# NilanEkanayake/TiTok-Video

Hardware: AMD Instinct MI355X
Metric: video clips/sec encode+decode (whole node) (higher is better)
Workload: dtype bf16

## Files before the change

### titok_video_amd/csrc/ttv_api.hip

```cpp
#include <stdarg.h>
#include <stdio.h>
#include <stdlib.h>
#include <string.h>

#include "ttv_common.h"
#include "ttv_kernels.h"

static thread_local char g_err[512] = "";

void ttv_set_error(const char* fmt, ...) {
  va_list ap;
  va_start(ap, fmt);
  vsnprintf(g_err, sizeof(g_err), fmt, ap);
  va_end(ap);
}

int g_ttv_prof_class = 0;
thread_local int g_ttv_debug = 0;
long long* g_ttv_stamps = nullptr;
static hipEvent_t* g_prof_start = nullptr;
static hipEvent_t* g_prof_stop = nullptr;
static int g_prof_cap = 0, g_prof_n = 0;

TtvProfScope::TtvProfScope(int cls, hipStream_t stream) : slot(-1), s(stream) {
  if (g_ttv_prof_class != 0 && cls == g_ttv_prof_class && g_prof_n < g_prof_cap) {
    slot = g_prof_n++;
    (void)hipEventRecord(g_prof_start[slot], s);
  }
}
TtvProfScope::~TtvProfScope() {
  if (slot >= 0) (void)hipEventRecord(g_prof_stop[slot], s);
}

#define TTV_TRY(expr)            \
  do {                           \
    int rc__ = (expr);           \
    if (rc__ != TTV_OK) return rc__; \
  } while (0)

static inline int esize(int dtype) { return dtype == TTV_BF16 ? 2 : 4; }
static inline int64_t align_up(int64_t v) { return (v + 255) & ~(int64_t)255; }

struct TowerWs {
  char *x, *xn, *qkv, *ao, *h, *pa, *pb;
  char *xl, *aol;
  char *f8, *f8mx;
  float* y32;
  float* rstd;
  int64_t total;
};

static TowerWs carve(const ttv_tower_dims* d, const ttv_batch* b, char* base) {
  const int64_t e = esize(d->dtype);
  const int64_t L = b->total_rows, P = b->sum_patches;
  const int64_t g = (int64_t)d->kv_heads * d->head_dim;
  const int64_t pd = (int64_t)d->pix_channels * d->patch_t * d->patch_h * d->patch_w;
  int64_t off = 0;
  TowerWs w;
  auto take = [&](int64_t bytes) { char* p = base ? base + off : nullptr; off += align_up(bytes); return p; };
  w.x = take(L * d->width * e);
  w.xn = take(L * d->width * e);
  w.qkv = take(L * (2 * d->width + 2 * g) * e);
  w.ao = take(L * d->width * e);
  w.y32 = (float*)take(L * d->width * 4);
  w.h = take(L * d->inner * e);
  w.pa = take(P * pd * e);
  w.pb = take(P * d->width * e);
  w.rstd = (float*)take(L * 4);
  w.xl = take((int64_t)b->sum_tokens * d->width * e);
  w.aol = take((int64_t)b->sum_tokens * d->width * e);
  w.f8 = w.f8mx = nullptr;
  if (d->dtype == TTV_BF16 && d->width != 256 && d->width % 128 == 0) {
    const int64_t wide = d->width > d->inner ? d->width : d->inner;
    w.f8 = take(L * wide);
    w.f8mx = take(L * (wide / 128 + 4) * 4);
  }
  w.total = off;
  return w;
}

static int check_dims(const ttv_tower_dims* d, const ttv_batch* b) {
  TTV_CHECK_ARG(d && b, "null dims/batch");
  TTV_CHECK_ARG(d->dtype == TTV_BF16 || d->dtype == TTV_F32, "bad dtype %d", d->dtype);
  TTV_CHECK_ARG(d->head_dim == 64 && d->width == d->q_heads * 64, "width must be q_heads*64");
  TTV_CHECK_ARG(d->width % 64 == 0 && d->width <= 1024, "width %d unsupported", d->width);
  TTV_CHECK_ARG(d->inner % 32 == 0, "GEGLU inner dim must be a multiple of 32");
  TTV_CHECK_ARG(d->token_size >= 1 && d->token_size <= TTV_MAX_TOKEN, "token_size out of range");
  TTV_CHECK_ARG(((int64_t)d->pix_channels * d->patch_t * d->patch_h * d->patch_w) % 8 == 0, "patch vector length must be a multiple of 8");
  TTV_CHECK_ARG(b->n_clips > 0 && b->total_rows == b->sum_tokens + b->sum_patches, "inconsistent batch");
  return TTV_OK;
}

static int run_layer_mx(const ttv_tower_dims* d, const ttv_layer_weights& lw, const ttv_batch* b, const TowerWs& ws, int i, bool& rstd_valid,
                        bool& xq_valid, bool attn_pipe, hipStream_t s) {
  const int L = b->total_rows, dm = d->width, g = d->kv_heads * d->head_dim, dt = d->dtype, nq = 2 * dm + 2 * g, I = d->inner;
  static const bool fused_env = !(getenv("TTV_MX_FUSED_QUANT") && getenv("TTV_MX_FUSED_QUANT")[0] == '0');
  const bool fused_q = fused_env && !(g_ttv_debug & 2048);
  if (!rstd_valid) TTV_TRY(ttvk_row_rstd(ws.x, dt, dm, ws.rstd, L, dm, d->eps, s));
  if (!xq_valid) TTV_TRY(ttvk_quant_mx_fp8(ws.x, dt, dm, ws.f8, dm, ws.f8mx, nullptr, L, dm, s));
  xq_valid = false;
  GemmArgs a = {};
  a.dtype = dt; a.x = ws.f8; a.ldx = dm; a.w = lw.to_qkv_f8; a.ldw = dm; a.M = L; a.N = nq; a.K = dm; a.y = ws.qkv; a.ldy = nq;
  a.rope_cs = b->rope_cs; a.rope_q_end = dm; a.rope_k_begin = 2 * dm; a.rope_k_end = 2 * dm + g;
  TTV_TRY(ttvk_gemm_fp8(EPI_QKV_ROPE, a, ws.rstd, lw.to_qkv_f8_scale, s, ws.f8mx, lw.to_qkv_mx));
  const bool q_scaled = lw.qkv_q_prescaled != 0;
  if (fused_q && q_scaled && !b->qblocks_paired && !attn_pipe && d->head_dim == 64) {
    TTV_TRY(ttvk_attention_mxout(ws.qkv, nq, ws.f8, ws.f8mx, (int)ttvk_mx_scale_ld(dm), b->cu_seqlens, b->qblocks, b->n_qblocks, d->q_heads,
                                 d->kv_heads, s));
  } else {
    TTV_TRY(ttvk_attention(ws.qkv, nq, ws.ao, dm, b->cu_seqlens, b->qblocks, b->n_qblocks, d->q_heads, d->kv_heads, d->head_dim,
                           TTV_ATTN_GATE | (b->qblocks_paired ? TTV_ATTN_PAIRED : 0) | (q_scaled ? TTV_ATTN_QSCALED : 0) |
                               ((b->qblocks_all_full && attn_pipe) ? TTV_ATTN_ALLFULL : 0) | (attn_pipe ? TTV_ATTN_PIPE : 0), dt, s));
    TTV_TRY(ttvk_quant_mx_fp8(ws.ao, dt, dm, ws.f8, dm, ws.f8mx, nullptr, L, dm, s));
  }
  GemmArgs o = {};
  o.dtype = dt; o.x = ws.f8; o.ldx = dm; o.w = lw.out_proj_f8; o.ldw = dm; o.M = L; o.N = dm; o.K = dm; o.resid = ws.x; o.ldr = dm;
  o.alpha = i == 0 ? 1.f : d->alpha; o.y = ws.x; o.ldy = dm;
  TTV_TRY(ttvk_gemm_fp8(EPI_RESID_T, o, nullptr, lw.out_proj_f8_scale, s, ws.f8mx, lw.out_proj_mx));
  if (i > 0) {
    TTV_TRY(ttvk_rmsnorm(ws.x, dt, dm, nullptr, ws.x, dt, dm, nullptr, lw.attn_post_ln, L, dm, d->eps, s, ws.rstd, fused_q ? ws.f8 : nullptr,
                         fused_q ? ws.f8mx : nullptr));
    if (!fused_q) TTV_TRY(ttvk_quant_mx_fp8(ws.x, dt, dm, ws.f8, dm, ws.f8mx, nullptr, L, dm, s));
  } else {
    TTV_TRY(ttvk_row_rstd(ws.x, dt, dm, ws.rstd, L, dm, d->eps, s));
    TTV_TRY(ttvk_quant_mx_fp8(ws.x, dt, dm, ws.f8, dm, ws.f8mx, nullptr, L, dm, s));
  }
  GemmArgs f = {};
  f.dtype = dt; f.x = ws.f8; f.ldx = dm; f.w = lw.w12_f8; f.ldw = dm; f.M = L; f.N = I; f.K = dm; f.y = ws.h; f.ldy = I;
  char* const hq = ws.h;
  char* const hq_mx = ws.xn;
  const bool h_fused = fused_q && (int64_t)ttvk_mx_scale_ld(I) <= (int64_t)dm * 2;
  if (h_fused) { f.yq = hq; f.yq_mx = hq_mx; }
  TTV_TRY(ttvk_gemm_fp8(EPI_GEGLU, f, ws.rstd, lw.w12_f8_scale, s, ws.f8mx, lw.w12_mx));
  GemmArgs f3 = {};
  if (h_fused) {
    f3.x = hq;
  } else {
    TTV_TRY(ttvk_quant_mx_fp8(ws.h, dt, I, ws.f8, I, ws.f8mx, nullptr, L, I, s));
    f3.x = ws.f8;
  }
  f3.dtype = dt; f3.ldx = I; f3.w = lw.w3_f8; f3.ldw = I; f3.M = L; f3.N = dm; f3.K = I; f3.resid = ws.x; f3.ldr = dm;
  f3.alpha = i == 0 ? 1.f : d->alpha; f3.y = ws.x; f3.ldy = dm;
  TTV_TRY(ttvk_gemm_fp8(EPI_RESID_T, f3, nullptr, lw.w3_f8_scale, s, h_fused ? hq_mx : ws.f8mx, lw.w3_mx));
  rstd_valid = false;
  if (i > 0) {
    TTV_TRY(ttvk_rmsnorm(ws.x, dt, dm, nullptr, ws.x, dt, dm, nullptr, lw.ffd_post_ln, L, dm, d->eps, s, ws.rstd, fused_q ? ws.f8 : nullptr,
                         fused_q ? ws.f8mx : nullptr));
    rstd_valid = true;
    xq_valid = fused_q;
  }
  return TTV_OK;
}

static bool rows_f8(int dt, int dm, const void* img, const void* row_scale, const void* mx, const void* folded) {
  return dt == TTV_BF16 && img && row_scale && !mx && dm % 128 == 0 && !(dm == 256 && folded);
}

static int run_layers(const ttv_tower_dims* d, const ttv_tower_weights* w, const ttv_batch* b, const TowerWs& ws, hipStream_t s) {
  const int L = b->total_rows, dm = d->width, g = d->kv_heads * d->head_dim, dt = d->dtype;
  const int split3 = (dt == TTV_F32 && w->f32_split3) ? 1 : 0;
  const bool gen_ok = (dt == TTV_BF16 && dm != 256) || split3;
  static const bool s3img_env = !(getenv("TTV_SPLIT3_IMAGES") && getenv("TTV_SPLIT3_IMAGES")[0] == '0');
  const int s3img = (split3 && s3img_env && !(g_ttv_debug & 4096)) ? 1 : 0;
  const int nq = 2 * dm + 2 * g;
  bool qkv_ready = false;
  bool rstd_valid = false;
  bool xq_valid = false;
  static const bool attn_pipe = getenv("TTV_ATTN_PIPE") && getenv("TTV_ATTN_PIPE")[0] == '1';
  static const bool lat_env = !(getenv("TTV_ENC_LATENT_LAST") && getenv("TTV_ENC_LATENT_LAST")[0] == '0');
  const bool lat_last = lat_env && !(g_ttv_debug & 524288) && d->kind == TTV_ENCODER && b->qblocks_latent && b->n_qblocks_latent > 0 &&
                        b->latent_rows && b->sum_tokens > 0 && b->sum_tokens < L;
  static const bool pat_env = !(getenv("TTV_DEC_PATCH_LAST") && getenv("TTV_DEC_PATCH_LAST")[0] == '0');
  const bool pat_last = pat_env && !(g_ttv_debug & 2097152) && d->kind == TTV_DECODER && d->layers >= 2 && b->qblocks_patch &&
                        b->n_qblocks_patch > 0 && !split3 && !b->qblocks_paired;
  bool compacted = false;
  for (int i = 0; i < d->layers; ++i) {
    const ttv_layer_weights& lw = w->layers[i];
    static const bool keel_f32 = getenv("TTV_KEEL_F32SUM") && getenv("TTV_KEEL_F32SUM")[0] == '1';
    if (dt == TTV_BF16 && dm != 256 && dm % 128 == 0 && d->inner % 128 == 0 && !keel_f32 && lw.to_qkv_f8 && lw.to_qkv_mx && lw.w12_f8 && lw.w12_mx &&
        lw.out_proj_f8 && lw.out_proj_mx && lw.w3_f8 && lw.w3_mx &&
        !(lat_last && i == d->layers - 1)) {
      TTV_TRY(run_layer_mx(d, lw, b, ws, i, rstd_valid, xq_valid, attn_pipe, s));
      qkv_ready = false;
      continue;
    }
    xq_valid = false;
    const bool f8_qkv = rows_f8(dt, dm, lw.to_qkv_f8, lw.to_qkv_f8_scale, lw.to_qkv_mx, lw.to_qkv_pn);
    const bool f8_w12 = rows_f8(dt, dm, lw.w12_f8, lw.w12_f8_scale, lw.w12_mx, lw.w12_pn);
    float* const f8_scales = reinterpret_cast<float*>(ws.xn + (((size_t)L * dm + 255) & ~(size_t)255));
    if (!qkv_ready && f8_qkv) {
      TTV_TRY(ttvk_quant_rows_fp8(ws.x, dt, dm, lw.pre_ln, d->eps, ws.xn, dm, f8_scales, L, dm, s));
      GemmArgs a = {};
      a.dtype = dt; a.x = ws.xn; a.ldx = dm; a.w = lw.to_qkv_f8; a.ldw = dm; a.M = L; a.N = nq; a.K = dm; a.y = ws.qkv; a.ldy = nq;
      a.rope_cs = b->rope_cs; a.rope_q_end = dm; a.rope_k_begin = 2 * dm; a.rope_k_end = 2 * dm + g;
      TTV_TRY(ttvk_gemm_fp8(EPI_QKV_ROPE, a, f8_scales, lw.to_qkv_f8_scale, s));
    } else if (!qkv_ready) {
      const bool fold_qkv = dt == TTV_BF16 && dm == 256 && lw.to_qkv_pn;
      const bool fold_gen = gen_ok && lw.to_qkv_pn;
      if (fold_gen && !rstd_valid) TTV_TRY(ttvk_row_rstd(ws.x, dt, dm, ws.rstd, L, dm, d->eps, s));
      if (!fold_qkv && !fold_gen) TTV_TRY(ttvk_rmsnorm(ws.x, dt, dm, nullptr, ws.xn, dt, dm, nullptr, lw.pre_ln, L, dm, d->eps, s, nullptr, nullptr, nullptr, s3img));
      GemmArgs a = {};
      a.dtype = dt; a.split3 = split3; a.x_image = s3img && !fold_qkv && !fold_gen; a.y_image = s3img ? 2 : 0;
      a.prenorm = fold_qkv; a.eps = d->eps;
      a.row_scale = fold_gen ? ws.rstd : nullptr;
      const void* w_plain = (dt == TTV_BF16 && lw.to_qkv_qs) ? lw.to_qkv_qs : lw.to_qkv;
      a.x = (fold_qkv || fold_gen) ? ws.x : ws.xn; a.ldx = dm; a.w = (fold_qkv || fold_gen) ? lw.to_qkv_pn : w_plain; a.ldw = dm; a.M = L; a.N = nq; a.K = dm; a.y = ws.qkv; a.ldy = nq;
      a.rope_cs = b->rope_cs; a.rope_q_end = dm; a.rope_k_begin = 2 * dm; a.rope_k_end = 2 * dm + g;
      a.rope_ids = b->rope_ids; a.rope_base = b->rope_ids ? b->rope_base : nullptr;
      TTV_TRY(ttvk_gemm(EPI_QKV_ROPE, a, s));
    }
    const bool q_scaled = dt == TTV_BF16 && (lw.to_qkv_pn ? lw.qkv_q_prescaled != 0 : lw.to_qkv_qs != nullptr);
    rstd_valid = false;
    qkv_ready = false;
    const bool lat_now = lat_last && i == d->layers - 1;
    if (lat_now)
      TTV_TRY(ttvk_attention(ws.qkv, nq, ws.ao, dm, b->cu_seqlens, b->qblocks_latent, b->n_qblocks_latent, d->q_heads, d->kv_heads, d->head_dim,
                             TTV_ATTN_GATE | (b->qblocks_all_full ? TTV_ATTN_ALLFULL : 0) | (q_scaled ? TTV_ATTN_QSCALED : 0) | (split3 ? TTV_ATTN_SPLIT3 : 0) |
                                 (s3img ? (TTV_ATTN_SPLIT_OUT | TTV_ATTN_SPLIT_IN) : 0), dt, s));
    else if (pat_last && i == d->layers - 1 && dt == TTV_BF16 && !attn_pipe)
      TTV_TRY(ttvk_attention(ws.qkv, nq, ws.ao, dm, b->cu_seqlens, b->qblocks_patch, b->n_qblocks_patch, d->q_heads, d->kv_heads, d->head_dim,
                             TTV_ATTN_GATE | (b->qblocks_all_full ? TTV_ATTN_ALLFULL : 0) | (q_scaled ? TTV_ATTN_QSCALED : 0), dt, s));
    else if (q_scaled && b->items64 && b->n_items64 > 0 && d->head_dim == 64)
      TTV_TRY(ttvk_attention64(ws.qkv, nq, ws.ao, dm, b->cu_seqlens, b->items64, b->n_items64, d->q_heads, d->kv_heads,
                               TTV_ATTN_GATE | TTV_ATTN_QSCALED, s));
    else
    TTV_TRY(ttvk_attention(ws.qkv, nq, ws.ao, dm, b->cu_seqlens, b->qblocks, b->n_qblocks, d->q_heads, d->kv_heads, d->head_dim,
                           TTV_ATTN_GATE | (b->qblocks_paired ? TTV_ATTN_PAIRED : 0) | (q_scaled ? TTV_ATTN_QSCALED : 0) |
                               (b->qblocks_all_full ? TTV_ATTN_ALLFULL : 0) | (attn_pipe ? TTV_ATTN_PIPE : 0) | (split3 ? TTV_ATTN_SPLIT3 : 0) |
                               (s3img ? (TTV_ATTN_SPLIT_OUT | TTV_ATTN_SPLIT_IN) : 0), dt, s));
    char* cx = ws.x;
    char* cao = ws.ao;
    int Lc = L;
    if (lat_now) {
      const int64_t rb = (int64_t)dm * esize(dt);
      TTV_TRY(ttvk_copy_rows(ws.x, (int64_t)dm * esize(dt), b->latent_rows, ws.xl, (int64_t)dm * esize(dt), nullptr, b->sum_tokens, dm * (int)esize(dt), s));
      TTV_TRY(ttvk_copy_rows(ws.ao, rb, b->latent_rows, ws.aol, rb, nullptr, b->sum_tokens, (int)rb, s));
      cx = ws.xl; cao = ws.aol; Lc = b->sum_tokens;
      compacted = true;
    }
    static const bool keel_f32sum = getenv("TTV_KEEL_F32SUM") && getenv("TTV_KEEL_F32SUM")[0] == '1';
    static const bool use_fused_mlp = !(getenv("TTV_FUSED_MLP") && getenv("TTV_FUSED_MLP")[0] == '0');
    static const bool use_fused_qkv = getenv("TTV_FUSED_QKV") && getenv("TTV_FUSED_QKV")[0] == '1';
    if (use_fused_mlp && ttvk_mlp_fused_supported(dt, dm, d->inner) && lw.mlp_pack) {
      MlpNextQkv nx = {};
      const bool back = use_fused_qkv && i + 1 < d->layers && lw.mlp_pack_qkv_rows == nq && nq % 64 == 0 && dm % 64 == 0 && g % 64 == 0;
      if (back) { nx.qkv = ws.qkv; nx.ld = nq; nx.rope_cs = b->rope_cs; nx.rows = nq; nx.rope_q_end = dm; nx.rope_k_begin = 2 * dm; nx.rope_k_end = 2 * dm + g; }
      TTV_TRY(ttvk_mlp_fused(cao, dm, i == 0 ? nullptr : lw.attn_post_ln, i == 0 ? 1.f : d->alpha, cx, dm, lw.mlp_pack, d->inner,
                             cx, dm, i == 0 ? nullptr : lw.ffd_post_ln, i == 0 ? 1.f : d->alpha, d->eps, Lc, back ? &nx : nullptr, s));
      qkv_ready = back;
      continue;
    }
    GemmArgs o = {};
    o.dtype = dt; o.split3 = split3; o.x_image = s3img;
    o.x = cao; o.ldx = dm; o.w = lw.out_proj; o.ldw = dm; o.M = Lc; o.N = dm; o.K = dm; o.resid = cx; o.ldr = dm;
    if (i == 0) {
      o.alpha = 1.f; o.y = cx; o.ldy = dm;
      TTV_TRY(ttvk_gemm(EPI_RESID_T, o, s));
    } else if (ttvk_gemm_supports_resid_norm(dt, dm, dm)) {
      o.alpha = d->alpha; o.y = cx; o.ldy = dm; o.norm_gain = lw.attn_post_ln; o.eps = d->eps;
      TTV_TRY(ttvk_gemm(EPI_RESID_NORM, o, s));
    } else {
      const bool want = gen_ok && lw.w12_pn && !f8_w12;
      if (dt == TTV_BF16 && !keel_f32sum) {
        o.alpha = d->alpha; o.y = cx; o.ldy = dm;
        TTV_TRY(ttvk_gemm(EPI_RESID_T, o, s));
        TTV_TRY(ttvk_rmsnorm(cx, dt, dm, nullptr, cx, dt, dm, nullptr, lw.attn_post_ln  , Lc, dm, d->eps, s, want ? ws.rstd : nullptr));
      } else {
        o.alpha = d->alpha; o.y = ws.y32; o.ldy = dm;
        TTV_TRY(ttvk_gemm(EPI_RESID_F32, o, s));
        TTV_TRY(ttvk_rmsnorm(ws.y32, TTV_F32, dm, nullptr, cx, dt, dm, nullptr, lw.attn_post_ln  , Lc, dm, d->eps, s, want ? ws.rstd : nullptr));
      }
      rstd_valid = want;
    }
    const bool fold_ffd = dt == TTV_BF16 && dm == 256 && lw.w12_pn;
    const bool fold_ffd_gen = gen_ok && lw.w12_pn && !f8_w12;
    if (f8_w12) {
      TTV_TRY(ttvk_quant_rows_fp8(cx, dt, dm, lw.ffd_norm, d->eps, ws.xn, dm, f8_scales, Lc, dm, s));
      GemmArgs f = {};
      f.dtype = dt; f.x = ws.xn; f.ldx = dm; f.w = lw.w12_f8; f.ldw = dm; f.M = Lc; f.N = d->inner; f.K = dm; f.y = ws.h; f.ldy = d->inner;
      TTV_TRY(ttvk_gemm_fp8(EPI_GEGLU, f, f8_scales, lw.w12_f8_scale, s));
    } else {
    if (fold_ffd_gen && !rstd_valid) TTV_TRY(ttvk_row_rstd(cx, dt, dm, ws.rstd  , Lc, dm, d->eps, s));
    if (!fold_ffd && !fold_ffd_gen) TTV_TRY(ttvk_rmsnorm(cx, dt, dm, nullptr, ws.xn, dt, dm, nullptr, lw.ffd_norm  , Lc, dm, d->eps, s, nullptr, nullptr, nullptr, s3img));
    GemmArgs f = {};
    f.dtype = dt; f.split3 = split3; f.x_image = s3img && !fold_ffd && !fold_ffd_gen; f.y_image = s3img;
    f.prenorm = fold_ffd; f.eps = d->eps;
    f.row_scale = fold_ffd_gen ? ws.rstd : nullptr;
    f.x = (fold_ffd || fold_ffd_gen) ? cx : ws.xn; f.ldx = dm; f.w = (fold_ffd || fold_ffd_gen) ? lw.w12_pn : lw.w12; f.ldw = dm; f.M = Lc; f.N = d->inner; f.K = dm; f.y = ws.h; f.ldy = d->inner;
    TTV_TRY(ttvk_gemm(EPI_GEGLU, f, s));
    }
    rstd_valid = false;
    GemmArgs f3 = {};
    f3.dtype = dt; f3.split3 = split3; f3.x_image = s3img;
    f3.x = ws.h; f3.ldx = d->inner; f3.w = lw.w3; f3.ldw = d->inner; f3.M = Lc; f3.N = dm; f3.K = d->inner; f3.resid = cx; f3.ldr = dm;
    if (i == 0) {
      f3.alpha = 1.f; f3.y = cx; f3.ldy = dm;
      TTV_TRY(ttvk_gemm(EPI_RESID_T, f3, s));
    } else if (ttvk_gemm_supports_resid_norm(dt, dm, d->inner)) {
      f3.alpha = d->alpha; f3.y = cx; f3.ldy = dm; f3.norm_gain = lw.ffd_post_ln; f3.eps = d->eps;
      TTV_TRY(ttvk_gemm(EPI_RESID_NORM, f3, s));
    } else {
      const bool want = gen_ok && i + 1 < d->layers && w->layers[i + 1].to_qkv_pn &&
                        !rows_f8(dt, dm, w->layers[i + 1].to_qkv_f8, w->layers[i + 1].to_qkv_f8_scale, w->layers[i + 1].to_qkv_mx, w->layers[i + 1].to_qkv_pn);
      if (dt == TTV_BF16 && !keel_f32sum) {
        f3.alpha = d->alpha; f3.y = cx; f3.ldy = dm;
        TTV_TRY(ttvk_gemm(EPI_RESID_T, f3, s));
        TTV_TRY(ttvk_rmsnorm(cx, dt, dm, nullptr, cx, dt, dm, nullptr, lw.ffd_post_ln  , Lc, dm, d->eps, s, want ? ws.rstd : nullptr));
      } else {
        f3.alpha = d->alpha; f3.y = ws.y32; f3.ldy = dm;
        TTV_TRY(ttvk_gemm(EPI_RESID_F32, f3, s));
        TTV_TRY(ttvk_rmsnorm(ws.y32, TTV_F32, dm, nullptr, cx, dt, dm, nullptr, lw.ffd_post_ln  , Lc, dm, d->eps, s, want ? ws.rstd : nullptr));
      }
      rstd_valid = want;
    }
  }
  if (compacted)
    TTV_TRY(ttvk_copy_rows(ws.xl, (int64_t)dm * esize(dt), nullptr, ws.x, (int64_t)dm * esize(dt), b->latent_rows, b->sum_tokens, dm * (int)esize(dt), s));
  return TTV_OK;
}

extern "C" {

const char* ttv_error_string(void) { return g_err; }
int ttv_version(void) { return 100; }

int ttv_fsq_forward(const ttv_fsq_params* p, const void* z, int z_dtype, int rows, void* codes, int codes_dtype, int32_t* indices,
                    float* bounded, void* stream) {
  TTV_CHECK_ARG(rows >= 0 && (rows == 0 || (z && codes && indices)), "fsq_forward: null buffer");
  return ttvk_fsq_forward(p, z, z_dtype, rows, codes, codes_dtype, indices, bounded, (hipStream_t)stream);
}

int ttv_fsq_indices_to_codes(const ttv_fsq_params* p, const int32_t* indices, int rows, void* codes, int codes_dtype, void* stream) {
  TTV_CHECK_ARG(rows >= 0 && (rows == 0 || (indices && codes)), "fsq_indices_to_codes: null buffer");
  return ttvk_fsq_indices_to_codes(p, indices, rows, codes, codes_dtype, (hipStream_t)stream);
}

int ttv_vq_codebook_norms(const void* codebook, int dtype, int ld, int N, int C, float* cnorm, void* stream) {
  TTV_CHECK_ARG(N == 0 || (codebook && cnorm), "vq_codebook_norms: null buffer");
  return ttvk_vq_norms(codebook, dtype, ld, N, C, cnorm, (hipStream_t)stream);
}

int64_t ttv_vq_workspace_bytes(int rows) { return ttvk_vq_workspace_bytes(rows); }

int ttv_vq_l2_argmin(const void* z, int dtype, int ldz, const void* codebook, int ldc, const float* cnorm, int rows, int N, int C,
                     int32_t* indices, float* best_dist, void* workspace, int64_t workspace_bytes, void* stream) {
  TTV_CHECK_ARG(rows == 0 || (z && codebook && cnorm && indices), "vq_l2_argmin: null buffer");
  TTV_CHECK_ARG(ldz >= C && ldc >= C, "vq_l2_argmin: leading dims smaller than the codebook dim");
  return ttvk_vq_l2_argmin(z, dtype, ldz, codebook, ldc, cnorm, rows, N, C, indices, best_dist, workspace, workspace_bytes, (hipStream_t)stream);
}

int ttv_vq_lookup(const void* codebook, int dtype, int ldc, const int32_t* indices, int rows, int C, void* codes, int ldo, void* stream) {
  TTV_CHECK_ARG(rows == 0 || (codebook && indices && codes), "vq_lookup: null buffer");
  return ttvk_vq_lookup(codebook, dtype, ldc, indices, rows, C, codes, ldo, (hipStream_t)stream);
}

int ttv_vq_lookup_backward(const void* dcodes, int dtype, int ld, const int32_t* indices, int rows, int C, float* dcodebook, int ldc, void* stream) {
  TTV_CHECK_ARG(rows == 0 || (dcodes && indices && dcodebook), "vq_lookup_backward: null buffer");
  TTV_CHECK_ARG(ld >= C && ldc >= C, "vq_lookup_backward: leading dims smaller than the codebook dim");
  return ttvk_vq_lookup_bwd(dcodes, dtype, ld, indices, rows, C, dcodebook, ldc, (hipStream_t)stream);
}

int ttv_quant_rows_fp8(const void* in, int dtype, int ld_in, const float* gain, float eps, void* out, int ld_out, float* scales, int rows,
                       int width, void* stream) {
  TTV_CHECK_ARG(rows == 0 || (in && out && scales), "quant_rows_fp8: null buffer");
  return ttvk_quant_rows_fp8(in, dtype, ld_in, gain, eps, out, ld_out, scales, rows, width, (hipStream_t)stream);
}

int ttv_split3_pack(const float* w, int ldw, void* out, int ldo, int rows, int K, void* stream) {
  TTV_CHECK_ARG(rows == 0 || (w && out), "split3_pack: null buffer");
  return ttvk_split3_pack(w, ldw, out, ldo, rows, K, (hipStream_t)stream);
}

int ttv_linear_split3(const float* x, int ldx, const void* w_image, int ldw, const float* bias, float* y, int ldy, int M, int N, int K, void* stream) {
  TTV_CHECK_ARG(M == 0 || (x && w_image && y), "linear_split3: null buffer");
  GemmArgs a = {};
  a.dtype = TTV_F32; a.split3 = 1; a.x = x; a.ldx = ldx; a.w = w_image; a.ldw = ldw; a.M = M; a.N = N; a.K = K; a.y = y; a.ldy = ldy; a.bias = bias;
  return ttvk_gemm(EPI_STORE, a, (hipStream_t)stream);
}

int64_t ttv_mx_scale_bytes_per_row(int width) { return ttvk_mx_scale_ld(width); }

int ttv_quant_mx_fp8(const void* in, int dtype, int ld_in, void* out, int ld_out, void* mx, float* row_scales, int rows, int width, void* stream) {
  TTV_CHECK_ARG(rows == 0 || (in && out && mx), "quant_mx_fp8: null buffer");
  TTV_CHECK_ARG(ld_in >= width && ld_out >= width, "quant_mx_fp8: leading dims smaller than the width");
  return ttvk_quant_mx_fp8(in, dtype, ld_in, out, ld_out, mx, row_scales, rows, width, (hipStream_t)stream);
}

int ttv_linear_fp8_mx(const void* xq, int ldx, const void* x_mx, const float* x_row_scale, const void* wq, int ldw, const void* w_mx,
                      const float* w_row_scale, void* y, int ldy, int M, int N, int K, int epilogue, const float* rope_cs, int d_model,
                      int gqa_dim, const void* resid, int ldr, float alpha, void* stream) {
  TTV_CHECK_ARG(M == 0 || (xq && wq && y && x_mx && w_mx), "linear_fp8_mx: null buffer");
  TTV_CHECK_ARG(epilogue >= 0 && epilogue <= 3, "linear_fp8_mx: epilogue 0 (store), 1 (qkv + rotary), 2 (GEGLU) or 3 (alpha * resid + acc)");
  GemmArgs a = {};
  a.dtype = TTV_BF16; a.x = xq; a.ldx = ldx; a.w = wq; a.ldw = ldw; a.M = M; a.N = N; a.K = K; a.y = y; a.ldy = ldy;
  if (epilogue == 1) {
    TTV_CHECK_ARG(rope_cs && N == 2 * d_model + 2 * gqa_dim, "linear_fp8_mx: qkv epilogue needs rope_cs and N = 2 d_model + 2 gqa_dim");
    a.rope_cs = rope_cs; a.rope_q_end = d_model; a.rope_k_begin = 2 * d_model; a.rope_k_end = 2 * d_model + gqa_dim;
  }
  if (epilogue == 3) { a.resid = resid; a.ldr = ldr; a.alpha = alpha; }
  return ttvk_gemm_fp8(epilogue == 0 ? EPI_STORE : epilogue == 1 ? EPI_QKV_ROPE : epilogue == 2 ? EPI_GEGLU : EPI_RESID_T, a, x_row_scale,
                       w_row_scale, (hipStream_t)stream, x_mx, w_mx);
}

int ttv_linear_fp8(const void* xq, int ldx, const float* x_scale, const void* wq, int ldw, const float* w_scale, void* y, int ldy, int M, int N,
                   int K, int epilogue, const float* rope_cs, int d_model, int gqa_dim, void* stream) {
  TTV_CHECK_ARG(M == 0 || (xq && wq && y), "linear_fp8: null buffer");
  TTV_CHECK_ARG(epilogue >= 0 && epilogue <= 2, "linear_fp8: epilogue 0 (store), 1 (qkv + rotary) or 2 (GEGLU)");
  GemmArgs a = {};
  a.dtype = TTV_BF16; a.x = xq; a.ldx = ldx; a.w = wq; a.ldw = ldw; a.M = M; a.N = N; a.K = K; a.y = y; a.ldy = ldy;
  if (epilogue == 1) {
    TTV_CHECK_ARG(rope_cs && N == 2 * d_model + 2 * gqa_dim, "linear_fp8: qkv epilogue needs rope_cs and N = 2 d_model + 2 gqa_dim");
    a.rope_cs = rope_cs; a.rope_q_end = d_model; a.rope_k_begin = 2 * d_model; a.rope_k_end = 2 * d_model + gqa_dim;
  }
  return ttvk_gemm_fp8(epilogue == 0 ? EPI_STORE : epilogue == 1 ? EPI_QKV_ROPE : EPI_GEGLU, a, x_scale, w_scale, (hipStream_t)stream);
}

int ttv_rmsnorm(const void* in, int in_dtype, int ld_in, const int32_t* src_rows, void* out, int out_dtype, int ld_out,
                const int32_t* dst_rows, const float* gain, int rows, int width, float eps, void* stream) {
  TTV_CHECK_ARG(rows >= 0 && (rows == 0 || (in && out && gain)), "rmsnorm: null buffer");
  return ttvk_rmsnorm(in, in_dtype, ld_in, src_rows, out, out_dtype, ld_out, dst_rows, gain, rows, width, eps, (hipStream_t)stream);
}

int ttv_rope_apply(void* x, int dtype, int ld, int rows, int heads, const float* rope_cs, void* stream) {
  TTV_CHECK_ARG(rows == 0 || (x && rope_cs), "rope_apply: null buffer");
  TTV_CHECK_ARG(ld % 4 == 0 && ld >= heads * 64, "rope_apply: bad leading dim");
  return ttvk_rope_apply(x, dtype, ld, rows, heads, rope_cs, (hipStream_t)stream);
}

int ttv_linear(const void* x, int ldx, const void* w, int ldw, const void* bias, const float* add_scalar, void* y, int ldy, int M,
               int N, int K, int dtype, void* stream) {
  TTV_CHECK_ARG(M == 0 || (x && w && y), "linear: null buffer");
  GemmArgs a = {};
  a.dtype = dtype; a.x = x; a.ldx = ldx; a.w = w; a.ldw = ldw; a.M = M; a.N = N; a.K = K; a.y = y; a.ldy = ldy;
  a.bias = bias; a.add_scalar = add_scalar;
  return ttvk_gemm(EPI_STORE, a, (hipStream_t)stream);
}

int ttv_linear_qkv_rope(const void* x, int ldx, const void* w, int ldw, void* y, int ldy, int M, int d_model, int gqa_dim,
                        const float* rope_cs, int dtype, void* stream) {
  TTV_CHECK_ARG(M == 0 || (x && w && y && rope_cs), "linear_qkv_rope: null buffer");
  GemmArgs a = {};
  a.dtype = dtype; a.x = x; a.ldx = ldx; a.w = w; a.ldw = ldw; a.M = M; a.N = 2 * d_model + 2 * gqa_dim; a.K = d_model;
  a.y = y; a.ldy = ldy; a.rope_cs = rope_cs; a.rope_q_end = d_model; a.rope_k_begin = 2 * d_model; a.rope_k_end = 2 * d_model + gqa_dim;
  return ttvk_gemm(EPI_QKV_ROPE, a, (hipStream_t)stream);
}

int ttv_linear_geglu(const void* x, int ldx, const void* w, int ldw, void* y, int ldy, int M, int I, int K, int dtype, void* stream) {
  TTV_CHECK_ARG(M == 0 || (x && w && y), "linear_geglu: null buffer");
  GemmArgs a = {};
  a.dtype = dtype; a.x = x; a.ldx = ldx; a.w = w; a.ldw = ldw; a.M = M; a.N = I; a.K = K; a.y = y; a.ldy = ldy;
  return ttvk_gemm(EPI_GEGLU, a, (hipStream_t)stream);
}

int ttv_linear_residual(const void* x, int ldx, const void* w, int ldw, const void* resid, int ldr, float alpha, void* y, int ldy,
                        int y_f32, int M, int N, int K, int dtype, void* stream) {
  TTV_CHECK_ARG(M == 0 || (x && w && y && resid), "linear_residual: null buffer");
  GemmArgs a = {};
  a.dtype = dtype; a.x = x; a.ldx = ldx; a.w = w; a.ldw = ldw; a.M = M; a.N = N; a.K = K; a.y = y; a.ldy = ldy;
  a.resid = resid; a.ldr = ldr; a.alpha = alpha;
  return ttvk_gemm(y_f32 ? EPI_RESID_F32 : EPI_RESID_T, a, (hipStream_t)stream);
}

int ttv_linear_residual_norm(const void* x, int ldx, const void* w, int ldw, const void* resid, int ldr, float alpha,
                             const float* gain, float eps, void* y, int ldy, int M, int N, int K, int dtype, void* stream) {
  TTV_CHECK_ARG(M == 0 || (x && w && y && resid && gain), "linear_residual_norm: null buffer");
  GemmArgs a = {};
  a.dtype = dtype; a.x = x; a.ldx = ldx; a.w = w; a.ldw = ldw; a.M = M; a.N = N; a.K = K; a.y = y; a.ldy = ldy;
  a.resid = resid; a.ldr = ldr; a.alpha = alpha; a.norm_gain = gain; a.eps = eps;
  if (!ttvk_gemm_supports_resid_norm(dtype, N, K)) {
    ttv_set_error("linear_residual_norm: only bf16 with N == 256 has a fused kernel");
    return TTV_ERR_UNSUPPORTED;
  }
  return ttvk_gemm(EPI_RESID_NORM, a, (hipStream_t)stream);
}

int64_t ttv_mlp_pack_bytes(int inner, int next_qkv_rows) { return ttvk_mlp_pack_bytes(inner, next_qkv_rows); }

int ttv_mlp_pack(const void* w12_folded, const void* w3, const void* out_proj, const void* next_qkv_folded, int next_qkv_rows, int inner,
                 int width, int dtype, void* packed, void* stream) {
  if (!ttvk_mlp_fused_supported(dtype, width, inner)) {
    ttv_set_error("mlp_pack: only bf16, width 256, inner %% 32 == 0");
    return TTV_ERR_UNSUPPORTED;
  }
  return ttvk_mlp_pack(w12_folded, w3, out_proj, next_qkv_folded, next_qkv_rows, inner, packed, (hipStream_t)stream);
}

int ttv_mlp_fused(const void* x, int ldx, const void* mlp_packed, int inner, void* y, int ldy, const float* post_gain, float alpha,
                  float eps, int M, int width, int dtype, void* stream) {
  if (!ttvk_mlp_fused_supported(dtype, width, inner)) {
    ttv_set_error("mlp_fused: only bf16, width 256, inner %% 32 == 0");
    return TTV_ERR_UNSUPPORTED;
  }
  return ttvk_mlp_fused(nullptr, 0, nullptr, 1.f, x, ldx, mlp_packed, inner, y, ldy, post_gain, alpha, eps, M, nullptr, (hipStream_t)stream);
}

int ttv_layer_tail_fused(const void* ao, int ldao, const float* attn_post_gain, float attn_alpha, const void* x, int ldx,
                         const void* mlp_packed, int inner, void* y, int ldy, const float* ffd_post_gain, float ffd_alpha, float eps,
                         int M, int width, int dtype, const ttv_next_qkv* next, void* stream) {
  if (!ttvk_mlp_fused_supported(dtype, width, inner)) {
    ttv_set_error("layer_tail_fused: only bf16, width 256, inner %% 32 == 0");
    return TTV_ERR_UNSUPPORTED;
  }
  TTV_CHECK_ARG(ao, "layer_tail_fused: null attention output");
  MlpNextQkv nx = {};
  if (next) { nx.qkv = next->qkv; nx.ld = next->ld; nx.rope_cs = next->rope_cs; nx.rows = next->rows; nx.rope_q_end = next->rope_q_end;
              nx.rope_k_begin = next->rope_k_begin; nx.rope_k_end = next->rope_k_end; }
  return ttvk_mlp_fused(ao, ldao, attn_post_gain, attn_alpha, x, ldx, mlp_packed, inner, y, ldy, ffd_post_gain, ffd_alpha, eps, M,
                        next ? &nx : nullptr, (hipStream_t)stream);
}

int ttv_fill_const_rows(void* x, int dtype, int ld, const int32_t* rows_map, int rows, int width, const float* mask_token,
                        const float* gain, float eps, void* stream) {
  TTV_CHECK_ARG(rows == 0 || (x && rows_map && mask_token && gain), "fill_const_rows: null buffer");
  return ttvk_fill_const_rows(x, dtype, ld, rows_map, rows, width, mask_token, gain, eps, (hipStream_t)stream);
}

int ttv_decoder_embed(const void* codes, int token_size, const void* w, const void* bias, const float* mask_token, const float* gain,
                      void* x, int dtype, int ld, const int32_t* rows_map, int rows, int width, float eps, void* stream) {
  TTV_CHECK_ARG(rows == 0 || (codes && w && bias && mask_token && gain && x && rows_map), "decoder_embed: null buffer");
  return ttvk_dec_embed(codes, token_size, w, bias, mask_token, gain, x, dtype, ld, rows_map, rows, width, eps, (hipStream_t)stream);
}

int ttv_attention(const void* qkvg, int ld, void* out, int ldo, const int32_t* cu_seqlens, const int32_t* qblocks, int n_qblocks,
                  int q_heads, int kv_heads, int head_dim, int flags, int dtype, void* stream) {
  TTV_CHECK_ARG(n_qblocks == 0 || (qkvg && out && cu_seqlens && qblocks), "attention: null buffer");
  return ttvk_attention(qkvg, ld, out, ldo, cu_seqlens, qblocks, n_qblocks, q_heads, kv_heads, head_dim, flags, dtype, (hipStream_t)stream);
}
int ttv_attention64(const void* qkvg, int ld, void* out, int ldo, const int32_t* cu_seqlens, const int32_t* items, int n_items, int q_heads,
                    int kv_heads, int head_dim, int flags, int dtype, void* stream) {
  TTV_CHECK_ARG(dtype == TTV_BF16 && head_dim == 64, "attention64: bf16, head_dim 64 only");
  return ttvk_attention64(qkvg, ld, out, ldo, cu_seqlens, items, n_items, q_heads, kv_heads, flags, (hipStream_t)stream);
}

int ttv_patch_gather(const void* const* clips, const int32_t* clip_desc, int clip0, int n_clips, int patch_t, int patch_h, int patch_w,
                     int channels, void* patches, int ld, int dtype, int max_patches_per_clip, void* stream) {
  TTV_CHECK_ARG(n_clips == 0 || (clips && clip_desc && patches), "patch_gather: null buffer");
  return ttvk_patch_copy(false, (void* const*)clips, clip_desc, clip0, n_clips, patch_t, patch_h, patch_w, channels, patches, ld, dtype, max_patches_per_clip, (hipStream_t)stream);
}

int ttv_patch_scatter(const void* patches, int ld, const int32_t* clip_desc, int clip0, int n_clips, int patch_t, int patch_h, int patch_w,
                      int channels, void* const* clips, int dtype, int max_patches_per_clip, void* stream) {
  TTV_CHECK_ARG(n_clips == 0 || (clips && clip_desc && patches), "patch_scatter: null buffer");
  return ttvk_patch_copy(true, clips, clip_desc, clip0, n_clips, patch_t, patch_h, patch_w, channels, (void*)patches, ld, dtype, max_patches_per_clip, (hipStream_t)stream);
}

int64_t ttv_tower_workspace_bytes(const ttv_tower_dims* dims, const ttv_batch* batch) {
  if (check_dims(dims, batch) != TTV_OK) return -1;
  return carve(dims, batch, nullptr).total;
}

int ttv_encoder_forward(const ttv_tower_dims* d, const ttv_tower_weights* w, const ttv_batch* b, const void* const* clips,
                        const ttv_fsq_params* fsq, float* z, void* codes, int32_t* indices, float* bounded, void* workspace,
                        int64_t workspace_bytes, void* stream) {
  TTV_TRY(check_dims(d, b));
  TTV_CHECK_ARG(d->kind == TTV_ENCODER, "encoder_forward: dims.kind is not TTV_ENCODER");
  TTV_CHECK_ARG(w && w->layers && clips && workspace, "encoder_forward: null argument");
  TTV_CHECK_ARG(fsq || z, "encoder_forward: neither fsq nor z requested");
  TTV_CHECK_ARG(!fsq || (codes && indices), "encoder_forward: fsq needs codes and indices buffers");
  hipStream_t s = (hipStream_t)stream;
  TowerWs ws = carve(d, b, (char*)workspace);
  TTV_CHECK_ARG(ws.total <= workspace_bytes, "encoder_forward: workspace too small (%lld < %lld)", (long long)workspace_bytes, (long long)ws.total);
  const int dm = d->width, dt = d->dtype, P = b->sum_patches;
  const int pd = d->pix_channels * d->patch_t * d->patch_h * d->patch_w;

  static const bool use_fused_patch = !(getenv("TTV_FUSED_PATCH") && getenv("TTV_FUSED_PATCH")[0] == '0');
  auto pow2 = [](int v) { return v > 0 && (v & (v - 1)) == 0; };
  const bool gather = use_fused_patch && dt == TTV_BF16 && d->patch_w == 8 && pow2(d->patch_t) && pow2(d->patch_h) &&
                      b->n_clips <= TTV_MAX_CLIPS_PER_LAUNCH && b->row_seq && pd % 64 == 0 && pd != 256;
  if (!gather) {
    for (int c0 = 0; c0 < b->n_clips; c0 += TTV_MAX_CLIPS_PER_LAUNCH) {
      const int n = b->n_clips - c0 < TTV_MAX_CLIPS_PER_LAUNCH ? b->n_clips - c0 : TTV_MAX_CLIPS_PER_LAUNCH;
      TTV_TRY(ttvk_patch_copy(false, (void* const*)(clips + c0), b->clip_desc, c0, n, d->patch_t, d->patch_h, d->patch_w, d->pix_channels, ws.pa, pd, dt, b->max_patches_per_clip, s));
    }
  }
  GemmArgs a = {};
  a.dtype = dt; a.x = ws.pa; a.ldx = pd; a.w = w->proj_in_w; a.ldw = pd; a.M = P; a.N = dm; a.K = pd; a.y = ws.pb; a.ldy = dm;
  a.bias = w->proj_in_b; a.add_scalar = w->mask_token;
  a.split3 = (dt == TTV_F32 && w->f32_split3) ? 1 : 0;
  if (gather) {
    a.gather = 1; a.clips = (void* const*)clips; a.n_clips = b->n_clips; a.clip_desc = b->clip_desc; a.patch_rows = b->patch_rows;
    a.row_seq = b->row_seq; a.patch_t = d->patch_t; a.patch_h = d->patch_h; a.patch_w = d->patch_w;
  }
  TTV_TRY(ttvk_gemm(EPI_STORE, a, s));
  TTV_TRY(ttvk_rmsnorm(ws.pb, dt, dm, nullptr, ws.x, dt, dm, b->patch_rows, w->ln_pre_p, P, dm, d->eps, s));
  TTV_TRY(ttvk_fill_const_rows(ws.x, dt, dm, b->latent_rows, b->sum_tokens, dm, w->mask_token, w->ln_pre_t, d->eps, s));

  TTV_TRY(run_layers(d, w, b, ws, s));

  TTV_TRY(ttvk_enc_tail(ws.x, dt, dm, b->latent_rows, b->sum_tokens, dm, w->ln_post, d->eps, w->proj_out_w, w->proj_out_b, d->token_size, fsq, z, codes, indices, bounded, s));
  return TTV_OK;
}

int ttv_decoder_forward(const ttv_tower_dims* d, const ttv_tower_weights* w, const ttv_batch* b, const void* codes,
                        void* const* clips_out, void* workspace, int64_t workspace_bytes, void* stream) {
  TTV_TRY(check_dims(d, b));
  TTV_CHECK_ARG(d->kind == TTV_DECODER, "decoder_forward: dims.kind is not TTV_DECODER");
  TTV_CHECK_ARG(w && w->layers && codes && clips_out && workspace, "decoder_forward: null argument");
  hipStream_t s = (hipStream_t)stream;
  TowerWs ws = carve(d, b, (char*)workspace);
  TTV_CHECK_ARG(ws.total <= workspace_bytes, "decoder_forward: workspace too small (%lld < %lld)", (long long)workspace_bytes, (long long)ws.total);
  const int dm = d->width, dt = d->dtype, P = b->sum_patches;
  const int pd = d->pix_channels * d->patch_t * d->patch_h * d->patch_w;

  TTV_TRY(ttvk_dec_embed(codes, d->token_size, w->proj_in_w, w->proj_in_b, w->mask_token, w->ln_pre_t, ws.x, dt, dm, b->latent_rows, b->sum_tokens, dm, d->eps, s));
  TTV_TRY(ttvk_fill_const_rows(ws.x, dt, dm, b->patch_rows, P, dm, w->mask_token, w->ln_pre_p, d->eps, s));

  TTV_TRY(run_layers(d, w, b, ws, s));

  GemmArgs a = {};
  a.dtype = dt; a.w = w->proj_out_w; a.ldw = dm; a.M = P; a.N = pd; a.K = dm; a.y = ws.pa; a.ldy = pd; a.ldx = dm;
  a.split3 = (dt == TTV_F32 && w->f32_split3) ? 1 : 0;
  a.bias = w->proj_out_b;
  if (dt == TTV_BF16 && dm == 256 && w->proj_out_pn && pd % 8 == 0) {
    a.x = ws.x; a.x_rows = b->patch_rows; a.w = w->proj_out_pn; a.prenorm = 1; a.eps = d->eps;
  } else {
    TTV_TRY(ttvk_rmsnorm(ws.x, dt, dm, b->patch_rows, ws.pb, dt, dm, nullptr, w->ln_post, P, dm, d->eps, s));
    a.x = ws.pb;
  }
  static const bool use_fused_patch = !(getenv("TTV_FUSED_PATCH") && getenv("TTV_FUSED_PATCH")[0] == '0');
  auto pow2 = [](int v) { return v > 0 && (v & (v - 1)) == 0; };
  if (use_fused_patch && dt == TTV_BF16 && dm == 256 && d->patch_w == 8 && pow2(d->patch_t) && pow2(d->patch_h) &&
      b->n_clips <= TTV_MAX_CLIPS_PER_LAUNCH && b->row_seq && pd % 64 == 0) {
    a.clips = clips_out; a.n_clips = b->n_clips; a.clip_desc = b->clip_desc; a.patch_rows = b->patch_rows; a.row_seq = b->row_seq;
    a.patch_t = d->patch_t; a.patch_h = d->patch_h; a.patch_w = d->patch_w;
    return ttvk_gemm(EPI_STORE_PATCH, a, s);
  }
  TTV_TRY(ttvk_gemm(EPI_STORE, a, s));
  for (int c0 = 0; c0 < b->n_clips; c0 += TTV_MAX_CLIPS_PER_LAUNCH) {
    const int n = b->n_clips - c0 < TTV_MAX_CLIPS_PER_LAUNCH ? b->n_clips - c0 : TTV_MAX_CLIPS_PER_LAUNCH;
    TTV_TRY(ttvk_patch_copy(true, clips_out + c0, b->clip_desc, c0, n, d->patch_t, d->patch_h, d->patch_w, d->pix_channels, ws.pa, pd, dt, b->max_patches_per_clip, s));
  }
  return TTV_OK;
}

int ttv_rope_table_build(const float* base_cos, const float* base_sin, int n_ids, int n_freqs, const int32_t* clip_desc, const int32_t* cu_seqlens,
                         const int32_t* row_seq, float* rope_cs, int total_rows, void* stream) {
  TTV_CHECK_ARG(total_rows == 0 || (base_cos && base_sin && clip_desc && cu_seqlens && row_seq && rope_cs), "rope_table_build: null buffer");
  TTV_CHECK_ARG(n_freqs >= 1 && 3 * n_freqs <= 32 && n_ids >= 1, "rope_table_build: bad table shape");
  return ttvk_rope_build(base_cos, base_sin, n_ids, n_freqs, clip_desc, cu_seqlens, row_seq, rope_cs, total_rows, (hipStream_t)stream);
}

int ttv_l1_loss(void* const* recon, void* const* target, void* const* grad, const int32_t* sizes, int n_clips, int dtype, float* loss,
                void* stream) {
  for (int c0 = 0; c0 < n_clips; c0 += TTV_MAX_CLIPS_PER_LAUNCH) {
    const int n = n_clips - c0 < TTV_MAX_CLIPS_PER_LAUNCH ? n_clips - c0 : TTV_MAX_CLIPS_PER_LAUNCH;
    TTV_TRY(ttvk_l1_loss(recon + c0, target + c0, grad ? grad + c0 : nullptr, sizes + c0, n, n_clips, dtype, loss, (hipStream_t)stream));
  }
  return TTV_OK;
}

int ttv_clip_from_u8(const void* frames_thwc, int T, int H, int W, void* clip_cthw, int dtype, void* stream) {
  TTV_CHECK_ARG(frames_thwc && clip_cthw && T > 0 && H > 0 && W > 0, "clip_from_u8: bad argument");
  return ttvk_clip_from_u8(frames_thwc, (long long)T * H * W, clip_cthw, dtype, (hipStream_t)stream);
}

int ttv_sq_err_accumulate(void* const* recon, void* const* target, const int32_t* sizes, int n_clips, int dtype, int clamp, double* acc,
                          void* stream) {
  for (int c0 = 0; c0 < n_clips; c0 += TTV_MAX_CLIPS_PER_LAUNCH) {
    const int n = n_clips - c0 < TTV_MAX_CLIPS_PER_LAUNCH ? n_clips - c0 : TTV_MAX_CLIPS_PER_LAUNCH;
    TTV_TRY(ttvk_sq_err(recon + c0, target + c0, sizes + c0, n, dtype, clamp, acc, (hipStream_t)stream));
  }
  return TTV_OK;
}

int ttv_debug_set(int flags) {
  g_ttv_debug = flags;
  return TTV_OK;
}

int ttv_debug_stamps(void* device_buffer) {
  g_ttv_stamps = (long long*)device_buffer;
  return TTV_OK;
}

int ttv_prof_begin(int kernel_class, int max_records) {
  TTV_CHECK_ARG(g_ttv_prof_class == 0, "prof_begin: already recording");
  TTV_CHECK_ARG(kernel_class > 0 && max_records > 0 && max_records <= (1 << 20), "prof_begin: bad arguments");
  g_prof_start = new hipEvent_t[max_records];
  g_prof_stop = new hipEvent_t[max_records];
  for (int i = 0; i < max_records; ++i) {
    if (hipEventCreate(&g_prof_start[i]) != hipSuccess || hipEventCreate(&g_prof_stop[i]) != hipSuccess) {
      ttv_set_error("prof_begin: hipEventCreate failed");
      return TTV_ERR_LAUNCH;
    }
  }
  g_prof_cap = max_records;
  g_prof_n = 0;
  g_ttv_prof_class = kernel_class;
  return TTV_OK;
}

int ttv_prof_end(double* total_ms, int* count) {
  TTV_CHECK_ARG(g_ttv_prof_class != 0 && total_ms && count, "prof_end: not recording");
  g_ttv_prof_class = 0;
  double tot = 0.0;
  for (int i = 0; i < g_prof_n; ++i) {
    float ms = 0.f;
    (void)hipEventSynchronize(g_prof_stop[i]);
    (void)hipEventElapsedTime(&ms, g_prof_start[i], g_prof_stop[i]);
    tot += ms;
  }
  *total_ms = tot;
  *count = g_prof_n;
  for (int i = 0; i < g_prof_cap; ++i) {
    (void)hipEventDestroy(g_prof_start[i]);
    (void)hipEventDestroy(g_prof_stop[i]);
  }
  delete[] g_prof_start;
  delete[] g_prof_stop;
  g_prof_start = g_prof_stop = nullptr;
  g_prof_cap = g_prof_n = 0;
  return TTV_OK;
}

int ttv_codebook_histogram(const int32_t* indices, int n, int64_t* counts, int codebook_size, void* stream) {
  TTV_CHECK_ARG(n == 0 || (indices && counts), "codebook_histogram: null buffer");
  return ttvk_histogram(indices, n, counts, codebook_size, (hipStream_t)stream);
}

}
```

### titok_video_amd/csrc/ttv_attn.hip

```cpp
#include <stdlib.h>

#include "ttv_common.h"
#include "ttv_kernels.h"

#define QB 128
#define KB 64
#define ATTN_DEFER_THR 8.0f
#ifndef ATTN_LAZY
#define ATTN_LAZY 1
#endif
#ifndef ATTN_DMA_LATE
#define ATTN_DMA_LATE 1
#endif
#ifndef ATTN_PRIO
#define ATTN_PRIO 0
#endif
#define ATTN_LAZY_LOG2 30
#define ATTN_LAZY_BIG 1073741824.0f
typedef float f32x2 __attribute__((ext_vector_type(2)));

typedef __attribute__((address_space(3))) bf16x4 lds_bf16x4;

__device__ __forceinline__ bf16x4 lds_read_tr16(const char* lds_ptr) {
  return __builtin_amdgcn_ds_read_tr16_b64_v4bf16((lds_bf16x4*)(lds_ptr));
// ... 1044 lines not shown
        l_run += psum;
#pragma unroll
        for (int e = 0; e < 16; ++e) {
          const int vk = t * 32 + (e & 3) + 8 * (e >> 2) + 4 * h;
          const float v0 = vl[vk * 64 + r], v1 = vl[vk * 64 + 32 + r];
          o_acc[0] = __builtin_amdgcn_mfma_f32_32x32x2f32(v0, sc[e], o_acc[0], 0, 0, 0);
          o_acc[1] = __builtin_amdgcn_mfma_f32_32x32x2f32(v1, sc[e], o_acc[1], 0, 0, 0);
        }
      }
    }
  }
#undef A32_GLOAD
#undef A32_LSTORE
  if (!wave_live) return;

  const float l_tot = l_run + __shfl_xor(l_run, 32, 64);
  const float inv_l = 1.0f / l_tot;
  if (lse_out && qrow < q_lim && h == 0)
    lse_out[(size_t)(s0 + qrow) * (d_model >> 6) + head] = m_run * (c_exp * 0.69314718055994530942f) + logf(l_tot);
  if (qrow < q_lim) {
    float* orow = out + (size_t)(s0 + qrow) * ldo + head * 64;
    const float* grow = gbase + (size_t)qrow * ld;
#pragma unroll
    for (int dt = 0; dt < 2; ++dt)
#pragma unroll
      for (int g = 0; g < 4; ++g) {
        const int d0 = dt * 32 + 8 * g + 4 * h;
        f32x4 v = {o_acc[dt][4 * g] * inv_l, o_acc[dt][4 * g + 1] * inv_l, o_acc[dt][4 * g + 2] * inv_l, o_acc[dt][4 * g + 3] * inv_l};
        if (GATE) {
          const f32x4 gt = *reinterpret_cast<const f32x4*>(grow + d0);
#pragma unroll
          for (int e = 0; e < 4; ++e) v[e] *= 1.0f / (1.0f + expf(-gt[e]));
        }
        *reinterpret_cast<f32x4*>(orow + d0) = v;
      }
  }
}

__device__ __forceinline__ void split4_f32(const uint4 v, uint2& hi, uint2& lo) {
  const float x0 = __uint_as_float(v.x), x1 = __uint_as_float(v.y), x2 = __uint_as_float(v.z), x3 = __uint_as_float(v.w);
  const bf16_t h0 = (bf16_t)x0, h1 = (bf16_t)x1, h2 = (bf16_t)x2, h3 = (bf16_t)x3;
  const bf16x4 hv = {h0, h1, h2, h3};
  const bf16x4 lv = {(bf16_t)(x0 - (float)h0), (bf16_t)(x1 - (float)h1), (bf16_t)(x2 - (float)h2), (bf16_t)(x3 - (float)h3)};
  hi = __builtin_bit_cast(uint2, hv);
  lo = __builtin_bit_cast(uint2, lv);
}

template <bool GATE, bool IMG = false>
__global__ __launch_bounds__(256, 2) void k_attn_split3(const float* __restrict__ qkvg, int ld, float* __restrict__ out, int ldo,
                                                        const int* __restrict__ cu, const int* __restrict__ qblocks, int d_model, int gqa,
                                                        int rep, float c_exp , int out_image) {
  __shared__ __attribute__((aligned(16))) uint4 tiles[2][4][KB * 8];
  const int tid = threadIdx.x, lane = tid & 63;
  const int wave = __builtin_amdgcn_readfirstlane(tid >> 6);
  const int r = lane & 31, h = lane >> 5;
  const int seq = qblocks[4 * blockIdx.x], q0 = qblocks[4 * blockIdx.x + 1], head = qblocks[4 * blockIdx.x + 2];
  const int mode = qblocks[4 * blockIdx.x + 3];
  if (seq < 0) return;
  const int s0 = cu[seq], S = cu[seq + 1] - s0;
  const int q_lim = (mode && q0 + 64 < S) ? q0 + 64 : S;
  const bool wave_live = !(mode && wave >= 2);
  const int kvh = head / rep;
  const float* qbase = qkvg + (size_t)s0 * ld + head * 64;
  const float* gbase = qkvg + (size_t)s0 * ld + d_model + head * 64;
  const float* kbase = qkvg + (size_t)s0 * ld + 2 * d_model + kvh * 64;
  const float* vbase = kbase + gqa;

  const int qrow = q0 + wave * 32 + r;
  const int qrc = qrow < S ? qrow : S - 1;
  bf16x8 qh[4], ql[4];
#pragma unroll
  for (int ks = 0; ks < 4; ++ks) {
    const uint4 a = *reinterpret_cast<const uint4*>(qbase + (size_t)qrc * ld + ks * 16 + h * 8);
    const uint4 b = *reinterpret_cast<const uint4*>(qbase + (size_t)qrc * ld + ks * 16 + h * 8 + 4);
    if (IMG) {
      qh[ks] = __builtin_bit_cast(bf16x8, a);
      ql[ks] = __builtin_bit_cast(bf16x8, b);
    } else {
      uint2 ah, al, bh, bl;
      split4_f32(a, ah, al);
      split4_f32(b, bh, bl);
      qh[ks] = __builtin_bit_cast(bf16x8, make_uint4(ah.x, ah.y, bh.x, bh.y));
      ql[ks] = __builtin_bit_cast(bf16x8, make_uint4(al.x, al.y, bl.x, bl.y));
    }
  }

  const int skey = tid >> 4, sch = tid & 15;
  uint4 sk[4], sv[4];
#define S3_GLOAD(kt_)                                                                      \
  do {                                                                                     \
    _Pragma("unroll") for (int i__ = 0; i__ < 4; ++i__) {                                  \
      int k__ = (kt_) * KB + skey + 16 * i__;                                              \
      k__ = k__ < S ? k__ : S - 1;                                                         \
      sk[i__] = *reinterpret_cast<const uint4*>(kbase + (size_t)k__ * ld + sch * 4);       \
      sv[i__] = *reinterpret_cast<const uint4*>(vbase + (size_t)k__ * ld + sch * 4);       \
    }                                                                                      \
  } while (0)
  char* const tile0 = reinterpret_cast<char*>(&tiles[0][0][0]);
  constexpr int STAGE = 4 * KB * 128, PLANE = KB * 128;
  const int kst = skey * 128 + (((sch >> 1) ^ ((skey >> 1) & 7)) << 4) + (sch & 1) * 8;
  const int vst = skey * 128 + (((sch >> 1) ^ (((skey >> 1) & 1) << 2)) << 4) + (sch & 1) * 8;
#define S3_LSTORE(stage_)                                                                  \
  do {                                                                                     \
    char* const sb__ = tile0 + (stage_) * STAGE;                                           \
    _Pragma("unroll") for (int i__ = 0; i__ < 4; ++i__) {                                  \
      uint2 hi__, lo__;                                                                    \
      split4_f32(sk[i__], hi__, lo__);                                                     \
      *reinterpret_cast<uint2*>(sb__ + kst + i__ * 2048) = hi__;                           \
      *reinterpret_cast<uint2*>(sb__ + PLANE + kst + i__ * 2048) = lo__;                   \
      split4_f32(sv[i__], hi__, lo__);                                                     \
      *reinterpret_cast<uint2*>(sb__ + 2 * PLANE + vst + i__ * 2048) = hi__;               \
      *reinterpret_cast<uint2*>(sb__ + 3 * PLANE + vst + i__ * 2048) = lo__;               \
    }                                                                                      \
  } while (0)

  const int ksw = (r >> 1) & 7;
  int koff[4];
#pragma unroll
  for (int ks = 0; ks < 4; ++ks) koff[ks] = r * 128 + (((ks * 2 + h) ^ ksw) << 4);
  const int gi = lane & 15, tq = gi >> 2, tp = gi & 3, g16 = (lane >> 4) & 1;
  const int vsw = (tq >> 1) & 1;
  const int vlane = (4 * h + tq) * 128 + (g16 * 2 + (tp >> 1)) * 16 + (tp & 1) * 8;
  const int voff_d0 = vlane + (vsw ? 64 : 0), voff_d1 = vlane + (vsw ? 0 : 64);

  f32x16 o_acc[2];
#pragma unroll
  for (int dt = 0; dt < 2; ++dt)
#pragma unroll
    for (int e = 0; e < 16; ++e) o_acc[dt][e] = 0.f;
  float m_run = -INFINITY, l_run = 0.f;
  const f32x16 zero16 = {0.f, 0.f, 0.f, 0.f, 0.f, 0.f, 0.f, 0.f, 0.f, 0.f, 0.f, 0.f, 0.f, 0.f, 0.f, 0.f};

  const int nkt = (S + KB - 1) / KB;
  const uint32_t tiles_lds = (uint32_t)(uintptr_t)(__attribute__((address_space(3))) void*)&tiles[0][0][0];
  const int drow = lane >> 3, dpos = lane & 7;
#define S3_DMA(voff_, base_, dst_)                                                                               \
  do {                                                                                                           \
    unsigned keep__;                                                                                             \
    asm volatile("s_mov_b32 %0, m0\n\ts_mov_b32 m0, %3\n\ts_nop 0\n\tglobal_load_lds_dwordx4 %1, %2\n\ts_mov_b32 m0, %0" \
                 : "=&s"(keep__) : "v"(voff_), "s"(base_), "s"(dst_) : "memory");                                 \
  } while (0)
#define S3_DMA_TILE(kt_, stage_)                                                                                 \
  do {                                                                                                           \
    _Pragma("unroll") for (int i__ = 0; i__ < 2; ++i__) {                                                        \
      const int row__ = wave * 16 + i__ * 8 + drow;                                                              \
      int key__ = (kt_) * KB + row__;                                                                            \
      key__ = key__ < S ? key__ : S - 1;                                                                         \
      const uint32_t rb__ = (uint32_t)key__ * (uint32_t)ld * 4u;                                                 \
      const uint32_t kc__ = (uint32_t)((dpos ^ ((row__ >> 1) & 7)) * 32);                                        \
      const uint32_t vc__ = (uint32_t)((dpos ^ (((row__ >> 1) & 1) << 2)) * 32);                                 \
      const uint32_t dst__ = tiles_lds + (stage_) * STAGE + (wave * 16 + i__ * 8) * 128;                         \
      S3_DMA(rb__ + kc__, kbase, dst__);                                                                         \
      S3_DMA(rb__ + kc__ + 16u, kbase, dst__ + PLANE);                                                           \
      S3_DMA(rb__ + vc__, vbase, dst__ + 2 * PLANE);                                                             \
      S3_DMA(rb__ + vc__ + 16u, vbase, dst__ + 3 * PLANE);                                                       \
    }                                                                                                            \
  } while (0)
  if (IMG) {
    S3_DMA_TILE(0, 0);
  } else {
    S3_GLOAD(0);
    S3_LSTORE(0);
    if (nkt > 1) S3_GLOAD(1);
  }
  for (int kt = 0; kt < nkt; ++kt) {
    if (IMG) __builtin_amdgcn_s_waitcnt(0x0F70);
    __syncthreads();
    if (IMG) {
      if (kt + 1 < nkt) S3_DMA_TILE(kt + 1, (kt + 1) & 1);
    } else if (kt + 1 < nkt) {
      S3_LSTORE((kt + 1) & 1);
      if (kt + 2 < nkt) S3_GLOAD(kt + 2);
    }
    if (!wave_live) continue;
    const char* const tk_h = tile0 + (kt & 1) * STAGE;
    const char* const tk_l = tk_h + PLANE;
    const char* const tv_h = tk_h + 2 * PLANE;
    const char* const tv_l = tk_h + 3 * PLANE;
#pragma unroll
    for (int t = 0; t < 2; ++t) {
      if (kt * KB + t * 32 >= S) break;
      f32x16 sc = zero16;
      {
        bf16x8 kfh[4], kfl[4];
#pragma unroll
        for (int ks = 0; ks < 4; ++ks) {
          kfh[ks] = *reinterpret_cast<const bf16x8*>(tk_h + koff[ks] + t * 4096);
          kfl[ks] = *reinterpret_cast<const bf16x8*>(tk_l + koff[ks] + t * 4096);
        }
#pragma unroll
        for (int ks = 0; ks < 4; ++ks) sc = __builtin_amdgcn_mfma_f32_32x32x16_bf16(kfl[ks], qh[ks], sc, 0, 0, 0);
#pragma unroll
        for (int ks = 0; ks < 4; ++ks) sc = __builtin_amdgcn_mfma_f32_32x32x16_bf16(kfh[ks], ql[ks], sc, 0, 0, 0);
#pragma unroll
        for (int ks = 0; ks < 4; ++ks) sc = __builtin_amdgcn_mfma_f32_32x32x16_bf16(kfh[ks], qh[ks], sc, 0, 0, 0);
      }
      if (kt * KB + t * 32 + 32 > S) {
#pragma unroll
        for (int e = 0; e < 16; ++e) {
          const int kk = kt * KB + t * 32 + (e & 3) + 8 * (e >> 2) + 4 * h;
          if (kk >= S) sc[e] = -INFINITY;
        }
      }
      float mx = sc[0];
#pragma unroll
      for (int e = 1; e < 16; ++e) mx = fmaxf(mx, sc[e]);
      mx = fmaxf(mx, __shfl_xor(mx, 32, 64));
      const float m_new = fmaxf(m_run, mx);
      const float mc = m_new * c_exp;
      float psum = 0.f;
#pragma unroll
      for (int e = 0; e < 16; ++e) {
        sc[e] = __builtin_amdgcn_exp2f(fmaf(sc[e], c_exp, -mc));
        psum += sc[e];
      }
      if (__builtin_amdgcn_ballot_w64(m_new > m_run) != 0ull) {
        const float alpha = __builtin_amdgcn_exp2f((m_run - m_new) * c_exp);
        l_run *= alpha;
#pragma unroll
        for (int dt = 0; dt < 2; ++dt)
#pragma unroll
          for (int e = 0; e < 16; ++e) o_acc[dt][e] *= alpha;
        m_run = m_new;
      }
      l_run += psum;
      bf16x8 ph[2], pl[2];
#pragma unroll
      for (int sp = 0; sp < 2; ++sp)
#pragma unroll
        for (int j = 0; j < 8; ++j) {
          const bf16_t hv = (bf16_t)sc[8 * sp + j];
          ph[sp][j] = hv;
          pl[sp][j] = (bf16_t)(sc[8 * sp + j] - (float)hv);
        }
#define S3_VFRAG(base_, dt_, sp_)                                                                                  \
  ({                                                                                                               \
    const char* vb__ = (base_) + ((dt_) == 0 ? voff_d0 : voff_d1) + t * 4096 + (sp_) * 2048;                       \
    const bf16x4 lo__ = lds_read_tr16(vb__), hi__ = lds_read_tr16(vb__ + 1024);                                    \
    (bf16x8){lo__[0], lo__[1], lo__[2], lo__[3], hi__[0], hi__[1], hi__[2], hi__[3]};                              \
  })
#pragma unroll
      for (int dt = 0; dt < 2; ++dt) {
        const bf16x8 vh0 = S3_VFRAG(tv_h, dt, 0), vh1 = S3_VFRAG(tv_h, dt, 1);
        const bf16x8 vl0 = S3_VFRAG(tv_l, dt, 0), vl1 = S3_VFRAG(tv_l, dt, 1);
        o_acc[dt] = __builtin_amdgcn_mfma_f32_32x32x16_bf16(vl0, ph[0], o_acc[dt], 0, 0, 0);
        o_acc[dt] = __builtin_amdgcn_mfma_f32_32x32x16_bf16(vl1, ph[1], o_acc[dt], 0, 0, 0);
        o_acc[dt] = __builtin_amdgcn_mfma_f32_32x32x16_bf16(vh0, pl[0], o_acc[dt], 0, 0, 0);
        o_acc[dt] = __builtin_amdgcn_mfma_f32_32x32x16_bf16(vh1, pl[1], o_acc[dt], 0, 0, 0);
        o_acc[dt] = __builtin_amdgcn_mfma_f32_32x32x16_bf16(vh0, ph[0], o_acc[dt], 0, 0, 0);
        o_acc[dt] = __builtin_amdgcn_mfma_f32_32x32x16_bf16(vh1, ph[1], o_acc[dt], 0, 0, 0);
      }
#undef S3_VFRAG
    }
  }
#undef S3_GLOAD
#undef S3_LSTORE
#undef S3_DMA_TILE
#undef S3_DMA
  if (!wave_live) return;

  const float l_tot = l_run + __shfl_xor(l_run, 32, 64);
  const float inv_l = 1.0f / l_tot;
  if (qrow < q_lim) {
    float* orow = out + (size_t)(s0 + qrow) * ldo + head * 64;
    const float* grow = gbase + (size_t)qrow * ld;
#pragma unroll
    for (int dt = 0; dt < 2; ++dt)
#pragma unroll
      for (int g = 0; g < 4; ++g) {
        const int d0 = dt * 32 + 8 * g + 4 * h;
        f32x4 v = {o_acc[dt][4 * g] * inv_l, o_acc[dt][4 * g + 1] * inv_l, o_acc[dt][4 * g + 2] * inv_l, o_acc[dt][4 * g + 3] * inv_l};
        if (GATE) {
          const f32x4 gt = *reinterpret_cast<const f32x4*>(grow + d0);
#pragma unroll
          for (int e = 0; e < 4; ++e) v[e] *= 1.0f / (1.0f + expf(-gt[e]));
        }
        if (out_image) {
          uint2 hi, lo;
          split4_f32(__builtin_bit_cast(uint4, v), hi, lo);
          *reinterpret_cast<uint4*>(orow + d0) = make_uint4(hi.x, hi.y, lo.x, lo.y);
        } else {
          *reinterpret_cast<f32x4*>(orow + d0) = v;
        }
      }
  }
}

int ttvk_attention_mxout(const void* qkvg, int ld, void* out_q, void* out_mx, int ld_mx, const int* cu_seqlens, const int* qblocks,
                         int n_qblocks, int q_heads, int kv_heads, hipStream_t s) {
  if (n_qblocks == 0) return TTV_OK;
  TTV_CHECK_ARG(kv_heads > 0 && q_heads % kv_heads == 0, "attention_mxout: q_heads %% kv_heads");
  const int d_model = q_heads * 64, gqa = kv_heads * 64, rep = q_heads / kv_heads;
  TTV_CHECK_ARG(ld >= 2 * d_model + 2 * gqa && ld % 8 == 0 && d_model % 128 == 0 && ld_mx == (int)(4 * ((d_model / 128 + 3) / 4 * 4)),
                "attention_mxout: bad leading dims (d_model %% 128, ld_mx = 4 * round_up(d_model / 128, 4))");
  TTV_CHECK_ARG(qkvg && out_q && out_mx && (uintptr_t)qkvg % 16 == 0 && (uintptr_t)out_q % 8 == 0, "attention_mxout: null / unaligned pointers");
  static const float defer_thr = getenv("TTV_ATTN_THR") ? (float)atof(getenv("TTV_ATTN_THR")) : ATTN_DEFER_THR;
  TtvProfScope prof(TTV_KC_ATTENTION, s);
  hipLaunchKernelGGL((k_attn_bf16<true, 1, true, false, true>), dim3(n_qblocks), dim3(256), 0, s, (const bf16_t*)qkvg, ld, (bf16_t*)nullptr, ld_mx,
                     cu_seqlens, qblocks, n_qblocks, d_model, gqa, rep, 1.0f, (float*)out_mx, (bf16_t*)out_q, defer_thr, g_ttv_stamps);
  TTV_CHECK_LAUNCH("attention_mxout");
  return TTV_OK;
}

int ttvk_attention(const void* qkvg, int ld, void* out, int ldo, const int* cu_seqlens, const int* qblocks, int n_qblocks,
                   int q_heads, int kv_heads, int head_dim, int flags, int dtype, hipStream_t s, float* lse_out, void* out_raw) {
  const int gate_mul = flags & 1, paired = (flags >> 1) & 1, prescaled = (flags >> 2) & 1;
  TTV_CHECK_ARG(!prescaled || dtype == TTV_BF16, "attention: pre-scaled q is a bf16 path option");
  TTV_CHECK_ARG(!out_raw || (dtype == TTV_BF16 && gate_mul), "attention: the second (ungated) output is a bf16 + gate option");
  if (n_qblocks == 0) return TTV_OK;
  TTV_CHECK_ARG(head_dim == 64, "attention: head_dim %d unsupported (the reference fixes 64, utils.py:8)", head_dim);
  TTV_CHECK_ARG(kv_heads > 0 && q_heads % kv_heads == 0, "attention: q_heads %% kv_heads");
  const int d_model = q_heads * 64, gqa = kv_heads * 64, rep = q_heads / kv_heads;
  TTV_CHECK_ARG(ld >= 2 * d_model + 2 * gqa && ld % 8 == 0 && ldo % 4 == 0, "attention: bad leading dims");
  TTV_CHECK_ARG((uintptr_t)qkvg % 16 == 0 && (uintptr_t)out % (dtype == TTV_F32 ? 16 : 8) == 0, "attention: unaligned pointers");
  dim3 grid(n_qblocks);
  const float scale = 0.125f;
  TtvProfScope prof(TTV_KC_ATTENTION, s);
  if (dtype == TTV_BF16) {
    const float c_exp = scale * 1.44269504088896340736f;
    const float c_eff = prescaled ? 1.0f : c_exp;
    static const float defer_thr = getenv("TTV_ATTN_THR") ? (float)atof(getenv("TTV_ATTN_THR")) : ATTN_DEFER_THR;
#define ATTN_LAUNCH(G_, NE_, P_, T_, grid_, threads_)                                                                                   \
  hipLaunchKernelGGL((k_attn_bf16<G_, NE_, (P_) && (NE_) == 1, T_>), grid_, dim3(threads_), 0, s, (const bf16_t*)qkvg, ld, (bf16_t*)out, ldo, \
                     cu_seqlens, qblocks, n_qblocks, d_model, gqa, rep, c_eff, lse_out, (bf16_t*)out_raw, defer_thr, g_ttv_stamps)
#define ATTN_PICK(NE_, grid_, threads_)                                                  \
  do {                                                                                   \
    if (tape) { if (gate_mul) ATTN_LAUNCH(true, NE_, false, true, grid_, threads_); else ATTN_LAUNCH(false, NE_, false, true, grid_, threads_); }  \
    else if (gate_mul) { if (prescaled) ATTN_LAUNCH(true, NE_, true, false, grid_, threads_); else ATTN_LAUNCH(true, NE_, false, false, grid_, threads_); }   \
    else { if (prescaled) ATTN_LAUNCH(false, NE_, true, false, grid_, threads_); else ATTN_LAUNCH(false, NE_, false, false, grid_, threads_); }          \
  } while (0)
    const bool tape = lse_out != nullptr || out_raw != nullptr;
    TTV_CHECK_ARG(!tape || !prescaled, "attention: the training-tape outputs need unscaled q");
    static const bool swp_env = !(getenv("TTV_ATTN_SWP") && getenv("TTV_ATTN_SWP")[0] == '0');
    if (swp_env && !(flags & TTV_ATTN_PIPE) && (flags & TTV_ATTN_ALLFULL) && prescaled && !paired && !tape && !(g_ttv_debug & 1048576)) {
      return ttvk_attention_swp(qkvg, ld, out, ldo, cu_seqlens, qblocks, n_qblocks, q_heads, kv_heads, gate_mul, s);
    }
    if ((flags & TTV_ATTN_PIPE) && (flags & TTV_ATTN_ALLFULL) && prescaled && !paired && !tape) {
      static const float pipe_thr = getenv("TTV_ATTN_PIPE_THR") ? (float)atof(getenv("TTV_ATTN_PIPE_THR")) : ATTN_PIPE_THR;
      if (gate_mul) hipLaunchKernelGGL((k_attn_pipe<true>), grid, dim3(256), 0, s, (const bf16_t*)qkvg, ld, (bf16_t*)out, ldo, cu_seqlens, qblocks, d_model, gqa, rep, pipe_thr, g_ttv_stamps);
      else hipLaunchKernelGGL((k_attn_pipe<false>), grid, dim3(256), 0, s, (const bf16_t*)qkvg, ld, (bf16_t*)out, ldo, cu_seqlens, qblocks, d_model, gqa, rep, pipe_thr, g_ttv_stamps);
    } else if (paired) {
      const int rows = ttv_cdiv(n_qblocks, 8), pairs = ttv_cdiv(rows, 2);
      dim3 g2(pairs * 8);
      ATTN_PICK(2, g2, 512);
    } else {
      ATTN_PICK(1, grid, 256);
    }
#undef ATTN_PICK
#undef ATTN_LAUNCH
  } else if (dtype == TTV_F32) {
    const float c_exp = scale * 1.44269504088896340736f;
    if (flags & TTV_ATTN_SPLIT3) {
      TTV_CHECK_ARG(!lse_out, "attention: the split-bf16 kernel is an inference path (no tape outputs)");
      const int img = (flags & TTV_ATTN_SPLIT_OUT) ? 1 : 0;
      if (flags & TTV_ATTN_SPLIT_IN) {
        if (gate_mul) hipLaunchKernelGGL((k_attn_split3<true, true>), grid, dim3(256), 0, s, (const float*)qkvg, ld, (float*)out, ldo, cu_seqlens, qblocks, d_model, gqa, rep, c_exp, img);
        else hipLaunchKernelGGL((k_attn_split3<false, true>), grid, dim3(256), 0, s, (const float*)qkvg, ld, (float*)out, ldo, cu_seqlens, qblocks, d_model, gqa, rep, c_exp, img);
      } else if (gate_mul) hipLaunchKernelGGL((k_attn_split3<true>), grid, dim3(256), 0, s, (const float*)qkvg, ld, (float*)out, ldo, cu_seqlens, qblocks, d_model, gqa, rep, c_exp, img);
      else hipLaunchKernelGGL((k_attn_split3<false>), grid, dim3(256), 0, s, (const float*)qkvg, ld, (float*)out, ldo, cu_seqlens, qblocks, d_model, gqa, rep, c_exp, img);
    } else if (gate_mul)
      hipLaunchKernelGGL((k_attn_f32<true>), grid, dim3(256), 0, s, (const float*)qkvg, ld, (float*)out, ldo, cu_seqlens, qblocks, d_model, gqa, rep, c_exp, lse_out);
    else
      hipLaunchKernelGGL((k_attn_f32<false>), grid, dim3(256), 0, s, (const float*)qkvg, ld, (float*)out, ldo, cu_seqlens, qblocks, d_model, gqa, rep, c_exp, lse_out);
  } else {
    ttv_set_error("attention: bad dtype");
    return TTV_ERR_INVALID;
  }
  TTV_CHECK_LAUNCH("attention");
  return TTV_OK;
}
```

### titok_video_amd/csrc/ttv_attn_swp.hip

```cpp
#include <stdlib.h>

#include "ttv_common.h"
#include "ttv_kernels.h"

#define SWP_KB 64
#define SWP_NS 3
#ifndef SWP_OCC
#define SWP_OCC 3
#endif

typedef __attribute__((address_space(3))) bf16x4 swp_lds_bf16x4;
__device__ __forceinline__ bf16x4 swp_read_tr16(const char* lds_ptr) {
  return __builtin_amdgcn_ds_read_tr16_b64_v4bf16((swp_lds_bf16x4*)(lds_ptr));
}

#ifdef SWP_STAMPS
#define SWP_STAMP_DECL unsigned long long st_prev__ = 0, st_acc__[6] = {0, 0, 0, 0, 0, 0}
#define SWP_STAMP_START()                                                                              \
  do {                                                                                                 \
    __builtin_amdgcn_sched_barrier(0);                                                                 \
    asm volatile("s_memtime %0\n\ts_waitcnt lgkmcnt(0)" : "=s"(st_prev__)::"memory");                  \
    __builtin_amdgcn_sched_barrier(0);                                                                 \
  } while (0)
#define SWP_STAMP(seg_)                                                                                \
  do {                                                                                                 \
    unsigned long long t__;                                                                            \
    __builtin_amdgcn_sched_barrier(0);                                                                 \
    asm volatile("s_memtime %0\n\ts_waitcnt lgkmcnt(0)" : "=s"(t__)::"memory");                        \
    __builtin_amdgcn_sched_barrier(0);                                                                 \
    st_acc__[seg_] += t__ - st_prev__;                                                                 \
    st_prev__ = t__;                                                                                   \
  } while (0)
#else
#define SWP_STAMP_DECL
#define SWP_STAMP_START()
#define SWP_STAMP(seg_)
#endif

template <bool GATE>
__global__ __launch_bounds__(256, SWP_OCC) void k_attn_swp(const bf16_t* __restrict__ qkvg, int ld, bf16_t* __restrict__ out, int ldo,
                                                     const int* __restrict__ cu, const int* __restrict__ qblocks, int d_model, int gqa,
                                                     int rep, long long* __restrict__ stamps) {
  __shared__ __attribute__((aligned(16))) uint4 kl[SWP_NS][SWP_KB * 8];
  __shared__ __attribute__((aligned(16))) uint4 vl[SWP_NS][SWP_KB * 8];

#ifdef SWP_STAMPS
  unsigned long long st_entry__;
  asm volatile("s_memtime %0\n\ts_waitcnt lgkmcnt(0)" : "=s"(st_entry__)::"memory");
#endif
  const int tid = threadIdx.x, lane = tid & 63;
  const int wave = __builtin_amdgcn_readfirstlane(tid >> 6);
  const int r = lane & 31, h = lane >> 5;
  const int tix = blockIdx.x;
  const int seq = qblocks[4 * tix], q0 = qblocks[4 * tix + 1], head = qblocks[4 * tix + 2];
  if (seq < 0) return;
  const int s0 = cu[seq], S = cu[seq + 1] - s0;
  const int kvh = head / rep;
  const bf16_t* qbase = qkvg + (size_t)s0 * ld + head * 64;
  const bf16_t* gbase = qkvg + (size_t)s0 * ld + d_model + head * 64;
  const bf16_t* kbase = qkvg + (size_t)s0 * ld + 2 * d_model + kvh * 64;
  const bf16_t* vbase = kbase + gqa;
  const int nkt = (S + SWP_KB - 1) / SWP_KB;

  const uint32_t kl_lds = (uint32_t)(uintptr_t)(__attribute__((address_space(3))) void*)&kl[0][0];
  const uint32_t vl_lds = (uint32_t)(uintptr_t)(__attribute__((address_space(3))) void*)&vl[0][0];
  const int drow = wave * 8 + (lane >> 3);
  const int kc = ((lane & 7) ^ ((drow >> 1) & 7)) * 8;
  const int vc = ((lane & 7) ^ (((drow >> 1) & 1) << 2)) * 8;
  const uint32_t dK = (uint32_t)(drow * ld + kc) * 2u;
  const uint32_t dV = (uint32_t)(drow * ld + vc) * 2u;
#define SWP_DMA16(voff_, base_, dst_)                                                                            \
  do {                                                                                                           \
    unsigned keep__;                                                                                             \
    asm volatile("s_mov_b32 %0, m0\n\ts_mov_b32 m0, %3\n\ts_nop 0\n\tglobal_load_lds_dwordx4 %1, %2\n\ts_mov_b32 m0, %0" \
                 : "=&s"(keep__) : "v"(voff_), "s"(base_), "s"(dst_) : "memory");                                 \
  } while (0)
#define SWP_DMA_TILE(base_, lds_, kt_, slot_, d_, c_)                                                            \
  do {                                                                                                           \
    const int key0__ = (kt_) * SWP_KB;                                                                           \
    if (key0__ >= S) break;                                                                                      \
    const bf16_t* b__ = (base_) + (size_t)key0__ * ld;                                                           \
    const uint32_t dst__ = (lds_) + (slot_) * (SWP_KB * 128) + wave * 1024;                                      \
    if (key0__ + SWP_KB <= S) {                                                                                  \
      const bf16_t* b32__ = b__ + (size_t)32 * ld;                                                               \
      unsigned keep__;                                                                                           \
      asm volatile("s_mov_b32 %0, m0\n\ts_mov_b32 m0, %4\n\ts_nop 0\n\tglobal_load_lds_dwordx4 %1, %2\n\t"         \
                   "s_add_u32 m0, %4, 0x1000\n\ts_nop 0\n\tglobal_load_lds_dwordx4 %1, %3\n\ts_mov_b32 m0, %0"      \
                   : "=&s"(keep__) : "v"(d_), "s"(b__), "s"(b32__), "s"(dst__) : "memory", "scc");                   \
    } else {                                                                                                     \
      const int lim__ = S - 1 - key0__;                                                                          \
      const int g0__ = drow < lim__ ? drow : lim__, g1__ = drow + 32 < lim__ ? drow + 32 : lim__;                \
      SWP_DMA16((uint32_t)(g0__ * ld + (c_)) * 2u, b__, dst__);                                                  \
      SWP_DMA16((uint32_t)(g1__ * ld + (c_)) * 2u, b__, dst__ + 4096);                                           \
    }                                                                                                            \
  } while (0)
#define SWP_DMA_K(kt_, slot_) SWP_DMA_TILE(kbase, kl_lds, kt_, slot_, dK, kc)
#define SWP_DMA_V(kt_, slot_) SWP_DMA_TILE(vbase, vl_lds, kt_, slot_, dV, vc)

  SWP_DMA_K(0, 0);
  SWP_DMA_V(0, 0);
  SWP_DMA_K(1, 1);
  SWP_DMA_K(2, 2);
  SWP_DMA_V(1, 1);
  const int qrow = q0 + wave * 32 + r;
  const int qrc = qrow < S ? qrow : S - 1;
  bf16x8 qf[4];
#pragma unroll
  for (int ks = 0; ks < 4; ++ks) qf[ks] = *reinterpret_cast<const bf16x8*>(qbase + (size_t)qrc * ld + ks * 16 + h * 8);

  const int ksw = (r >> 1) & 7;
  const char* const kbase_lds = reinterpret_cast<const char*>(&kl[0][0]);
  const char* const vbase_lds = reinterpret_cast<const char*>(&vl[0][0]);
  const char* const ka0 = kbase_lds + r * 128 + (((0 * 2 + h) ^ ksw) << 4);
  const char* const ka1 = kbase_lds + r * 128 + (((1 * 2 + h) ^ ksw) << 4);
  const char* const ka2 = kbase_lds + r * 128 + (((2 * 2 + h) ^ ksw) << 4);
  const char* const ka3 = kbase_lds + r * 128 + (((3 * 2 + h) ^ ksw) << 4);
  const int gi = lane & 15, tq = gi >> 2, tp = gi & 3, g16 = (lane >> 4) & 1;
  const int vsw = (tq >> 1) & 1;
  const int vlane = (4 * h + tq) * 128 + (g16 * 2 + (tp >> 1)) * 16 + (tp & 1) * 8;
  const char* const va0 = vbase_lds + vlane + (vsw ? 64 : 0);
  const char* const va1 = vbase_lds + vlane + (vsw ? 0 : 64);
  const f32x16 zero16 = {0.f, 0.f, 0.f, 0.f, 0.f, 0.f, 0.f, 0.f, 0.f, 0.f, 0.f, 0.f, 0.f, 0.f, 0.f, 0.f};

  f32x16 o0 = zero16, o1 = zero16;
  float l_run = 0.f;
  f32x16 sA0, sA1, sB0, sB1;
  bf16x8 kf00, kf01, kf02, kf03, kf10, kf11, kf12, kf13;
  bf16x8 vf00, vf01, vf02, vf03, vf10, vf11, vf12, vf13;
  bf16x8 pa0, pa1, pa2, pa3, pb0, pb1, pb2, pb3;
  float sum_a, sum_b;

#define SWP_LOADK_H(J_, so_)                                                                                     \
  do {                                                                                                           \
    if ((J_) == 0) {                                                                                             \
      kf00 = *reinterpret_cast<const bf16x8*>(ka0 + (so_));                                                      \
      kf01 = *reinterpret_cast<const bf16x8*>(ka1 + (so_));                                                      \
      kf02 = *reinterpret_cast<const bf16x8*>(ka2 + (so_));                                                      \
      kf03 = *reinterpret_cast<const bf16x8*>(ka3 + (so_));                                                      \
    } else {                                                                                                     \
      kf10 = *reinterpret_cast<const bf16x8*>(ka0 + (so_) + 4096);                                               \
      kf11 = *reinterpret_cast<const bf16x8*>(ka1 + (so_) + 4096);                                               \
      kf12 = *reinterpret_cast<const bf16x8*>(ka2 + (so_) + 4096);                                               \
      kf13 = *reinterpret_cast<const bf16x8*>(ka3 + (so_) + 4096);                                               \
    }                                                                                                            \
  } while (0)
#define SWP_VFRAG(va_, OFF_)                                                                                     \
  ({                                                                                                             \
    const bf16x4 lo__ = swp_read_tr16((va_) + (OFF_)), hi__ = swp_read_tr16((va_) + (OFF_) + 1024);              \
    (bf16x8){lo__[0], lo__[1], lo__[2], lo__[3], hi__[0], hi__[1], hi__[2], hi__[3]};                            \
  })
#define SWP_LOADV_H(J_, so_)                                                                                     \
  do {                                                                                                           \
    if ((J_) == 0) {                                                                                             \
      vf00 = SWP_VFRAG(va0, (so_));        vf10 = SWP_VFRAG(va1, (so_));                                         \
      vf01 = SWP_VFRAG(va0, (so_) + 2048); vf11 = SWP_VFRAG(va1, (so_) + 2048);                                  \
    } else {                                                                                                     \
      vf02 = SWP_VFRAG(va0, (so_) + 4096); vf12 = SWP_VFRAG(va1, (so_) + 4096);                                  \
      vf03 = SWP_VFRAG(va0, (so_) + 6144); vf13 = SWP_VFRAG(va1, (so_) + 6144);                                  \
    }                                                                                                            \
  } while (0)
#define SWP_EXP8(s_, Q_, f_, FIRST_)                                                                             \
  do {                                                                                                           \
    float p__[8];                                                                                                \
    _Pragma("unroll") for (int e__ = 0; e__ < 8; ++e__) p__[e__] = __builtin_amdgcn_exp2f(s_[8 * (Q_) + e__]);   \
    if (FIRST_) { sum_a = p__[0]; sum_b = p__[1]; } else { sum_a += p__[0]; sum_b += p__[1]; }                   \
    _Pragma("unroll") for (int e__ = 2; e__ < 8; e__ += 2) { sum_a += p__[e__]; sum_b += p__[e__ + 1]; }         \
    f_ = (bf16x8){(bf16_t)p__[0], (bf16_t)p__[1], (bf16_t)p__[2], (bf16_t)p__[3], (bf16_t)p__[4], (bf16_t)p__[5],  \
                  (bf16_t)p__[6], (bf16_t)p__[7]};                                                               \
     \
    asm volatile("" : "+v"(f_), "+v"(sum_a), "+v"(sum_b));                                                       \
  } while (0)
#define SWP_MASK(c0_, c1_, kt_)                                                                                  \
  do {                                                                                                           \
    if ((kt_) == nkt - 1 && nkt * SWP_KB > S) {                                                                  \
      int h4__ = 4 * h;                                                                                          \
      asm volatile("" : "+v"(h4__));       \
      _Pragma("unroll") for (int e__ = 0; e__ < 16; ++e__) {                                                     \
        const int key__ = (kt_) * SWP_KB + (e__ & 3) + 8 * (e__ >> 2) + h4__;                                    \
        if (key__ >= S) c0_[e__] = -INFINITY;                                                                    \
        if (key__ + 32 >= S) c1_[e__] = -INFINITY;                                                               \
      }                                                                                                          \
    }                                                                                                            \
  } while (0)
#define SWP_SCORES_H(d_, k0_, k1_, k2_, k3_)                                                                     \
  do {                                                                                                           \
    d_ = __builtin_amdgcn_mfma_f32_32x32x16_bf16(k0_, qf[0], zero16, 0, 0, 0);                                   \
    d_ = __builtin_amdgcn_mfma_f32_32x32x16_bf16(k1_, qf[1], d_, 0, 0, 0);                                       \
    d_ = __builtin_amdgcn_mfma_f32_32x32x16_bf16(k2_, qf[2], d_, 0, 0, 0);                                       \
    d_ = __builtin_amdgcn_mfma_f32_32x32x16_bf16(k3_, qf[3], d_, 0, 0, 0);                                       \
  } while (0)
#define SWP_PV_H(va_, vb_, vc_, vd_, f0_, f1_)                                                                   \
  do {                                                                                                           \
    o0 = __builtin_amdgcn_mfma_f32_32x32x16_bf16(va_, f0_, o0, 0, 0, 0);                                         \
    o1 = __builtin_amdgcn_mfma_f32_32x32x16_bf16(vb_, f0_, o1, 0, 0, 0);                                         \
    o0 = __builtin_amdgcn_mfma_f32_32x32x16_bf16(vc_, f1_, o0, 0, 0, 0);                                         \
    o1 = __builtin_amdgcn_mfma_f32_32x32x16_bf16(vd_, f1_, o1, 0, 0, 0);                                         \
  } while (0)
#define SWP_GAPS4(NDS_)                                                                                          \
  do {                                                                                                           \
    _Pragma("unroll") for (int i__ = 0; i__ < 4; ++i__) {                                                        \
      __builtin_amdgcn_sched_group_barrier(0x008, 1, 0);                                                         \
      __builtin_amdgcn_sched_group_barrier(0x100, NDS_, 0);                                                      \
      __builtin_amdgcn_sched_group_barrier(0x400, 2, 0);                                                         \
      __builtin_amdgcn_sched_group_barrier(0x002, 3, 0);                                                         \
    }                                                                                                            \
    __builtin_amdgcn_sched_barrier(0);                                                                           \
  } while (0)

#define SWP_TOP(t_)                                                                                              \
  do {                                                                                                           \
    if ((t_) + 3 < nkt) asm volatile("s_waitcnt vmcnt(4) lgkmcnt(0)" ::: "memory");                              \
    else if ((t_) + 1 < nkt) asm volatile("s_waitcnt vmcnt(2) lgkmcnt(0)" ::: "memory");                         \
    else asm volatile("s_waitcnt vmcnt(0) lgkmcnt(0)" ::: "memory");                                             \
    SWP_STAMP(0);                                                                                                \
    asm volatile("s_barrier" ::: "memory");       \
    SWP_STAMP(1);                                                                                                \
  } while (0)

#define SWP_ITER(t_, so0_, so1_, so2_, cur1_, nxt0_, nxt1_, pc0_, pc1_, pc2_, pc3_, pn0_, pn1_)                  \
  do {                                                                                                           \
    const int tt__ = (t_);                                                                                       \
    SWP_TOP(tt__);                                                                                               \
          \
    SWP_LOADV_H(0, so0_);                                                                                        \
    SWP_SCORES_H(nxt0_, kf00, kf01, kf02, kf03);                                                                 \
    SWP_EXP8(cur1_, 0, pc2_, false);                                                                             \
    SWP_GAPS4(2);                                                                                                \
    SWP_DMA_V(tt__ + 2, (so2_) >> 13);                                                                           \
    __builtin_amdgcn_sched_barrier(0);                                                                           \
    SWP_LOADV_H(1, so0_);                                                                                        \
    SWP_SCORES_H(nxt1_, kf10, kf11, kf12, kf13);                                                                 \
    SWP_EXP8(cur1_, 1, pc3_, false);                                                                             \
    SWP_GAPS4(2);                                                                                                \
    SWP_STAMP(2);                                                                                                \
    l_run += sum_a + sum_b;                                                                                      \
    if (tt__ + 1 == nkt - 1 && nkt * SWP_KB > S) {                                                               \
      asm volatile("s_nop 7\n\ts_nop 7\n\ts_nop 3" ::: "memory");      \
      SWP_MASK(nxt0_, nxt1_, tt__ + 1);                                                                          \
    }                                                                                                            \
    SWP_STAMP(3);                                                                                                \
     \
    SWP_LOADK_H(0, so2_);                                                                                        \
    SWP_PV_H(vf00, vf10, vf01, vf11, pc0_, pc1_);                                                                \
    SWP_EXP8(nxt0_, 0, pn0_, true);                                                                              \
    SWP_GAPS4(1);                                                                                                \
    SWP_DMA_K(tt__ + 4, (so1_) >> 13);                                                                           \
    __builtin_amdgcn_sched_barrier(0);                                                                           \
    SWP_LOADK_H(1, so2_);                                                                                        \
    SWP_PV_H(vf02, vf12, vf03, vf13, pc2_, pc3_);                                                                \
    SWP_EXP8(nxt0_, 1, pn1_, false);                                                                             \
    SWP_GAPS4(1);                                                                                                \
    SWP_STAMP(4);                                                                                                \
  } while (0)

  __builtin_amdgcn_s_waitcnt(0x0F70);
  __syncthreads();
  SWP_LOADK_H(0, 0);
  SWP_LOADK_H(1, 0);
  SWP_SCORES_H(sA0, kf00, kf01, kf02, kf03);
  SWP_SCORES_H(sA1, kf10, kf11, kf12, kf13);
  SWP_MASK(sA0, sA1, 0);
  __syncthreads();
  SWP_DMA_K(3, 0);
  SWP_LOADK_H(0, SWP_KB * 128);
  SWP_LOADK_H(1, SWP_KB * 128);
  SWP_EXP8(sA0, 0, pa0, true);
  SWP_EXP8(sA0, 1, pa1, false);
  SWP_STAMP_DECL;
  SWP_STAMP_START();
#ifdef SWP_STAMPS
  const unsigned long long st_loop_start__ = st_prev__;
  unsigned long long st_real0__;
  asm volatile("s_memrealtime %0\n\ts_waitcnt lgkmcnt(0)" : "=s"(st_real0__)::"memory");
#endif

#define SWP_LAST(t_, so0_, cur1_, pc0_, pc1_, pc2_, pc3_)                                                        \
  do {                                                                                                           \
    SWP_TOP(t_);                                                                                                 \
    SWP_LOADV_H(0, so0_);                                                                                        \
    SWP_PV_H(vf00, vf10, vf01, vf11, pc0_, pc1_);                                                                \
    SWP_EXP8(cur1_, 0, pc2_, false);                                                                             \
    SWP_GAPS4(2);                                                                                                \
    SWP_LOADV_H(1, so0_);                                                                                        \
    SWP_EXP8(cur1_, 1, pc3_, false);                                                                             \
    __builtin_amdgcn_sched_barrier(0);                                                                           \
    SWP_STAMP(2);                                                                                                \
    l_run += sum_a + sum_b;                                                                                      \
    SWP_PV_H(vf02, vf12, vf03, vf13, pc2_, pc3_);                                                                \
    SWP_STAMP(4);                                                                                                \
  } while (0)

  {
    int t = 0;
    int so0 = 0, so1 = SWP_KB * 128, so2 = 2 * SWP_KB * 128;
    for (;;) {
      if (t == nkt - 1) break;
      SWP_ITER(t, so0, so1, so2, sA1, sB0, sB1, pa0, pa1, pa2, pa3, pb0, pb1);
      ++t;
      if (t == nkt - 1) {
        sA1 = sB1; pa0 = pb0; pa1 = pb1; so0 = so1;
        break;
      }
      SWP_ITER(t, so1, so2, so0, sB1, sA0, sA1, pb0, pb1, pb2, pb3, pa0, pa1);
      ++t;
      const int so = so0;
      so0 = so2;
      so2 = so1;
      so1 = so;
    }
    SWP_LAST(t, so0, sA1, pa0, pa1, pa2, pa3);
  }
#ifdef SWP_STAMPS
  const unsigned long long st_loop_end__ = st_prev__;
  unsigned long long st_real1__;
  asm volatile("s_memrealtime %0\n\ts_waitcnt lgkmcnt(0)" : "=s"(st_real1__)::"memory");
  st_acc__[5] = st_real1__ - st_real0__;
#endif

  float l_tot = l_run + __shfl_xor(l_run, 32, 64);
  const bool out_of_range = !(l_tot > 8.6736174e-19f && l_tot < 1.1529215e18f);
  if (__syncthreads_or(out_of_range)) {
    float m_run = -INFINITY;
    l_run = 0.f;
    o0 = zero16;
    o1 = zero16;
    for (int kt = 0; kt < nkt; ++kt) {
      __syncthreads();
      SWP_DMA_K(kt, 0);
      SWP_DMA_V(kt, 0);
      __builtin_amdgcn_s_waitcnt(0x0F70);
      __syncthreads();
      SWP_LOADK_H(0, 0);
      SWP_LOADK_H(1, 0);
      SWP_SCORES_H(sA0, kf00, kf01, kf02, kf03);
      SWP_SCORES_H(sA1, kf10, kf11, kf12, kf13);
      SWP_MASK(sA0, sA1, kt);
      float mx = fmaxf(sA0[0], sA1[0]);
#pragma unroll
      for (int e = 1; e < 16; ++e) mx = fmaxf(mx, fmaxf(sA0[e], sA1[e]));
      mx = fmaxf(mx, __shfl_xor(mx, 32, 64));
      const float m_new = fmaxf(m_run, mx);
      const float alpha = __builtin_amdgcn_exp2f(m_run - m_new);
      float ps = 0.f;
#pragma unroll
      for (int e = 0; e < 16; ++e) {
        sA0[e] = __builtin_amdgcn_exp2f(sA0[e] - m_new);
        sA1[e] = __builtin_amdgcn_exp2f(sA1[e] - m_new);
        ps += sA0[e] + sA1[e];
        o0[e] *= alpha;
        o1[e] *= alpha;
      }
      l_run = l_run * alpha + ps;
      m_run = m_new;
#define SWP_PACKS(c_, Q_)                                                                                         \
  ((bf16x8){(bf16_t)c_[8 * Q_ + 0], (bf16_t)c_[8 * Q_ + 1], (bf16_t)c_[8 * Q_ + 2], (bf16_t)c_[8 * Q_ + 3], (bf16_t)c_[8 * Q_ + 4], \
            (bf16_t)c_[8 * Q_ + 5], (bf16_t)c_[8 * Q_ + 6], (bf16_t)c_[8 * Q_ + 7]})
      pa0 = SWP_PACKS(sA0, 0); pa1 = SWP_PACKS(sA0, 1); pa2 = SWP_PACKS(sA1, 0); pa3 = SWP_PACKS(sA1, 1);
#undef SWP_PACKS
      SWP_LOADV_H(0, 0);
      SWP_LOADV_H(1, 0);
      SWP_PV_H(vf00, vf10, vf01, vf11, pa0, pa1);
      SWP_PV_H(vf02, vf12, vf03, vf13, pa2, pa3);
    }
    l_tot = l_run + __shfl_xor(l_run, 32, 64);
  }

  const float inv_l = __builtin_amdgcn_rcpf(l_tot);
  {
    bf16_t* orow = out + (size_t)(s0 + qrc) * ldo + head * 64;
    const bf16_t* grow = gbase + (size_t)qrc * ld;
    const bool store = qrow < S;
#pragma unroll
    for (int dt = 0; dt < 2; ++dt)
#pragma unroll
      for (int gp = 0; gp < 2; ++gp) {
        uint2 pk[2];
#pragma unroll
        for (int gg = 0; gg < 2; ++gg) {
          const int g = 2 * gp + gg;
          const int d0 = dt * 32 + 8 * g + 4 * h;
          const f32x16& oa = dt ? o1 : o0;
          f32x4 v = {oa[4 * g] * inv_l, oa[4 * g + 1] * inv_l, oa[4 * g + 2] * inv_l, oa[4 * g + 3] * inv_l};
          if (GATE) {
            const f32x4 gt = Vec4<bf16_t>::load(grow + d0);
#pragma unroll
            for (int e = 0; e < 4; ++e) v[e] *= __builtin_amdgcn_rcpf(1.0f + __builtin_amdgcn_exp2f(gt[e] * -1.44269504088896340736f));
          }
          const bf16x4 b4 = {(bf16_t)v[0], (bf16_t)v[1], (bf16_t)v[2], (bf16_t)v[3]};
          pk[gg] = __builtin_bit_cast(uint2, b4);
        }
        const auto sx = __builtin_amdgcn_permlane32_swap(pk[0].x, pk[1].x, false, false);
        const auto sy = __builtin_amdgcn_permlane32_swap(pk[0].y, pk[1].y, false, false);
        const uint4 o16 = {sx[0], sy[0], sx[1], sy[1]};
        if (store) *reinterpret_cast<uint4*>(orow + dt * 32 + 16 * gp + 8 * h) = o16;
      }
  }
#ifdef SWP_STAMPS
  if (stamps && blockIdx.x % 37 == 0 && lane == 0) {
    unsigned long long st_end__;
    asm volatile("s_waitcnt vmcnt(0)\n\ts_memtime %0\n\ts_waitcnt lgkmcnt(0)" : "=s"(st_end__)::"memory");
    long long* dst = stamps + ((size_t)(blockIdx.x / 37) * 4 + wave) * 8;
    for (int i = 0; i < 6; ++i) dst[i] = (long long)st_acc__[i];
    dst[6] = (long long)(st_loop_start__ - st_entry__);
    dst[7] = (long long)(st_end__ - st_loop_end__);
  }
#endif
}

int ttvk_attention_swp(const void* qkvg, int ld, void* out, int ldo, const int* cu_seqlens, const int* qblocks, int n_qblocks,
                       int q_heads, int kv_heads, int gate_mul, hipStream_t s) {
  const int d_model = q_heads * 64, gqa = kv_heads * 64, rep = q_heads / kv_heads;
  dim3 grid(n_qblocks);
  if (gate_mul)
    hipLaunchKernelGGL((k_attn_swp<true>), grid, dim3(256), 0, s, (const bf16_t*)qkvg, ld, (bf16_t*)out, ldo, cu_seqlens, qblocks, d_model,
                       gqa, rep, g_ttv_stamps);
  else
    hipLaunchKernelGGL((k_attn_swp<false>), grid, dim3(256), 0, s, (const bf16_t*)qkvg, ld, (bf16_t*)out, ldo, cu_seqlens, qblocks, d_model,
                       gqa, rep, g_ttv_stamps);
  TTV_CHECK_LAUNCH("attention_swp");
  return TTV_OK;
}
```

### titok_video_amd/csrc/ttv_elem.hip

```cpp
#include "ttv_common.h"
#include "ttv_kernels.h"

#define ROWS_PER_BLOCK 4
#define MAX_ITERS 4

__device__ __forceinline__ int mx_quant4(const f32x4 y, int& byte) {
  float a = fmaxf(fmaxf(fabsf(y[0]), fabsf(y[1])), fmaxf(fabsf(y[2]), fabsf(y[3])));
  a = fmaxf(a, __shfl_xor(a, 1));
  a = fmaxf(a, __shfl_xor(a, 2));
  a = fmaxf(a, __shfl_xor(a, 4));
  const uint32_t tb = __float_as_uint(a * (1.0f / 448.0f));
  byte = (int)((tb >> 23) & 0xFF) + ((tb & 0x7FFFFF) ? 1 : 0);
  byte = a > 0.f ? (byte < 1 ? 1 : (byte > 254 ? 254 : byte)) : 127;
  const float inv_blk = __uint_as_float((uint32_t)(254 - byte) << 23);
  int w = 0;
  w = __builtin_amdgcn_cvt_pk_fp8_f32(y[0] * inv_blk, y[1] * inv_blk, w, false);
  w = __builtin_amdgcn_cvt_pk_fp8_f32(y[2] * inv_blk, y[3] * inv_blk, w, true);
  return w;
}

template <typename TI, typename TO>
__global__ __launch_bounds__(256) void k_rmsnorm(const TI* __restrict__ in, int ld_in, const int* __restrict__ src_rows,
                                                 TO* __restrict__ out, int ld_out, const int* __restrict__ dst_rows,
                                                 const float* __restrict__ gain, int rows, int d, float eps,
// ... 238 lines not shown
    }
  }
}

int ttvk_quant_rows_fp8(const void* in, int in_dtype, int ld_in, const float* gain, float eps, void* out, int ld_out, float* scales, int rows,
                        int d, hipStream_t s) {
  if (rows == 0) return TTV_OK;
  TTV_CHECK_ARG(d % 4 == 0 && d <= 64 * 4 * MAX_ITERS, "quant_rows_fp8: width %d must be a multiple of 4 and <= 1024", d);
  TTV_CHECK_ARG(ld_in % 4 == 0 && ld_out % 4 == 0 && (uintptr_t)out % 4 == 0, "quant_rows_fp8: leading dims must be multiples of 4");
  dim3 grid(ttv_cdiv(rows, ROWS_PER_BLOCK));
  if (in_dtype == TTV_BF16) hipLaunchKernelGGL((k_quant_rows_fp8<bf16_t>), grid, dim3(256), 0, s, (const bf16_t*)in, ld_in, gain, eps, (uint8_t*)out, ld_out, scales, rows, d);
  else if (in_dtype == TTV_F32) hipLaunchKernelGGL((k_quant_rows_fp8<float>), grid, dim3(256), 0, s, (const float*)in, ld_in, gain, eps, (uint8_t*)out, ld_out, scales, rows, d);
  else { ttv_set_error("quant_rows_fp8: bad dtype"); return TTV_ERR_INVALID; }
  TTV_CHECK_LAUNCH("quant_rows_fp8");
  return TTV_OK;
}

__global__ __launch_bounds__(256) void k_split3_pack(const float* __restrict__ w, int ldw, uint4* __restrict__ out, int ldo4, int rows, int k4) {
  const long i = (long)blockIdx.x * 256 + threadIdx.x;
  if (i >= (long)rows * k4) return;
  const int r = (int)(i / k4), c = (int)(i % k4);
  const f32x4 v = *reinterpret_cast<const f32x4*>(w + (size_t)r * ldw + c * 4);
  bf16x4 hv, lv;
#pragma unroll
  for (int e = 0; e < 4; ++e) {
    hv[e] = (bf16_t)v[e];
    lv[e] = (bf16_t)(v[e] - (float)hv[e]);
  }
  const uint2 hp = __builtin_bit_cast(uint2, hv), lp = __builtin_bit_cast(uint2, lv);
  out[(size_t)r * ldo4 + c] = make_uint4(hp.x, hp.y, lp.x, lp.y);
}

int ttvk_split3_pack(const float* w, int ldw, void* out, int ldo, int rows, int K, hipStream_t s) {
  if (rows == 0) return TTV_OK;
  TTV_CHECK_ARG(K > 0 && K % 4 == 0 && ldw % 4 == 0 && ldo % 4 == 0 && (uintptr_t)w % 16 == 0 && (uintptr_t)out % 16 == 0, "split3_pack: K and leading dims must be multiples of 4, pointers 16-byte aligned");
  const long n = (long)rows * (K / 4);
  hipLaunchKernelGGL(k_split3_pack, dim3((unsigned)((n + 255) / 256)), dim3(256), 0, s, w, ldw, (uint4*)out, ldo / 4, rows, K / 4);
  TTV_CHECK_LAUNCH("split3_pack");
  return TTV_OK;
}

template <typename TI>
__global__ __launch_bounds__(256) void k_quant_mx_fp8(const TI* __restrict__ in, int ld_in, uint8_t* __restrict__ out, int ld_out,
                                                      uint8_t* __restrict__ mx, int ld_mx, int nkp, float* __restrict__ row_scales,
                                                      int rows, int d) {
  const int wave = threadIdx.x >> 6, lane = threadIdx.x & 63;
  const int r = blockIdx.x * ROWS_PER_BLOCK + wave;
  if (r >= rows) return;
  const TI* p = in + (size_t)r * ld_in;
  float inv_row = 1.0f;
  if (row_scales) {
    float amax = 0.f;
    for (int c = lane * 4; c < d; c += 256) {
      const f32x4 y = Vec4<TI>::load(p + c);
      amax = fmaxf(amax, fmaxf(fmaxf(fabsf(y[0]), fabsf(y[1])), fmaxf(fabsf(y[2]), fabsf(y[3]))));
    }
    amax = wave_max(amax);
    const float scale = amax > 0.f ? amax * (1.0f / 448.0f) : 1.0f;
    inv_row = 1.0f / scale;
    if (lane == 0) row_scales[r] = scale;
  }
  uint8_t* q = out + (size_t)r * ld_out;
  uint8_t* m = mx + (size_t)r * ld_mx;
  for (int c = lane * 4; c < d; c += 256) {
    const f32x4 y = Vec4<TI>::load(p + c) * inv_row;
    float a = fmaxf(fmaxf(fabsf(y[0]), fabsf(y[1])), fmaxf(fabsf(y[2]), fabsf(y[3])));
    a = fmaxf(a, __shfl_xor(a, 1));
    a = fmaxf(a, __shfl_xor(a, 2));
    a = fmaxf(a, __shfl_xor(a, 4));
    const uint32_t tb = __float_as_uint(a * (1.0f / 448.0f));
    int byte = (int)((tb >> 23) & 0xFF) + ((tb & 0x7FFFFF) ? 1 : 0);
    byte = a > 0.f ? (byte < 1 ? 1 : (byte > 254 ? 254 : byte)) : 127;
    const float inv_blk = __uint_as_float((uint32_t)(254 - byte) << 23);
    int w = 0;
    w = __builtin_amdgcn_cvt_pk_fp8_f32(y[0] * inv_blk, y[1] * inv_blk, w, false);
    w = __builtin_amdgcn_cvt_pk_fp8_f32(y[2] * inv_blk, y[3] * inv_blk, w, true);
    *reinterpret_cast<int*>(q + c) = w;
    if ((lane & 7) == 0) {
      const int b = c >> 5;
      m[(b & 3) * nkp + (b >> 2)] = (uint8_t)byte;
    }
  }
}

int64_t ttvk_mx_scale_ld(int d) { return 4 * (int64_t)((d / 128 + 3) / 4 * 4); }

int ttvk_quant_mx_fp8(const void* in, int in_dtype, int ld_in, void* out, int ld_out, void* mx, float* row_scales, int rows, int d, hipStream_t s) {
  if (rows == 0) return TTV_OK;
  TTV_CHECK_ARG(d > 0 && d % 128 == 0, "quant_mx_fp8: width %d must be a multiple of 128", d);
  TTV_CHECK_ARG(ld_in % 4 == 0 && ld_out % 4 == 0 && (uintptr_t)out % 4 == 0 && (uintptr_t)mx % 4 == 0, "quant_mx_fp8: alignment");
  const int nkp = (d / 128 + 3) / 4 * 4;
  dim3 grid(ttv_cdiv(rows, ROWS_PER_BLOCK));
  if (in_dtype == TTV_BF16) hipLaunchKernelGGL((k_quant_mx_fp8<bf16_t>), grid, dim3(256), 0, s, (const bf16_t*)in, ld_in, (uint8_t*)out, ld_out, (uint8_t*)mx, 4 * nkp, nkp, row_scales, rows, d);
  else if (in_dtype == TTV_F32) hipLaunchKernelGGL((k_quant_mx_fp8<float>), grid, dim3(256), 0, s, (const float*)in, ld_in, (uint8_t*)out, ld_out, (uint8_t*)mx, 4 * nkp, nkp, row_scales, rows, d);
  else { ttv_set_error("quant_mx_fp8: bad dtype"); return TTV_ERR_INVALID; }
  TTV_CHECK_LAUNCH("quant_mx_fp8");
  return TTV_OK;
}

template <typename T>
__global__ __launch_bounds__(256) void k_fill_const_rows(T* __restrict__ x, int ld, const int* __restrict__ rows_map, int rows,
                                                         int d, const float* __restrict__ mask_token,
                                                         const float* __restrict__ gain, float eps) {
  const int wave = threadIdx.x >> 6, lane = threadIdx.x & 63;
  const int r = blockIdx.x * ROWS_PER_BLOCK + wave;
  if (r >= rows) return;
  const float m = round_to<T>(mask_token[0]);
  const float rstd = 1.0f / sqrtf(m * m + eps);
  T* q = x + (size_t)rows_map[r] * ld;
  for (int c = lane * 4; c < d; c += 256) {
    const f32x4 g = *reinterpret_cast<const f32x4*>(gain + c);
    f32x4 o = {m * rstd * g[0], m * rstd * g[1], m * rstd * g[2], m * rstd * g[3]};
    Vec4<T>::store(q + c, o);
  }
}

int ttvk_fill_const_rows(void* x, int dtype, int ld, const int* rows_map, int rows, int d, const float* mask_token,
                         const float* gain, float eps, hipStream_t s) {
  if (rows == 0) return TTV_OK;
  TTV_CHECK_ARG(d % 4 == 0, "fill_const_rows: width %% 4");
  dim3 grid(ttv_cdiv(rows, ROWS_PER_BLOCK));
  if (dtype == TTV_BF16)
    hipLaunchKernelGGL((k_fill_const_rows<bf16_t>), grid, dim3(256), 0, s, (bf16_t*)x, ld, rows_map, rows, d, mask_token, gain, eps);
  else
    hipLaunchKernelGGL((k_fill_const_rows<float>), grid, dim3(256), 0, s, (float*)x, ld, rows_map, rows, d, mask_token, gain, eps);
  TTV_CHECK_LAUNCH("fill_const_rows");
  return TTV_OK;
}

template <typename T>
__global__ __launch_bounds__(256) void k_dec_embed(const T* __restrict__ codes, int C, const T* __restrict__ w ,
                                                   const T* __restrict__ bias, const float* __restrict__ mask_token,
                                                   const float* __restrict__ gain, T* __restrict__ x, int ld,
                                                   const int* __restrict__ rows_map, int rows, int d, float eps, T* __restrict__ hpre) {
  const int wave = threadIdx.x >> 6, lane = threadIdx.x & 63;
  const int r = blockIdx.x * ROWS_PER_BLOCK + wave;
  if (r >= rows) return;
  float cz[TTV_MAX_FSQ];
#pragma unroll
  for (int c = 0; c < TTV_MAX_FSQ; ++c) cz[c] = c < C ? Cvt<T>::to_f(codes[(size_t)r * C + c]) : 0.f;
  const T* crow = codes + (size_t)r * C;
  const float m = round_to<T>(mask_token[0]);
  float v[MAX_ITERS][4];
  float ss = 0.f;
#pragma unroll
  for (int it = 0; it < MAX_ITERS; ++it) {
#pragma unroll
    for (int e = 0; e < 4; ++e) {
      const int f = (it * 64 + lane) * 4 + e;
      float h = 0.f;
      if (f < d) {
        if (C <= TTV_MAX_FSQ) {
#pragma unroll
          for (int c = 0; c < TTV_MAX_FSQ; ++c)
            if (c < C) h += cz[c] * Cvt<T>::to_f(w[(size_t)f * C + c]);
        } else if ((C & 3) == 0) {
          const T* wrow = w + (size_t)f * C;
          for (int c = 0; c < C; c += 4) {
            const f32x4 cv = Vec4<T>::load(crow + c), wv = Vec4<T>::load(wrow + c);
            h += cv[0] * wv[0];
            h += cv[1] * wv[1];
            h += cv[2] * wv[2];
            h += cv[3] * wv[3];
          }
        } else {
          for (int c = 0; c < C; ++c) h += Cvt<T>::to_f(crow[c]) * Cvt<T>::to_f(w[(size_t)f * C + c]);
        }
        h = round_to<T>(h + Cvt<T>::to_f(bias[f]));
        h = round_to<T>(h + m);
      }
      v[it][e] = h;
      ss += h * h;
    }
    if (hpre && (it * 64 + lane) * 4 < d)
      Vec4<T>::store(hpre + (size_t)r * d + (it * 64 + lane) * 4, (f32x4){v[it][0], v[it][1], v[it][2], v[it][3]});
  }
  ss = wave_sum(ss);
  const float rstd = 1.0f / sqrtf(ss / (float)d + eps);
  T* q = x + (size_t)rows_map[r] * ld;
#pragma unroll
  for (int it = 0; it < MAX_ITERS; ++it) {
    const int c0 = (it * 64 + lane) * 4;
    if (c0 < d) {
      const f32x4 g = *reinterpret_cast<const f32x4*>(gain + c0);
      f32x4 o = {v[it][0] * rstd * g[0], v[it][1] * rstd * g[1], v[it][2] * rstd * g[2], v[it][3] * rstd * g[3]};
      Vec4<T>::store(q + c0, o);
    }
  }
}

int ttvk_dec_embed(const void* codes, int C, const void* w, const void* bias, const float* mask_token, const float* gain,
                   void* x, int dtype, int ld, const int* rows_map, int rows, int d, float eps, hipStream_t s) {
  return ttvk_dec_embed_ex(codes, C, w, bias, mask_token, gain, x, dtype, ld, rows_map, rows, d, eps, nullptr, s);
}

int ttvk_dec_embed_ex(const void* codes, int C, const void* w, const void* bias, const float* mask_token, const float* gain, void* x,
                      int dtype, int ld, const int* rows_map, int rows, int d, float eps, void* hpre, hipStream_t s) {
  if (rows == 0) return TTV_OK;
  TTV_CHECK_ARG(C >= 1 && C <= TTV_MAX_TOKEN, "dec_embed: token_size %d out of range", C);
  TTV_CHECK_ARG(d % 4 == 0 && d <= 1024, "dec_embed: width");
  dim3 grid(ttv_cdiv(rows, ROWS_PER_BLOCK));
  if (dtype == TTV_BF16)
    hipLaunchKernelGGL((k_dec_embed<bf16_t>), grid, dim3(256), 0, s, (const bf16_t*)codes, C, (const bf16_t*)w, (const bf16_t*)bias, mask_token, gain, (bf16_t*)x, ld, rows_map, rows, d, eps, (bf16_t*)hpre);
  else
    hipLaunchKernelGGL((k_dec_embed<float>), grid, dim3(256), 0, s, (const float*)codes, C, (const float*)w, (const float*)bias, mask_token, gain, (float*)x, ld, rows_map, rows, d, eps, (float*)hpre);
  TTV_CHECK_LAUNCH("dec_embed");
  return TTV_OK;
}

struct FsqDev {
  int n;
  float half_l[TTV_MAX_FSQ], offset[TTV_MAX_FSQ], shift[TTV_MAX_FSQ], half_width[TTV_MAX_FSQ], basis[TTV_MAX_FSQ];
  int levels[TTV_MAX_FSQ], ibasis[TTV_MAX_FSQ];
};

static FsqDev to_dev(const ttv_fsq_params* p) {
  FsqDev d;
  d.n = p->n;
  for (int i = 0; i < TTV_MAX_FSQ; ++i) {
    d.half_l[i] = p->half_l[i]; d.offset[i] = p->offset[i]; d.shift[i] = p->shift[i];
    d.half_width[i] = p->half_width[i]; d.basis[i] = (float)p->basis[i];
    d.levels[i] = p->levels[i]; d.ibasis[i] = p->basis[i];
  }
  return d;
}

__device__ __forceinline__ float fsq_channel(const FsqDev& p, int c, float z, float* bounded_out, float* code_out) {
  const float b = __fsub_rn(__fmul_rn(tanhf(__fadd_rn(z, p.shift[c])), p.half_l[c]), p.offset[c]);
  const float q = rintf(b);
  const float code = __fdiv_rn(q, p.half_width[c]);
  const float zhat = __fadd_rn(__fmul_rn(code, p.half_width[c]), p.half_width[c]);
  *bounded_out = b;
  *code_out = code;
  return __fmul_rn(zhat, p.basis[c]);
}

template <typename TZ, typename TC>
__global__ __launch_bounds__(256) void k_fsq_forward(FsqDev p, const TZ* __restrict__ z, int rows, TC* __restrict__ codes,
                                                     int* __restrict__ indices, float* __restrict__ bounded) {
  const int r = blockIdx.x * 256 + threadIdx.x;
  if (r >= rows) return;
  float acc = 0.f;
  for (int c = 0; c < p.n; ++c) {
    float b, code;
    acc = __fadd_rn(acc, fsq_channel(p, c, Cvt<TZ>::to_f(z[(size_t)r * p.n + c]), &b, &code));
    codes[(size_t)r * p.n + c] = Cvt<TC>::from_f(code);
    if (bounded) bounded[(size_t)r * p.n + c] = b;
  }
  indices[r] = (int)acc;
}

int ttvk_fsq_forward(const ttv_fsq_params* p, const void* z, int z_dtype, int rows, void* codes, int codes_dtype, int* indices,
                     float* bounded, hipStream_t s) {
  TTV_CHECK_ARG(p && p->n >= 1 && p->n <= TTV_MAX_FSQ, "fsq: codebook_dim out of range");
  if (rows == 0) return TTV_OK;
  FsqDev d = to_dev(p);
  dim3 grid(ttv_cdiv(rows, 256));
  if (z_dtype == TTV_F32 && codes_dtype == TTV_F32)
    hipLaunchKernelGGL((k_fsq_forward<float, float>), grid, dim3(256), 0, s, d, (const float*)z, rows, (float*)codes, indices, bounded);
  else if (z_dtype == TTV_F32 && codes_dtype == TTV_BF16)
    hipLaunchKernelGGL((k_fsq_forward<float, bf16_t>), grid, dim3(256), 0, s, d, (const float*)z, rows, (bf16_t*)codes, indices, bounded);
  else if (z_dtype == TTV_BF16 && codes_dtype == TTV_BF16)
    hipLaunchKernelGGL((k_fsq_forward<bf16_t, bf16_t>), grid, dim3(256), 0, s, d, (const bf16_t*)z, rows, (bf16_t*)codes, indices, bounded);
  else if (z_dtype == TTV_BF16 && codes_dtype == TTV_F32)
    hipLaunchKernelGGL((k_fsq_forward<bf16_t, float>), grid, dim3(256), 0, s, d, (const bf16_t*)z, rows, (float*)codes, indices, bounded);
  else { ttv_set_error("fsq: bad dtypes"); return TTV_ERR_INVALID; }
  TTV_CHECK_LAUNCH("fsq_forward");
  return TTV_OK;
}

template <typename TC>
__global__ __launch_bounds__(256) void k_fsq_indices_to_codes(FsqDev p, const int* __restrict__ indices, int rows,
                                                              TC* __restrict__ codes) {
  const int r = blockIdx.x * 256 + threadIdx.x;
  if (r >= rows) return;
  const int idx = indices[r];
  for (int c = 0; c < p.n; ++c) {
    const int lvl = (idx / p.ibasis[c]) % p.levels[c];
    const float hw = p.half_width[c];
    codes[(size_t)r * p.n + c] = Cvt<TC>::from_f(__fdiv_rn(__fsub_rn((float)lvl, hw), hw));
  }
}

int ttvk_fsq_indices_to_codes(const ttv_fsq_params* p, const int* indices, int rows, void* codes, int codes_dtype, hipStream_t s) {
  TTV_CHECK_ARG(p && p->n >= 1 && p->n <= TTV_MAX_FSQ, "fsq: codebook_dim out of range");
  if (rows == 0) return TTV_OK;
  FsqDev d = to_dev(p);
  dim3 grid(ttv_cdiv(rows, 256));
  if (codes_dtype == TTV_F32) hipLaunchKernelGGL((k_fsq_indices_to_codes<float>), grid, dim3(256), 0, s, d, indices, rows, (float*)codes);
  else hipLaunchKernelGGL((k_fsq_indices_to_codes<bf16_t>), grid, dim3(256), 0, s, d, indices, rows, (bf16_t*)codes);
  TTV_CHECK_LAUNCH("fsq_indices_to_codes");
  return TTV_OK;
}

template <typename T>
__global__ __launch_bounds__(256) void k_enc_tail(const T* __restrict__ x, int ld, const int* __restrict__ rows_map, int rows,
                                                  int d, const float* __restrict__ gain, float eps,
                                                  const T* __restrict__ w , const T* __restrict__ bias, int C,
                                                  FsqDev p, int have_fsq, float* __restrict__ z_out, T* __restrict__ codes,
                                                  int* __restrict__ indices, float* __restrict__ bounded) {
  const int wave = threadIdx.x >> 6, lane = threadIdx.x & 63;
  const int r = blockIdx.x * ROWS_PER_BLOCK + wave;
  if (r >= rows) return;
  const T* px = x + (size_t)rows_map[r] * ld;
  f32x4 v[MAX_ITERS];
  float ss = 0.f;
#pragma unroll
  for (int it = 0; it < MAX_ITERS; ++it) {
    const int c = (it * 64 + lane) * 4;
    if (c < d) {
      v[it] = Vec4<T>::load(px + c);
      ss += v[it][0] * v[it][0] + v[it][1] * v[it][1] + v[it][2] * v[it][2] + v[it][3] * v[it][3];
    } else {
      v[it] = (f32x4){0.f, 0.f, 0.f, 0.f};
    }
  }
  ss = wave_sum(ss);
  const float rstd = 1.0f / sqrtf(ss / (float)d + eps);
#pragma unroll
  for (int it = 0; it < MAX_ITERS; ++it) {
    const int c = (it * 64 + lane) * 4;
    if (c < d) {
      const f32x4 g = *reinterpret_cast<const f32x4*>(gain + c);
#pragma unroll
      for (int e = 0; e < 4; ++e) v[it][e] = round_to<T>(v[it][e] * rstd * g[e]);
    }
  }
  float zc[TTV_MAX_FSQ];
#pragma unroll
  for (int c = 0; c < TTV_MAX_FSQ; ++c) zc[c] = 0.f;
  for (int c = 0; c < C; ++c) {
    float acc = 0.f;
#pragma unroll
    for (int it = 0; it < MAX_ITERS; ++it) {
      const int f = (it * 64 + lane) * 4;
      if (f < d) {
        const f32x4 wv = Vec4<T>::load(w + (size_t)c * d + f);
        acc += v[it][0] * wv[0] + v[it][1] * wv[1] + v[it][2] * wv[2] + v[it][3] * wv[3];
      }
    }
    const float zv = wave_sum(acc) + Cvt<T>::to_f(bias[c]);
    if (lane == 0 && z_out) z_out[(size_t)r * C + c] = zv;
    if (have_fsq) {
#pragma unroll
      for (int k = 0; k < TTV_MAX_FSQ; ++k)
        if (k == c) zc[k] = zv;
    }
  }
  if (lane == 0 && have_fsq) {
    float idx = 0.f;
    for (int c = 0; c < C; ++c) {
      {
        float b, code;
        idx = __fadd_rn(idx, fsq_channel(p, c, zc[c], &b, &code));
        codes[(size_t)r * C + c] = Cvt<T>::from_f(code);
        if (bounded) bounded[(size_t)r * C + c] = b;
      }
    }
    if (have_fsq) indices[r] = (int)idx;
  }
}

int ttvk_enc_tail(const void* x, int dtype, int ld, const int* rows_map, int rows, int d, const float* gain, float eps,
                  const void* w, const void* bias, int C, const ttv_fsq_params* fsq, float* z_out, void* codes, int* indices,
                  float* bounded, hipStream_t s) {
  if (rows == 0) return TTV_OK;
  TTV_CHECK_ARG(C >= 1 && C <= (fsq ? TTV_MAX_FSQ : TTV_MAX_TOKEN), "enc_tail: token_size %d out of range", C);
  TTV_CHECK_ARG(d % 4 == 0 && d <= 1024, "enc_tail: width");
  TTV_CHECK_ARG(!fsq || fsq->n == C, "enc_tail: fsq dim != token_size");
  FsqDev p;
  if (fsq) p = to_dev(fsq); else { p = FsqDev(); p.n = 0; }
  dim3 grid(ttv_cdiv(rows, ROWS_PER_BLOCK));
  if (dtype == TTV_BF16)
    hipLaunchKernelGGL((k_enc_tail<bf16_t>), grid, dim3(256), 0, s, (const bf16_t*)x, ld, rows_map, rows, d, gain, eps, (const bf16_t*)w, (const bf16_t*)bias, C, p, fsq ? 1 : 0, z_out, (bf16_t*)codes, indices, bounded);
  else
    hipLaunchKernelGGL((k_enc_tail<float>), grid, dim3(256), 0, s, (const float*)x, ld, rows_map, rows, d, gain, eps, (const float*)w, (const float*)bias, C, p, fsq ? 1 : 0, z_out, (float*)codes, indices, bounded);
  TTV_CHECK_LAUNCH("enc_tail");
  return TTV_OK;
}


template <typename T, bool SCATTER>
__global__ __launch_bounds__(256) void k_patch_copy(ClipPtrs clips, const int* __restrict__ clip_desc, int clip0, int pt, int ph,
                                                    int pw, int C, T* __restrict__ patches, int ld) {
  const int* ds = clip_desc + (size_t)(clip0 + blockIdx.y) * 8;
  const int Tn = ds[0], H = ds[1], W = ds[2], gh = ds[4], gw = ds[5], base = ds[6];
  const int P = ds[3] * gh * gw;
  const int nseg = C * pt * ph;
  const int total = P * nseg;
  T* clip = reinterpret_cast<T*>(clips.p[blockIdx.y]);
  for (int idx = blockIdx.x * 256 + threadIdx.x; idx < total; idx += gridDim.x * 256) {
    const int p = idx / nseg, sg = idx - p * nseg;
    const int c = sg / (pt * ph), ipt = (sg / ph) % pt, iph = sg % ph;
    const int gwi = p % gw, ghi = (p / gw) % gh, gti = p / (gw * gh);
    T* src = clip + (((size_t)c * Tn + gti * pt + ipt) * H + ghi * ph + iph) * W + gwi * pw;
    T* dst = patches + (size_t)(base + p) * ld + sg * pw;
    if ((pw * sizeof(T)) % 16 == 0) {
      for (int e = 0; e < (int)(pw * sizeof(T) / 16); ++e) {
        if (SCATTER) reinterpret_cast<uint4*>(src)[e] = reinterpret_cast<const uint4*>(dst)[e];
        else reinterpret_cast<uint4*>(dst)[e] = reinterpret_cast<const uint4*>(src)[e];
      }
    } else {
      for (int e = 0; e < pw; ++e) {
        if (SCATTER) src[e] = dst[e]; else dst[e] = src[e];
      }
    }
  }
}

int ttvk_patch_copy(bool scatter, void* const* clips, const int* clip_desc, int clip0, int n_clips, int pt, int ph, int pw,
                    int C, void* patches, int ld, int dtype, int max_patches, hipStream_t s) {
  TTV_CHECK_ARG(n_clips >= 0 && n_clips <= TTV_MAX_CLIPS_PER_LAUNCH, "patch_copy: at most %d clips per call", TTV_MAX_CLIPS_PER_LAUNCH);
  if (n_clips == 0 || max_patches == 0) return TTV_OK;
  ClipPtrs cp;
  for (int i = 0; i < n_clips; ++i) cp.p[i] = clips[i];
  TtvProfScope prof(TTV_KC_PATCH, s);
  const int total = max_patches * C * pt * ph;
  dim3 grid(ttv_cdiv(total, 256) > 4096 ? 4096 : ttv_cdiv(total, 256), n_clips);
  if (dtype == TTV_BF16) {
    if (scatter) hipLaunchKernelGGL((k_patch_copy<bf16_t, true>), grid, dim3(256), 0, s, cp, clip_desc, clip0, pt, ph, pw, C, (bf16_t*)patches, ld);
    else hipLaunchKernelGGL((k_patch_copy<bf16_t, false>), grid, dim3(256), 0, s, cp, clip_desc, clip0, pt, ph, pw, C, (bf16_t*)patches, ld);
  } else {
    if (scatter) hipLaunchKernelGGL((k_patch_copy<float, true>), grid, dim3(256), 0, s, cp, clip_desc, clip0, pt, ph, pw, C, (float*)patches, ld);
    else hipLaunchKernelGGL((k_patch_copy<float, false>), grid, dim3(256), 0, s, cp, clip_desc, clip0, pt, ph, pw, C, (float*)patches, ld);
  }
  TTV_CHECK_LAUNCH("patch_copy");
  return TTV_OK;
}

template <typename T>
__global__ __launch_bounds__(256) void k_rope_apply(T* __restrict__ x, int ld, int rows, int heads,
                                                    const float* __restrict__ cs, float sgn) {
  const long total = (long)rows * heads * 16;
  for (long i = (long)blockIdx.x * 256 + threadIdx.x; i < total; i += (long)gridDim.x * 256) {
    const int q4 = (int)(i % 16), h = (int)((i / 16) % heads);
    const long r = i / (16 * heads);
    T* p = x + r * ld + h * 64 + q4 * 4;
    const float* c = cs + r * 64 + q4 * 2;
    f32x4 v = Vec4<T>::load(p);
    const float c0 = c[0], c1 = c[1], s0 = sgn * c[32], s1 = sgn * c[33];
    f32x4 o = {v[0] * c0 - v[1] * s0, v[0] * s0 + v[1] * c0, v[2] * c1 - v[3] * s1, v[2] * s1 + v[3] * c1};
    Vec4<T>::store(p, o);
  }
}

int ttvk_rope_apply(void* x, int dtype, int ld, int rows, int heads, const float* cs, hipStream_t s) {
  return ttvk_rope_apply_dir(x, dtype, ld, rows, heads, cs, 0, s);
}

int ttvk_rope_apply_dir(void* x, int dtype, int ld, int rows, int heads, const float* cs, int conj, hipStream_t s) {
  if (rows == 0) return TTV_OK;
  const float sgn = conj ? -1.f : 1.f;
  const long total = (long)rows * heads * 16;
  int blocks = (int)((total + 255) / 256);
  if (blocks > 8192) blocks = 8192;
  if (dtype == TTV_BF16) hipLaunchKernelGGL((k_rope_apply<bf16_t>), dim3(blocks), dim3(256), 0, s, (bf16_t*)x, ld, rows, heads, cs, sgn);
  else hipLaunchKernelGGL((k_rope_apply<float>), dim3(blocks), dim3(256), 0, s, (float*)x, ld, rows, heads, cs, sgn);
  TTV_CHECK_LAUNCH("rope_apply");
  return TTV_OK;
}

__global__ __launch_bounds__(256) void k_histogram(const int* __restrict__ idx, int n, unsigned long long* __restrict__ counts,
                                                   int size) {
  for (int i = blockIdx.x * 256 + threadIdx.x; i < n; i += gridDim.x * 256) {
    const int v = idx[i];
    if (v >= 0 && v < size) atomicAdd(&counts[v], 1ULL);
  }
}

int ttvk_histogram(const int* idx, int n, int64_t* counts, int size, hipStream_t s) {
  if (n == 0) return TTV_OK;
  int blocks = ttv_cdiv(n, 256);
  if (blocks > 1024) blocks = 1024;
  hipLaunchKernelGGL(k_histogram, dim3(blocks), dim3(256), 0, s, idx, n, (unsigned long long*)counts, size);
  TTV_CHECK_LAUNCH("histogram");
  return TTV_OK;
}

template <typename T>
__global__ __launch_bounds__(256) void k_const_rows_bwd(const float* __restrict__ colsum, const float* __restrict__ mask_token,
                                                        const float* __restrict__ gain, float eps, float* __restrict__ dgain,
                                                        float* __restrict__ dmask, int d) {
  __shared__ float red[4];
  const float m = round_to<T>(mask_token[0]);
  const float rstd = 1.0f / sqrtf(m * m + eps);
  float acc = 0.f;
  for (int f = threadIdx.x; f < d; f += 256) {
    atomicAdd(dgain + f, colsum[f] * m * rstd);
    acc += colsum[f] * gain[f];
  }
  acc = wave_sum(acc);
  if ((threadIdx.x & 63) == 0) red[threadIdx.x >> 6] = acc;
  __syncthreads();
  if (threadIdx.x == 0) atomicAdd(dmask, (red[0] + red[1] + red[2] + red[3]) * eps * rstd * rstd * rstd);
}

int ttvk_const_rows_bwd(const float* colsum, const float* mask_token, const float* gain, int dt, float eps, float* dgain, float* dmask,
                        int d, hipStream_t s) {
  if (!dgain && !dmask) return TTV_OK;
  if (dt == TTV_BF16) hipLaunchKernelGGL((k_const_rows_bwd<bf16_t>), dim3(1), dim3(256), 0, s, colsum, mask_token, gain, eps, dgain, dmask, d);
  else hipLaunchKernelGGL((k_const_rows_bwd<float>), dim3(1), dim3(256), 0, s, colsum, mask_token, gain, eps, dgain, dmask, d);
  TTV_CHECK_LAUNCH("const_rows_bwd");
  return TTV_OK;
}

__global__ __launch_bounds__(256) void k_rope_build(const float* __restrict__ base_cos, const float* __restrict__ base_sin, int n_ids,
                                                    int F, const int* __restrict__ clip_desc, const int* __restrict__ cu,
                                                    const int* __restrict__ row_seq, float* __restrict__ out, int total_rows) {
  const int i = blockIdx.x * 256 + threadIdx.x;
  if (i >= total_rows * 32) return;
  const int row = i >> 5, j = i & 31;
  const int b = row_seq[row];
  const int* ds = clip_desc + b * 8;
  const int gh = ds[4], gw = ds[5];
  const int P = ds[3] * gh * gw, S = cu[b + 1] - cu[b], K = S - P;
  const int local = row - cu[b];
  float c = 1.f, sn = 0.f;
  if (j < 3 * F) {
    const int f = j / 3, axis = j - 3 * f;
    int id;
    if (local < K) id = local;
    else {
      const int p = local - K;
      const int w = p % gw, h = (p / gw) % gh, t = p / (gw * gh);
      id = (axis == 0 ? t : axis == 1 ? h : w) + K;
    }
    id = id < n_ids ? id : n_ids - 1;
    c = base_cos[id * F + f];
    sn = base_sin[id * F + f];
  }
  out[(size_t)row * 64 + j] = c;
  out[(size_t)row * 64 + 32 + j] = sn;
}

int ttvk_rope_build(const float* base_cos, const float* base_sin, int n_ids, int F, const int* clip_desc, const int* cu, const int* row_seq,
                    float* out, int total_rows, hipStream_t s) {
  if (total_rows == 0) return TTV_OK;
  hipLaunchKernelGGL(k_rope_build, dim3(ttv_cdiv(total_rows * 32, 256)), dim3(256), 0, s, base_cos, base_sin, n_ids, F, clip_desc, cu, row_seq, out, total_rows);
  TTV_CHECK_LAUNCH("rope_build");
  return TTV_OK;
}


template <typename T>
__global__ __launch_bounds__(256) void k_clip_from_u8(const uint8_t* __restrict__ frames, T* __restrict__ clip, long long n_pix) {
  const long long q = (long long)blockIdx.x * 256 + threadIdx.x;
  const long long p0 = q * 4;
  if (p0 >= n_pix) return;
  if (p0 + 4 <= n_pix) {
    const uint32_t* src = reinterpret_cast<const uint32_t*>(frames + p0 * 3);
    const uint32_t w0 = src[0], w1 = src[1], w2 = src[2];
    const uint8_t b[12] = {(uint8_t)w0, (uint8_t)(w0 >> 8), (uint8_t)(w0 >> 16), (uint8_t)(w0 >> 24), (uint8_t)w1, (uint8_t)(w1 >> 8),
                           (uint8_t)(w1 >> 16), (uint8_t)(w1 >> 24), (uint8_t)w2, (uint8_t)(w2 >> 8), (uint8_t)(w2 >> 16), (uint8_t)(w2 >> 24)};
#pragma unroll
    for (int c = 0; c < 3; ++c) {
      f32x4 v;
#pragma unroll
      for (int i = 0; i < 4; ++i) v[i] = __fsub_rn(__fdiv_rn((float)b[3 * i + c], 127.5f), 1.0f);
      Vec4<T>::store(clip + (size_t)c * n_pix + p0, v);
    }
  } else {
    for (long long p = p0; p < n_pix; ++p)
      for (int c = 0; c < 3; ++c) clip[(size_t)c * n_pix + p] = Cvt<T>::from_f(__fsub_rn(__fdiv_rn((float)frames[p * 3 + c], 127.5f), 1.0f));
  }
}

int ttvk_clip_from_u8(const void* frames, long long n_pix, void* clip, int dtype, hipStream_t s) {
  if (n_pix == 0) return TTV_OK;
  TTV_CHECK_ARG((uintptr_t)frames % 4 == 0 && (uintptr_t)clip % 16 == 0 && n_pix % 4 == 0, "clip_from_u8: frames 4-byte, clip 16-byte aligned, T*H*W %% 4 == 0");
  const long long groups = (n_pix + 3) / 4;
  dim3 grid((unsigned)((groups + 255) / 256));
  if (dtype == TTV_BF16) hipLaunchKernelGGL((k_clip_from_u8<bf16_t>), grid, dim3(256), 0, s, (const uint8_t*)frames, (bf16_t*)clip, n_pix);
  else if (dtype == TTV_F32) hipLaunchKernelGGL((k_clip_from_u8<float>), grid, dim3(256), 0, s, (const uint8_t*)frames, (float*)clip, n_pix);
  else { ttv_set_error("clip_from_u8: bad dtype"); return TTV_ERR_INVALID; }
  TTV_CHECK_LAUNCH("clip_from_u8");
  return TTV_OK;
}
```

### titok_video_amd/csrc/ttv_kernels.h

```cpp
#pragma once
#include <hip/hip_runtime.h>
#include <stdint.h>

#include "../../include/titok_hip.h"

int ttvk_rmsnorm(const void* in, int in_dtype, int ld_in, const int* src_rows, void* out, int out_dtype, int ld_out,
                 const int* dst_rows, const float* gain, int rows, int d, float eps, hipStream_t s, float* next_rstd = nullptr,
                 void* mx_q = nullptr, void* mx_s = nullptr,
                 int split_image = 0);
int ttvk_row_rstd(const void* in, int dtype, int ld_in, float* rstd, int rows, int d, float eps, hipStream_t s);
int ttvk_copy_rows(const void* src, int64_t ld_src_bytes, const int* src_rows, void* dst, int64_t ld_dst_bytes, const int* dst_rows, int rows,
                   int row_bytes, hipStream_t s);
int ttvk_fill_const_rows(void* x, int dtype, int ld, const int* rows_map, int rows, int d, const float* mask_token,
                         const float* gain, float eps, hipStream_t s);
int ttvk_dec_embed(const void* codes, int C, const void* w, const void* bias, const float* mask_token, const float* gain,
                   void* x, int dtype, int ld, const int* rows_map, int rows, int d, float eps, hipStream_t s);
int ttvk_fsq_forward(const ttv_fsq_params* p, const void* z, int z_dtype, int rows, void* codes, int codes_dtype, int* indices,
                     float* bounded, hipStream_t s);
int ttvk_fsq_indices_to_codes(const ttv_fsq_params* p, const int* indices, int rows, void* codes, int codes_dtype, hipStream_t s);
int ttvk_enc_tail(const void* x, int dtype, int ld, const int* rows_map, int rows, int d, const float* gain, float eps,
                  const void* w, const void* bias, int C, const ttv_fsq_params* fsq, float* z_out, void* codes, int* indices,
                  float* bounded, hipStream_t s);
int ttvk_patch_copy(bool scatter, void* const* clips, const int* clip_desc, int clip0, int n_clips, int pt, int ph, int pw,
                    int C, void* patches, int ld, int dtype, int max_patches, hipStream_t s);
int ttvk_rope_apply(void* x, int dtype, int ld, int rows, int heads, const float* cs, hipStream_t s);
int ttvk_histogram(const int* idx, int n, int64_t* counts, int size, hipStream_t s);
int ttvk_quant_rows_fp8(const void* in, int in_dtype, int ld_in, const float* gain, float eps, void* out, int ld_out, float* scales, int rows,
                        int d, hipStream_t s);

int ttvk_split3_pack(const float* w, int ldw, void* out, int ldo, int rows, int K, hipStream_t s);
int64_t ttvk_mx_scale_ld(int d);
int ttvk_quant_mx_fp8(const void* in, int in_dtype, int ld_in, void* out, int ld_out, void* mx, float* row_scales, int rows, int d, hipStream_t s);

int ttvk_clip_from_u8(const void* frames, long long n_pix, void* clip, int dtype, hipStream_t s);

enum GemmEpilogue {
  EPI_STORE = 0,
  EPI_QKV_ROPE,
  EPI_GEGLU,
  EPI_RESID_T,
  EPI_RESID_F32,
  EPI_RESID_NORM,
  EPI_STORE_PATCH,
};

struct GemmArgs {
  const void* x; int ldx;
  const void* w; int ldw;
  int M, N, K;
  void* y; int ldy;
  const void* bias;
  const float* add_scalar;
  const void* resid; int ldr;
  float alpha;
  const float* rope_cs;
  const int* rope_ids; const float* rope_base;
  int rope_q_end, rope_k_begin, rope_k_end;
  int dtype;
  const float* norm_gain;
  float* sum_f32; int ld_sum;
  void* y2; int ldy2; const float* norm_gain2;
  void* yq; void* yq_mx;
  int split3;
  int x_image, y_image;
  int prenorm;
  const float* row_scale;
  const int* x_rows;
  float eps;
  int gather;
  void* const* clips;
  int n_clips;
  const int* clip_desc;
  const int* patch_rows;
  const int* row_seq;
  int patch_t, patch_h, patch_w;
};
struct ClipPtrs { void* p[TTV_MAX_CLIPS_PER_LAUNCH]; };
int ttvk_gemm(GemmEpilogue epi, const GemmArgs& a, hipStream_t s);
int ttvk_gemm_fp8(GemmEpilogue epi, const GemmArgs& a, const float* x_scale, const float* w_scale, hipStream_t s, const void* x_mx = nullptr,
                  const void* w_mx = nullptr);
bool ttvk_gemm_supports_resid_norm(int dtype, int N, int K);

int ttvk_attention(const void* qkvg, int ld, void* out, int ldo, const int* cu_seqlens, const int* qblocks, int n_qblocks,
                   int q_heads, int kv_heads, int head_dim, int flags, int dtype, hipStream_t s, float* lse_out = nullptr,
                   void* out_raw = nullptr);

int ttvk_attention_swp(const void* qkvg, int ld, void* out, int ldo, const int* cu_seqlens, const int* qblocks, int n_qblocks,
                       int q_heads, int kv_heads, int gate_mul, hipStream_t s);
int ttvk_attention_mxout(const void* qkvg, int ld, void* out_q, void* out_mx, int ld_mx, const int* cu_seqlens, const int* qblocks,
                         int n_qblocks, int q_heads, int kv_heads, hipStream_t s);

int ttvk_attention64(const void* qkvg, int ld, void* out, int ldo, const int* cu_seqlens, const int* items, int n_items, int q_heads,
                     int kv_heads, int flags, hipStream_t s);

int ttvk_vq_norms(const void* cb, int dtype, int ld, int N, int C, float* cnorm, hipStream_t s);
int64_t ttvk_vq_workspace_bytes(int rows);
int ttvk_vq_l2_argmin(const void* z, int dtype, int ldz, const void* cb, int ldc, const float* cnorm, int rows, int N, int C, int* indices,
                      float* best_dist, void* workspace, int64_t workspace_bytes, hipStream_t s);
int ttvk_vq_lookup(const void* cb, int dtype, int ldc, const int* indices, int rows, int C, void* codes, int ldo, hipStream_t s);
int ttvk_vq_lookup_bwd(const void* dcodes, int dtype, int ld, const int* indices, int rows, int C, float* dcb, int ldc, hipStream_t s);

bool ttvk_mlp_fused_supported(int dtype, int width, int inner);
struct MlpNextQkv {
  void* qkv; int ld;
  const float* rope_cs;
  int rows;
  int rope_q_end, rope_k_begin, rope_k_end;
};
int64_t ttvk_mlp_pack_bytes(int inner, int next_qkv_rows);
int ttvk_mlp_pack(const void* w12_folded, const void* w3, const void* wo, const void* next_qkv_folded, int next_qkv_rows, int inner,
                  void* packed, hipStream_t s);
int ttvk_mlp_fused(const void* ao, int ldao, const float* front_gain, float front_alpha, const void* x, int ldx, const void* packed,
                   int inner, void* y, int ldy, const float* post_gain, float alpha, float eps, int M, const MlpNextQkv* nq, hipStream_t s);

int ttvk_l1_loss(void* const* recon, void* const* target, void* const* grad, const int* sizes, int n_clips, int total_clips, int dtype,
                 float* loss, hipStream_t s);
int ttvk_sq_err(void* const* recon, void* const* target, const int* sizes, int n_clips, int dtype, int clamp, double* acc2, hipStream_t s);
int ttvk_rmsnorm_bwd_chain(const void* x, int ldx, const void* dy, int lddy, const float* gain1, float* dgain1, float* dx, int lddx,
                           const void* y, int y_dt, int ldy, const float* gain2, float* dgain2, float out_scale, void* cast_out, int ldc, int rows,
                           int d, float eps, int dt, hipStream_t s);
int ttvk_rmsnorm_bwd(const void* x, int x_dt, int ldx, const int* xr, const void* dy, int dy_dt, int lddy, const int* dyr,
                     const float* gain, void* dx, int dx_dt, int lddx, const int* dxr, int acc, float* dgain, int rows, int d, float eps,
                     hipStream_t s);
int ttvk_colsum(const void* a, int dt, int lda, const int* rows_map, int rows, int n, float* out, hipStream_t s);
int ttvk_sumall(const void* a, int dt, int lda, const int* rows_map, int rows, int n, const float* colw, float scale, float* out, hipStream_t s);
int ttvk_gate_fwd(const void* a, int lda, const void* gate, int ldg, void* ag, int ldo, int rows, int d, int dt, hipStream_t s);
int ttvk_gate_bwd(const void* dag, int ldd, const void* a, int lda, const void* gate, int ldg, void* da, int ldda, void* dgate, int lddg,
                  int rows, int d, int dt, float* delta, hipStream_t s);
int ttvk_geglu_fwd(const void* u, int ldu, void* h, int ldh, int rows, int I, int dt, hipStream_t s);
int ttvk_geglu_bwd(const void* u, int ldu, const void* dh, int lddh, void* du, int lddu, int rows, int I, int dt, hipStream_t s);
int ttvk_scale_cast(const float* a, float alpha, float* b, void* c, int dt, long n, hipStream_t s);
int ttvk_to_f32(const void* a, int dt, float* b, long n, int accumulate, hipStream_t s);
int ttvk_fsq_bwd(const ttv_fsq_params* fp, const float* z, const void* dcodes, int dt, float* dz, int rows, hipStream_t s);
#define TTV_WGRAD_BATCH 6
struct WgradBatch {
  int n = 0;
  int64_t used_bytes = 0;
  struct Entry { const float* part; float* dw; int splits, lddw, N, K, tiles_n, tiles; } e[TTV_WGRAD_BATCH];
};
int ttvk_wgrad(const void* dy, int lddy, const void* x, int ldx, float* dw, int lddw, int L, int N, int K, int dt, float* part,
               int64_t part_bytes, hipStream_t s, WgradBatch* batch = nullptr);
int ttvk_wgrad_flush(WgradBatch* batch, hipStream_t s);
int64_t ttvk_wgrad_ws_bytes(int L, int N, int K);
int ttvk_outer_small(const void* a, int a_dt, int lda, int C, const void* b, int b_dt, int ldb, const int* b_rows, float* dw, int lddw,
                     int transpose_out, int rows, int d, hipStream_t s);
int ttvk_expand_small(const void* a, int a_dt, int lda, int C, const void* w, int w_dt, int ldw, int w_cf, void* out, int o_dt, int ldo,
                      int rows, int d, hipStream_t s);
int ttvk_reduce_small(const void* a, int a_dt, int lda, const int* a_rows, const void* w, int w_dt, int ldw, int C, float* out, int ldo,
                      int rows, int d, hipStream_t s);
int ttvk_attention_bwd(const void* qkvg, int ld, const void* o, int ldo, const void* dout, int ldd, const float* lse, float* delta,
                       const int* cu, const int* blocks64, int n_blocks64, const int* row_seq, void* dqkvg, int ldg, float* dkv_scratch,
                       int total_rows, int hq, int hkv, int dt, const float* rope_cs, hipStream_t s, int delta_ready = 0, const int* qlim_desc = nullptr);
int ttvk_rope_apply_dir(void* x, int dtype, int ld, int rows, int heads, const float* cs, int conj, hipStream_t s);
int ttvk_dec_embed_ex(const void* codes, int C, const void* w, const void* bias, const float* mask_token, const float* gain, void* x,
                      int dtype, int ld, const int* rows_map, int rows, int d, float eps, void* hpre, hipStream_t s);
int ttvk_const_rows_bwd(const float* colsum, const float* mask_token, const float* gain, int dt, float eps, float* dgain, float* dmask,
                        int d, hipStream_t s);
int ttvk_rope_build(const float* base_cos, const float* base_sin, int n_ids, int F, const int* clip_desc, const int* cu, const int* row_seq,
                    float* out, int total_rows, hipStream_t s);
```

### titok_video_amd/csrc/ttv_mlp.hip

```cpp
#include "ttv_common.h"
#include "ttv_kernels.h"

#define MLP_W12_CHUNKS 2048
#define MLP_W3_CHUNKS 1024
#define MLP_PANEL_CHUNKS (MLP_W12_CHUNKS + MLP_W3_CHUNKS)
#define MLP_WO_CHUNKS (4 * MLP_W12_CHUNKS)

struct MlpDev {
  const bf16_t* x; int ldx;
  const uint4* pack;
  const bf16_t* ao; int ldao;
  const float* front_gain;
  float front_alpha;
  bf16_t* qkv; int ldq;
  const float* rope_cs;
  int nqp, rope_q_end, rope_k_begin, rope_k_end;
  int I;
  bf16_t* y; int ldy;
  const float* post_gain;
  float alpha, eps;
  int M, n_tiles, debug;
  long long* stamps;
};

__global__ void k_mlp_pack(const bf16_t* __restrict__ w12f, const bf16_t* __restrict__ w3, const bf16_t* __restrict__ wo,
                           const bf16_t* __restrict__ wq, int nq_rows, int I, uint4* __restrict__ out) {
  const int np = I / 32;
  const int nqp = (nq_rows + 63) / 64;
  const int o = blockIdx.x * blockDim.x + threadIdx.x;
  if (o >= np * MLP_PANEL_CHUNKS + MLP_WO_CHUNKS + nqp * MLP_W12_CHUNKS) return;
  if (o >= np * MLP_PANEL_CHUNKS + MLP_WO_CHUNKS) {
    const int c = o - np * MLP_PANEL_CHUNKS - MLP_WO_CHUNKS, qp = c / MLP_W12_CHUNKS, cc = c - qp * MLP_W12_CHUNKS;
    const int r = cc >> 5, cp = cc & 31;
    const int ch = (cp & 16) | ((cp & 15) ^ (r & 15));
    int srow = qp * 64 + r;
    srow = srow < nq_rows ? srow : nq_rows - 1;
    const bf16_t* src = wq + (size_t)srow * 256 + (ch >> 2) * 32 + (ch & 3) * 4;
    const uint2 lo = *reinterpret_cast<const uint2*>(src), hi = *reinterpret_cast<const uint2*>(src + 16);
    out[o] = make_uint4(lo.x, lo.y, hi.x, hi.y);
    return;
  }
  if (o >= np * MLP_PANEL_CHUNKS) {
    const int c = o - np * MLP_PANEL_CHUNKS, wp = c / MLP_W12_CHUNKS, cc = c - wp * MLP_W12_CHUNKS;
    const int r = cc >> 5, cp = cc & 31;
    const int ch = (cp & 16) | ((cp & 15) ^ (r & 15));
    out[o] = wo ? *reinterpret_cast<const uint4*>(wo + (size_t)(wp * 64 + r) * 256 + ch * 8) : make_uint4(0, 0, 0, 0);
    return;
  }
  const int pn = o / MLP_PANEL_CHUNKS, c = o - pn * MLP_PANEL_CHUNKS;
  if (c < MLP_W12_CHUNKS) {
    const int r = c >> 5, cp = c & 31;
    const int ch = (cp & 16) | ((cp & 15) ^ (r & 15));
    const int srow = r < 32 ? pn * 32 + r : I + pn * 32 + (r - 32);
    const bf16_t* src = w12f + (size_t)srow * 256 + (ch >> 2) * 32 + (ch & 3) * 4;
    const uint2 lo = *reinterpret_cast<const uint2*>(src), hi = *reinterpret_cast<const uint2*>(src + 16);
    out[o] = make_uint4(lo.x, lo.y, hi.x, hi.y);
  } else {
    const int c3 = c - MLP_W12_CHUNKS, kq = c3 >> 8, row = c3 & 255;
    bf16x8 v;
#pragma unroll
    for (int j = 0; j < 8; ++j) v[j] = w3[(size_t)row * I + pn * 32 + (j < 4 ? 4 * kq + j : 16 + 4 * kq + (j - 4))];
    out[o] = __builtin_bit_cast(uint4, v);
  }
}

typedef uint32_t u32x2_t __attribute__((ext_vector_type(2)));
typedef uint32_t u32x4_t __attribute__((ext_vector_type(4)));
__device__ __forceinline__ f32x4 cvt4(bf16x4 b) { return (f32x4){(float)b[0], (float)b[1], (float)b[2], (float)b[3]}; }
#define MLP_LD12(img_, t_, s8_)                                                                                    \
  __builtin_bit_cast(bf16x8, (img_)[((t_) * 16 + l15) * 32 + ((((s8_) * 4 + kq) & 16) | ((((s8_) * 4 + kq) & 15) ^ l15))])
#define MLP_GLDS_4(src_, dst_)                                                                                     \
  do {                                                                                                             \
    unsigned keep__;                                                                                               \
    asm volatile("s_mov_b32 %0, m0\n\t"                                                                            \
                 "s_mov_b32 m0, %6\n\ts_nop 0\n\tglobal_load_lds_dwordx4 %1, %5\n\t"                               \
                 "s_add_u32 m0, %6, 0x2000\n\ts_nop 0\n\tglobal_load_lds_dwordx4 %2, %5\n\t"                       \
                 "s_add_u32 m0, %6, 0x4000\n\ts_nop 0\n\tglobal_load_lds_dwordx4 %3, %5\n\t"                       \
                 "s_add_u32 m0, %6, 0x6000\n\ts_nop 0\n\tglobal_load_lds_dwordx4 %4, %5\n\t"                       \
                 "s_mov_b32 m0, %0"                                                                                \
                 : "=&s"(keep__)                                                                                   \
                 : "v"(lane16), "v"(lane16 + 8192u), "v"(lane16 + 16384u), "v"(lane16 + 24576u), "s"(src_), "s"(dst_) \
                 : "memory", "scc");                                                                               \
  } while (0)
#define MLP_GLDS_2(src_, dst_)                                                                                     \
  do {                                                                                                             \
    unsigned keep__;                                                                                               \
    asm volatile("s_mov_b32 %0, m0\n\t"                                                                            \
                 "s_mov_b32 m0, %4\n\ts_nop 0\n\tglobal_load_lds_dwordx4 %1, %3\n\t"                               \
                 "s_add_u32 m0, %4, 0x2000\n\ts_nop 0\n\tglobal_load_lds_dwordx4 %2, %3\n\t"                       \
                 "s_mov_b32 m0, %0"                                                                                \
                 : "=&s"(keep__)                                                                                   \
                 : "v"(lane16), "v"(lane16 + 8192u), "s"(src_), "s"(dst_)                                          \
                 : "memory", "scc");                                                                               \
  } while (0)
#ifdef MLP_STAMPS
#define MLP_STAMP()                                                                                                \
  do {                                                                                                             \
    if (p.stamps && blockIdx.x == 0 && (wave & 3) == 0 && lane == 0 && n_stamp < 64)                               \
      p.stamps[(wave >> 2) * 64 + n_stamp++] = (long long)__builtin_readcyclecounter();                            \
  } while (0)
#else
#define MLP_STAMP() do { (void)n_stamp; } while (0)
#endif

template <int TPB, int T1, int T2, bool GELU_FIRST, bool KEEL, bool FRONT, bool BACK>
__device__ __forceinline__ void mlp_wave(const MlpDev& p, uint4* l12, uint4* l3, uint4* hb, const float* gl, int tile, int wave, int lane,
                                         int P1F, int P2F, int& n_stamp) {
  constexpr int T1A = T1 > 0 ? T1 : 1, T2A = T2 > 0 ? T2 : 1;
  const int l15 = lane & 15, kq = lane >> 4;
  const int np = p.I / 32;
  const uint32_t lane16 = lane * 16;
  const uint32_t lds_l12 = (uint32_t)(uintptr_t)(__attribute__((address_space(3))) void*)l12;
  const uint32_t lds_l3 = (uint32_t)(uintptr_t)(__attribute__((address_space(3))) void*)l3;
#define GLDS_W12(pn_, buf_)                                                                                        \
  do {                                                                                                             \
    const uint4* src__ = p.pack + ((size_t)(pn_) * MLP_PANEL_CHUNKS + wave * 64);                                  \
    const uint32_t dst__ = lds_l12 + ((buf_) * MLP_W12_CHUNKS + wave * 64) * 16;                                   \
    MLP_GLDS_4(src__, dst__);                                                                                      \
  } while (0)
#define GLDS_W3(pn_, buf_)                                                                                         \
  do {                                                                                                             \
    const uint4* src__ = p.pack + ((size_t)(pn_) * MLP_PANEL_CHUNKS + MLP_W12_CHUNKS + wave * 64);                 \
    const uint32_t dst__ = lds_l3 + ((buf_) * MLP_W3_CHUNKS + wave * 64) * 16;                                     \
    MLP_GLDS_2(src__, dst__);                                                                                      \
  } while (0)

  const int tok0 = tile * (16 * TPB) + l15;
  typedef __attribute__((address_space(1))) char gchar;
  typedef __attribute__((address_space(1))) const char gcchar;
  gcchar* const gx = (gcchar*)p.x;
  gcchar* const gao = (gcchar*)p.ao;
  gchar* const gy = (gchar*)p.y;

  MLP_STAMP();
  __syncthreads();

  bf16x8 bfr[T1A][8];
  float rstd[T1A];
  if (FRONT) {
#define GLDS_WO(wp_, buf_)                                                                                         \
  do {                                                                                                             \
    const uint4* src__ = p.pack + ((size_t)np * MLP_PANEL_CHUNKS + (wp_) * MLP_W12_CHUNKS + wave * 64);            \
    const uint32_t dst__ = lds_l12 + ((buf_) * MLP_W12_CHUNKS + wave * 64) * 16;                                   \
    MLP_GLDS_4(src__, dst__);                                                                                      \
  } while (0)
    GLDS_WO(0, 0);
    bf16x8 abf[T1A][8];
#pragma unroll
    for (int j = 0; j < T1; ++j) {
      const int t = tok0 + 16 * (P1F + j);
      const int tc = t < p.M ? t : p.M - 1;
      const uint32_t aoff = ((uint32_t)tc * (uint32_t)p.ldao + kq * 8) * 2u;
#pragma unroll
      for (int s8 = 0; s8 < 8; ++s8) abf[j][s8] = *(const __attribute__((address_space(1))) bf16x8*)(gao + aoff + s8 * 64);
    }
    f32x4 facc[16][T1A];
    __builtin_amdgcn_s_waitcnt(0x0F70);
    __syncthreads();
#pragma unroll
    for (int wp = 0; wp < 4; ++wp) {
      if (wp + 1 < 4) GLDS_WO(wp + 1, (wp + 1) & 1);
      const uint4* img = l12 + (wp & 1) * MLP_W12_CHUNKS;
      bf16x8 a[2][4];
      if constexpr (T1 > 0) {
#pragma unroll
      for (int i = 0; i < 4; ++i) a[0][i] = MLP_LD12(img, i, 0);
#pragma unroll
      for (int s8 = 0; s8 < 8; ++s8) {
        if (s8 + 1 < 8) {
#pragma unroll
          for (int i = 0; i < 4; ++i) a[(s8 + 1) & 1][i] = MLP_LD12(img, i, s8 + 1);
        }
#pragma unroll
        for (int i = 0; i < 4; ++i)
#pragma unroll
          for (int j = 0; j < T1; ++j)
            facc[4 * wp + i][j] = __builtin_amdgcn_mfma_f32_16x16x32_bf16(a[s8 & 1][i], abf[j][s8],
                                                                           s8 ? facc[4 * wp + i][j] : (f32x4){0.f, 0.f, 0.f, 0.f}, 0, 0, 0);
        if (s8 + 1 < 8) __builtin_amdgcn_sched_group_barrier(0x100, 4, 0);
        __builtin_amdgcn_sched_group_barrier(0x008, 4 * T1A, 0);
        __builtin_amdgcn_sched_barrier(0);
      }
      }
      __builtin_amdgcn_s_waitcnt(0x0F70);
      __syncthreads();
    }
#undef GLDS_WO
    GLDS_W12(0, 0);
#pragma unroll
    for (int j = 0; j < T1; ++j) {
      const int t = tok0 + 16 * (P1F + j);
      const int tc = t < p.M ? t : p.M - 1;
      const uint32_t roff = ((uint32_t)tc * (uint32_t)p.ldx + kq * 4) * 2u;
      float ss = 0.f;
#pragma unroll
      for (int m = 0; m < 16; ++m) {
        facc[m][j] += p.front_alpha * cvt4(*(const __attribute__((address_space(1))) bf16x4*)(gx + roff + m * 32));
#pragma unroll
        for (int e = 0; e < 4; ++e) ss = fmaf(facc[m][j][e], facc[m][j][e], ss);
      }
      float scale = 1.0f;
      if (p.front_gain) {
        ss = quad16_sum(ss);
        scale = 1.0f / sqrtf(ss * (1.0f / 256.0f) + p.eps);
      }
      float ss2 = 0.f;
#pragma unroll
      for (int s8 = 0; s8 < 8; ++s8) {
        bf16x4 q[2];
#pragma unroll
        for (int u = 0; u < 2; ++u) {
          const int m = 2 * s8 + u;
          f32x4 v = facc[m][j];
          if (p.front_gain) {
            const f32x4 g = *reinterpret_cast<const f32x4*>(gl + 256 + m * 16 + kq * 4);
#pragma unroll
            for (int e = 0; e < 4; ++e) v[e] = v[e] * scale * g[e];
          }
          q[u] = (bf16x4){(bf16_t)v[0], (bf16_t)v[1], (bf16_t)v[2], (bf16_t)v[3]};
#pragma unroll
          for (int e = 0; e < 4; ++e) {
            const float r = (float)q[u][e];
            ss2 = fmaf(r, r, ss2);
          }
        }
        bfr[j][s8] = (bf16x8){q[0][0], q[0][1], q[0][2], q[0][3], q[1][0], q[1][1], q[1][2], q[1][3]};
      }
      ss2 = quad16_sum(ss2);
      rstd[j] = 1.0f / sqrtf(ss2 * (1.0f / 256.0f) + p.eps);
    }
  } else {
    GLDS_W12(0, 0);
#pragma unroll
    for (int j = 0; j < T1; ++j) {
      const int t = tok0 + 16 * (P1F + j);
      const int tc = t < p.M ? t : p.M - 1;
      const uint32_t xoff = ((uint32_t)tc * (uint32_t)p.ldx + kq * 4) * 2u;
#pragma unroll
      for (int s8 = 0; s8 < 8; ++s8) {
        const u32x2_t lo = *(const __attribute__((address_space(1))) u32x2_t*)(gx + xoff + s8 * 64);
        const u32x2_t hi = *(const __attribute__((address_space(1))) u32x2_t*)(gx + xoff + (s8 * 64 + 32));
        bfr[j][s8] = __builtin_bit_cast(bf16x8, (u32x4_t){lo.x, lo.y, hi.x, hi.y});
      }
    }
#pragma unroll
    for (int j = 0; j < T1; ++j) {
      float ss = 0.f;
#pragma unroll
      for (int s8 = 0; s8 < 8; ++s8)
#pragma unroll
        for (int e = 0; e < 8; ++e) {
          const float v = (float)bfr[j][s8][e];
          ss = fmaf(v, v, ss);
        }
      ss = quad16_sum(ss);
      rstd[j] = 1.0f / sqrtf(ss * (1.0f / 256.0f) + p.eps);
    }
  }
  f32x4 out[16][T2A];
#pragma unroll
  for (int m = 0; m < 16; ++m)
#pragma unroll
    for (int j = 0; j < T2; ++j) out[m][j] = (f32x4){0.f, 0.f, 0.f, 0.f};

  __builtin_amdgcn_s_waitcnt(0x0F70);
  __syncthreads();
  MLP_STAMP();

  for (int it = 0; it <= np; ++it) {
    if (it + 1 < np && !(p.debug & 2)) GLDS_W12(it + 1, (it + 1) & 1);
    if (it < np && (!(p.debug & 2) || it == 0)) GLDS_W3(it, it & 1);

    f32x4 acc1[4][T1A];
    if (T1 > 0 && it < np) {
      const uint4* img = l12 + (it & 1) * MLP_W12_CHUNKS;
      bf16x8 a[2][4];
#pragma unroll
      for (int i = 0; i < 4; ++i) a[0][i] = MLP_LD12(img, i, 0);
#pragma unroll
      for (int s8 = 0; s8 < 8; ++s8) {
        if (s8 + 1 < 8) {
#pragma unroll
          for (int i = 0; i < 4; ++i) a[(s8 + 1) & 1][i] = MLP_LD12(img, i, s8 + 1);
        }
#pragma unroll
        for (int i = 0; i < 4; ++i)
#pragma unroll
          for (int j = 0; j < T1; ++j)
            acc1[i][j] = __builtin_amdgcn_mfma_f32_16x16x32_bf16(a[s8 & 1][i], bfr[j][s8],
                                                                  s8 ? acc1[i][j] : (f32x4){0.f, 0.f, 0.f, 0.f}, 0, 0, 0);
        if (s8 + 1 < 8) __builtin_amdgcn_sched_group_barrier(0x100, 4, 0);
        __builtin_amdgcn_sched_group_barrier(0x008, 4 * T1A, 0);
        __builtin_amdgcn_sched_barrier(0);
      }
    }
    if (!GELU_FIRST) {
      if (T2 > 0 && it >= 1 && !(p.debug & 16)) {
        const int pn = it - 1;
        const uint4* w3l = l3 + (pn & 1) * MLP_W3_CHUNKS + kq * 256 + l15;
        const uint4* hsrc = hb + ((pn & 1) * TPB + P2F) * 64 + lane;
        bf16x8 hf[T2A];
  #pragma unroll
        for (int j = 0; j < T2; ++j) hf[j] = __builtin_bit_cast(bf16x8, hsrc[j * 64]);
        bf16x8 w3f[4];
  #pragma unroll
        for (int r = 0; r < 4; ++r) w3f[r] = __builtin_bit_cast(bf16x8, w3l[r * 16]);
  #pragma unroll
        for (int m = 0; m < 16; ++m) {
  #pragma unroll
          for (int j = 0; j < T2; ++j) out[m][j] = __builtin_amdgcn_mfma_f32_16x16x32_bf16(w3f[m & 3], hf[j], out[m][j], 0, 0, 0);
          if (m + 4 < 16) w3f[m & 3] = __builtin_bit_cast(bf16x8, w3l[(m + 4) * 16]);
          __builtin_amdgcn_sched_group_barrier(0x008, T2A, 0);
          if (m + 4 < 16) __builtin_amdgcn_sched_group_barrier(0x100, 1, 0);
          __builtin_amdgcn_sched_barrier(0);
        }
      }
    }
    if (T1 > 0 && it < np) {
      uint4* hdst = hb + ((it & 1) * TPB + P1F) * 64 + lane;
#pragma unroll
      for (int j = 0; j < T1; ++j) {
        float gg[8], xx[8], hh[8];
#pragma unroll
        for (int i = 0; i < 2; ++i)
#pragma unroll
          for (int e = 0; e < 4; ++e) {
            gg[4 * i + e] = acc1[2 + i][j][e] * rstd[j];
            xx[4 * i + e] = acc1[i][j][e] * rstd[j];
          }
        if (p.debug & 4) {
#pragma unroll
          for (int k = 0; k < 8; ++k) hh[k] = gg[k] + xx[k];
        } else {
          geglu_fast8(gg, xx, hh);
        }
        uint32_t hw[4];
        typedef bf16_t bf16x2_t __attribute__((ext_vector_type(2)));
#pragma unroll
        for (int k = 0; k < 4; ++k) {
          const bf16x2_t q = {(bf16_t)hh[2 * k], (bf16_t)hh[2 * k + 1]};
          hw[k] = __builtin_bit_cast(uint32_t, q);
        }
        hdst[j * 64] = make_uint4(hw[0], hw[1], hw[2], hw[3]);
      }
    }
    if (GELU_FIRST) {
      if (T2 > 0 && it >= 1 && !(p.debug & 16)) {
        const int pn = it - 1;
        const uint4* w3l = l3 + (pn & 1) * MLP_W3_CHUNKS + kq * 256 + l15;
        const uint4* hsrc = hb + ((pn & 1) * TPB + P2F) * 64 + lane;
        bf16x8 hf[T2A];
  #pragma unroll
        for (int j = 0; j < T2; ++j) hf[j] = __builtin_bit_cast(bf16x8, hsrc[j * 64]);
        bf16x8 w3f[4];
  #pragma unroll
        for (int r = 0; r < 4; ++r) w3f[r] = __builtin_bit_cast(bf16x8, w3l[r * 16]);
  #pragma unroll
        for (int m = 0; m < 16; ++m) {
  #pragma unroll
          for (int j = 0; j < T2; ++j) out[m][j] = __builtin_amdgcn_mfma_f32_16x16x32_bf16(w3f[m & 3], hf[j], out[m][j], 0, 0, 0);
          if (m + 4 < 16) w3f[m & 3] = __builtin_bit_cast(bf16x8, w3l[(m + 4) * 16]);
          __builtin_amdgcn_sched_group_barrier(0x008, T2A, 0);
          if (m + 4 < 16) __builtin_amdgcn_sched_group_barrier(0x100, 1, 0);
          __builtin_amdgcn_sched_barrier(0);
        }
      }
    }
    if (it >= 4 && it < 8) MLP_STAMP();
    __builtin_amdgcn_s_waitcnt(0x0F70);
    __syncthreads();
    if (it >= 4 && it < 8) MLP_STAMP();
  }
  MLP_STAMP();

  uint4* const xres = l12;
  if (FRONT) {
#pragma unroll
    for (int j = 0; j < T1; ++j)
#pragma unroll
      for (int s8 = 0; s8 < 8; ++s8) xres[((P1F + j) * 8 + s8) * 64 + lane] = __builtin_bit_cast(uint4, bfr[j][s8]);
    __syncthreads();
  }

  bf16x8 xq[T2A][8];
  float rstdq[T2A];
#pragma unroll
  for (int j = 0; j < T2; ++j) {
    const int t = tok0 + 16 * (P2F + j);
    const bool tv = t < p.M;
    const int tc = tv ? t : p.M - 1;
    const uint32_t roff = ((uint32_t)tc * (uint32_t)p.ldx + kq * 4) * 2u;
    float ss = 0.f;
#pragma unroll
    for (int s8 = 0; s8 < 8; ++s8) {
      f32x4 rv0, rv1;
      if (FRONT) {
        const bf16x8 rb = __builtin_bit_cast(bf16x8, xres[((P2F + j) * 8 + s8) * 64 + lane]);
        rv0 = (f32x4){(float)rb[0], (float)rb[1], (float)rb[2], (float)rb[3]};
        rv1 = (f32x4){(float)rb[4], (float)rb[5], (float)rb[6], (float)rb[7]};
      } else {
        rv0 = cvt4(*(const __attribute__((address_space(1))) bf16x4*)(gx + roff + (2 * s8) * 32));
        rv1 = cvt4(*(const __attribute__((address_space(1))) bf16x4*)(gx + roff + (2 * s8 + 1) * 32));
      }
      out[2 * s8][j] += p.alpha * rv0;
      out[2 * s8 + 1][j] += p.alpha * rv1;
#pragma unroll
      for (int e = 0; e < 4; ++e) {
        ss = fmaf(out[2 * s8][j][e], out[2 * s8][j][e], ss);
        ss = fmaf(out[2 * s8 + 1][j][e], out[2 * s8 + 1][j][e], ss);
      }
    }
    float scale = 1.0f;
    if (KEEL) {
      ss = quad16_sum(ss);
      scale = 1.0f / sqrtf(ss * (1.0f / 256.0f) + p.eps);
    }
    const bool odd = kq & 1;
    const uint32_t yoff = ((uint32_t)tc * (uint32_t)p.ldy + (odd ? 16 + kq * 4 - 4 : kq * 4)) * 2u;
    float ssq = 0.f;
#pragma unroll
    for (int ip = 0; ip < 8; ++ip) {
      const int i0 = 2 * ip, i1 = 2 * ip + 1;
      f32x4 y0 = out[i0][j], y1 = out[i1][j];
      if (KEEL) {
        const f32x4 g0 = *reinterpret_cast<const f32x4*>(gl + i0 * 16 + kq * 4);
        const f32x4 g1 = *reinterpret_cast<const f32x4*>(gl + i1 * 16 + kq * 4);
#pragma unroll
        for (int e = 0; e < 4; ++e) { y0[e] = y0[e] * scale * g0[e]; y1[e] = y1[e] * scale * g1[e]; }
      }
      const bf16x4 q0 = {(bf16_t)y0[0], (bf16_t)y0[1], (bf16_t)y0[2], (bf16_t)y0[3]};
      const bf16x4 q1 = {(bf16_t)y1[0], (bf16_t)y1[1], (bf16_t)y1[2], (bf16_t)y1[3]};
      const uint2 p0 = __builtin_bit_cast(uint2, q0), p1 = __builtin_bit_cast(uint2, q1);
      if (BACK) {
        xq[j][ip] = __builtin_bit_cast(bf16x8, make_uint4(p0.x, p0.y, p1.x, p1.y));
#pragma unroll
        for (int e = 0; e < 4; ++e) {
          const float r0 = (float)q0[e], r1 = (float)q1[e];
          ssq = fmaf(r0, r0, ssq);
          ssq = fmaf(r1, r1, ssq);
        }
      }
      const uint4 ov = xchg16_pair(p0, p1);
      if (tv && !(p.debug & 1)) *(__attribute__((address_space(1))) u32x4_t*)(gy + yoff + ip * 64) = (u32x4_t){ov.x, ov.y, ov.z, ov.w};
    }
    if (BACK) {
      ssq = quad16_sum(ssq);
      rstdq[j] = 1.0f / sqrtf(ssq * (1.0f / 256.0f) + p.eps);
    }
  }
  MLP_STAMP();

  if (BACK) {
#define GLDS_WQ(qp_, buf_)                                                                                         \
  do {                                                                                                             \
    const uint4* src__ = p.pack + ((size_t)np * MLP_PANEL_CHUNKS + MLP_WO_CHUNKS + (qp_) * MLP_W12_CHUNKS + wave * 64); \
    const uint32_t dst__ = lds_l12 + ((buf_) * MLP_W12_CHUNKS + wave * 64) * 16;                                   \
    MLP_GLDS_4(src__, dst__);                                                                                      \
  } while (0)
    __syncthreads();
    GLDS_WQ(0, 0);
    gchar* const gq = (gchar*)p.qkv;
    gcchar* const grope = (gcchar*)p.rope_cs;
    f32x2 rc[4][T2A], rs[4][T2A];
    uint32_t qoff[T2A];
    bool qv[T2A];
#pragma unroll
    for (int j = 0; j < T2; ++j) {
      const int t = tok0 + 16 * (P2F + j);
      qv[j] = t < p.M;
      const int tc = qv[j] ? t : p.M - 1;
      qoff[j] = ((uint32_t)tc * (uint32_t)p.ldq + kq * 4) * 2u;
      gcchar* cs = grope + ((uint32_t)tc * 64u + kq * 2) * 4u;
#pragma unroll
      for (int i = 0; i < 4; ++i) {
        rc[i][j] = *(const __attribute__((address_space(1))) f32x2*)(cs + i * 32);
        rs[i][j] = *(const __attribute__((address_space(1))) f32x2*)(cs + 128 + i * 32);
      }
    }
    __builtin_amdgcn_s_waitcnt(0x0F70);
    __syncthreads();
    for (int qp = 0; qp < p.nqp; ++qp) {
      if (qp + 1 < p.nqp) GLDS_WQ(qp + 1, (qp + 1) & 1);
      const uint4* img = l12 + (qp & 1) * MLP_W12_CHUNKS;
      f32x4 qa[4][T2A];
      bf16x8 a[2][4];
#pragma unroll
      for (int i = 0; i < 4; ++i) a[0][i] = MLP_LD12(img, i, 0);
#pragma unroll
      for (int s8 = 0; s8 < 8; ++s8) {
        if (s8 + 1 < 8) {
#pragma unroll
          for (int i = 0; i < 4; ++i) a[(s8 + 1) & 1][i] = MLP_LD12(img, i, s8 + 1);
        }
#pragma unroll
        for (int i = 0; i < 4; ++i)
#pragma unroll
          for (int j = 0; j < T2; ++j)
            qa[i][j] = __builtin_amdgcn_mfma_f32_16x16x32_bf16(a[s8 & 1][i], xq[j][s8], s8 ? qa[i][j] : (f32x4){0.f, 0.f, 0.f, 0.f}, 0, 0, 0);
        if (s8 + 1 < 8) __builtin_amdgcn_sched_group_barrier(0x100, 4, 0);
        __builtin_amdgcn_sched_group_barrier(0x008, 4 * T2A, 0);
        __builtin_amdgcn_sched_barrier(0);
      }
      __builtin_amdgcn_s_waitcnt(0x0F70);
      __syncthreads();
      const int f_first = qp * 64;
      const bool rot = f_first < p.rope_q_end || (f_first >= p.rope_k_begin && f_first < p.rope_k_end);
#pragma unroll
      for (int j = 0; j < T2; ++j) {
        const bool odd = kq & 1;
        gchar* const qrow = gq + (qoff[j] - (uint32_t)(kq * 4) * 2u) + (uint32_t)(f_first + (odd ? 16 + kq * 4 - 4 : kq * 4)) * 2u;
#pragma unroll
        for (int ip = 0; ip < 2; ++ip) {
          uint2 pk[2];
#pragma unroll
          for (int u = 0; u < 2; ++u) {
            const int i = 2 * ip + u;
            f32x4 v = qa[i][j] * rstdq[j];
            if (rot)
              v = (f32x4){v[0] * rc[i][j].x - v[1] * rs[i][j].x, v[0] * rs[i][j].x + v[1] * rc[i][j].x,
                          v[2] * rc[i][j].y - v[3] * rs[i][j].y, v[2] * rs[i][j].y + v[3] * rc[i][j].y};
            const bf16x4 q = {(bf16_t)v[0], (bf16_t)v[1], (bf16_t)v[2], (bf16_t)v[3]};
            pk[u] = __builtin_bit_cast(uint2, q);
          }
          const uint4 ox = xchg16_pair(pk[0], pk[1]);
          const u32x4_t ov = {ox.x, ox.y, ox.z, ox.w};
          if (qv[j]) *(__attribute__((address_space(1))) u32x4_t*)(qrow + ip * 64) = ov;
        }
      }
    }
#undef GLDS_WQ
    MLP_STAMP();
  }
#undef GLDS_W12
#undef GLDS_W3
}

template <int TILES, bool KEEL, bool FRONT, bool BACK>
__global__ __launch_bounds__(512, 1) void k_mlp256(MlpDev p) {
  extern __shared__ __attribute__((aligned(16))) uint4 smem[];
  uint4* const l12 = smem;
  uint4* const l3 = smem + 2 * MLP_W12_CHUNKS;
  uint4* const hb = l3 + 2 * MLP_W3_CHUNKS;
  float* const gl = reinterpret_cast<float*>(hb + 2 * TILES * 64);
  if (threadIdx.x < 256) {
    gl[threadIdx.x] = p.post_gain ? p.post_gain[threadIdx.x] : 1.0f;
    gl[256 + threadIdx.x] = (FRONT && p.front_gain) ? p.front_gain[threadIdx.x] : 1.0f;
  }
  const int lane = threadIdx.x & 63;
  const int wave = __builtin_amdgcn_readfirstlane(threadIdx.x >> 6);
  int n_stamp = 0;
  const int tile = blockIdx.x;
  if constexpr (TILES == 9) {
    if (wave < 4) mlp_wave<9, 2, 0, false, KEEL, FRONT, BACK>(p, l12, l3, hb, gl, tile, wave, lane, 2 * wave, 0, n_stamp);
    else if (wave < 6) mlp_wave<9, 0, 3, false, KEEL, FRONT, BACK>(p, l12, l3, hb, gl, tile, wave, lane, 0, 3 * (wave - 4), n_stamp);
    else if (wave == 6) mlp_wave<9, 1, 1, false, KEEL, FRONT, BACK>(p, l12, l3, hb, gl, tile, wave, lane, 8, 6, n_stamp);
    else mlp_wave<9, 0, 2, false, KEEL, FRONT, BACK>(p, l12, l3, hb, gl, tile, wave, lane, 0, 7, n_stamp);
  } else {
    constexpr int NT = TILES / 4;
    constexpr int TA = NT - NT / 2;
    const int g0 = (wave & 3) * NT;
    if (wave < 4) mlp_wave<TILES, TA, NT - TA, false, KEEL, FRONT, BACK>(p, l12, l3, hb, gl, tile, wave, lane, g0, g0 + TA, n_stamp);
    else mlp_wave<TILES, NT - TA, TA, false, KEEL, FRONT, BACK>(p, l12, l3, hb, gl, tile, wave, lane, g0 + TA, g0, n_stamp);
  }
}
#undef MLP_LD12
#undef MLP_GLDS_4
#undef MLP_GLDS_2
#undef MLP_STAMP

bool ttvk_mlp_fused_supported(int dtype, int width, int inner) { return dtype == TTV_BF16 && width == 256 && inner % 32 == 0 && inner > 0; }

int64_t ttvk_mlp_pack_bytes(int inner, int next_qkv_rows) {
  if (inner <= 0 || inner % 32 != 0 || next_qkv_rows < 0) return 0;
  return ((int64_t)(inner / 32) * MLP_PANEL_CHUNKS + MLP_WO_CHUNKS + (int64_t)((next_qkv_rows + 63) / 64) * MLP_W12_CHUNKS) * 16;
}

int ttvk_mlp_pack(const void* w12_folded, const void* w3, const void* wo, const void* next_qkv_folded, int next_qkv_rows, int inner,
                  void* packed, hipStream_t s) {
  TTV_CHECK_ARG(w12_folded && w3 && packed, "mlp_pack: null buffer");
  TTV_CHECK_ARG(inner > 0 && inner % 32 == 0, "mlp_pack: inner %% 32");
  TTV_CHECK_ARG((next_qkv_folded != nullptr) == (next_qkv_rows > 0), "mlp_pack: next_qkv weight and row count must come together");
  TTV_CHECK_ARG(((uintptr_t)w12_folded % 16 == 0) && ((uintptr_t)packed % 16 == 0) && ((uintptr_t)wo % 16 == 0) &&
                    ((uintptr_t)next_qkv_folded % 16 == 0), "mlp_pack: 16-byte alignment");
  const int total = inner / 32 * MLP_PANEL_CHUNKS + MLP_WO_CHUNKS + (next_qkv_rows + 63) / 64 * MLP_W12_CHUNKS;
  hipLaunchKernelGGL(k_mlp_pack, dim3(ttv_cdiv(total, 256)), dim3(256), 0, s, (const bf16_t*)w12_folded, (const bf16_t*)w3,
                     (const bf16_t*)wo, (const bf16_t*)next_qkv_folded, next_qkv_rows, inner, (uint4*)packed);
  TTV_CHECK_LAUNCH("mlp_pack");
  return TTV_OK;
}

int ttvk_mlp_fused(const void* ao, int ldao, const float* front_gain, float front_alpha, const void* x, int ldx, const void* packed,
                   int inner, void* y, int ldy, const float* post_gain, float alpha, float eps, int M, const MlpNextQkv* nq, hipStream_t s) {
  if (M == 0) return TTV_OK;
  TTV_CHECK_ARG(x && packed && y, "mlp_fused: null buffer");
  TTV_CHECK_ARG(inner % 32 == 0 && ldx % 8 == 0 && ldy % 8 == 0 && (!ao || ldao % 8 == 0), "mlp_fused: inner %% 32, leading dims %% 8");
  TTV_CHECK_ARG(((uintptr_t)x % 16 == 0) && ((uintptr_t)packed % 16 == 0) && ((uintptr_t)y % 16 == 0) && ((uintptr_t)ao % 16 == 0),
                "mlp_fused: 16-byte alignment");
  MlpDev d;
  d.x = (const bf16_t*)x; d.ldx = ldx; d.pack = (const uint4*)packed; d.I = inner;
  d.ao = (const bf16_t*)ao; d.ldao = ldao; d.front_gain = front_gain; d.front_alpha = front_alpha;
  d.y = (bf16_t*)y; d.ldy = ldy; d.post_gain = post_gain; d.alpha = alpha; d.eps = eps; d.M = M; d.debug = g_ttv_debug; d.stamps = g_ttv_stamps;
  d.qkv = nullptr; d.ldq = 0; d.rope_cs = nullptr; d.nqp = 0; d.rope_q_end = d.rope_k_begin = d.rope_k_end = 0;
  if (nq) {
    TTV_CHECK_ARG(nq->qkv && nq->rope_cs && nq->rows > 0 && nq->rows % 64 == 0 && nq->ld >= nq->rows && nq->ld % 4 == 0 &&
                      (uintptr_t)nq->qkv % 8 == 0, "mlp_fused: bad next-qkv arguments (rows %% 64, ld %% 4, 8-byte aligned)");
    TTV_CHECK_ARG(nq->rope_q_end % 64 == 0 && nq->rope_k_begin % 64 == 0 && nq->rope_k_end % 64 == 0, "mlp_fused: rotary ranges must be whole heads");
    d.qkv = (bf16_t*)nq->qkv; d.ldq = nq->ld; d.rope_cs = nq->rope_cs; d.nqp = nq->rows / 64;
    d.rope_q_end = nq->rope_q_end; d.rope_k_begin = nq->rope_k_begin; d.rope_k_end = nq->rope_k_end;
  }
  const int cus = 256;
  int tiles = 4;
  long best = -1;
  for (int c = 1; c <= 3; ++c) {
    const long cost = (long)ttv_cdiv(ttv_cdiv(M, 64 * c), cus) * (16 + 19 * c);
    if (best < 0 || cost < best) { best = cost; tiles = 4 * c; }
  }
  if (!nq && !(g_ttv_debug & 32)) {
    const long cost9 = (long)ttv_cdiv(ttv_cdiv(M, 144), cus) * (16 + 14 * 3);
    if (cost9 < best) { best = cost9; tiles = 9; }
  }
  if ((g_ttv_debug & 512) && !nq) tiles = 9;
  if (g_ttv_debug & 8) tiles = 8;
  if (g_ttv_debug & 64) tiles = 4;
  d.n_tiles = ttv_cdiv(M, 16 * tiles);
  const int grid = d.n_tiles;
  const size_t smem = (size_t)(2 * MLP_W12_CHUNKS + 2 * MLP_W3_CHUNKS + 2 * tiles * 64) * sizeof(uint4) + 2048;
  TtvProfScope prof(TTV_KC_GEMM_GEGLU, s);
#define LAUNCH_MLP(TILES_, KEEL_, FRONT_, BACK_)                                                                    \
  do {                                                                                                              \
    (void)hipFuncSetAttribute((const void*)k_mlp256<TILES_, KEEL_, FRONT_, BACK_>, hipFuncAttributeMaxDynamicSharedMemorySize, (int)smem); \
    hipLaunchKernelGGL((k_mlp256<TILES_, KEEL_, FRONT_, BACK_>), dim3(grid), dim3(512), smem, s, d);                \
  } while (0)
#define LAUNCH_MLP_F(TILES_, KEEL_)                                                                                 \
  do {                                                                                                              \
    if (ao && nq) LAUNCH_MLP(TILES_, KEEL_, true, true);                                                            \
    else if (ao) LAUNCH_MLP(TILES_, KEEL_, true, false);                                                            \
    else LAUNCH_MLP(TILES_, KEEL_, false, false);                                                                   \
  } while (0)
#define LAUNCH_MLP_9(KEEL_)                                                                                         \
  do {                                                                                                              \
    if (ao) LAUNCH_MLP(9, KEEL_, true, false);                                                                      \
    else LAUNCH_MLP(9, KEEL_, false, false);                                                                        \
  } while (0)
  TTV_CHECK_ARG(!nq || ao, "mlp_fused: the next-qkv part needs the out_proj front (ttv_layer_tail_fused)");
  if (post_gain) {
    if (tiles == 9) LAUNCH_MLP_9(true); else if (tiles == 12) LAUNCH_MLP_F(12, true); else if (tiles == 8) LAUNCH_MLP_F(8, true); else LAUNCH_MLP_F(4, true);
  } else {
    if (tiles == 9) LAUNCH_MLP_9(false); else if (tiles == 12) LAUNCH_MLP_F(12, false); else if (tiles == 8) LAUNCH_MLP_F(8, false); else LAUNCH_MLP_F(4, false);
  }
#undef LAUNCH_MLP_9
#undef LAUNCH_MLP_F
#undef LAUNCH_MLP
  TTV_CHECK_LAUNCH("mlp_fused");
  return TTV_OK;
}
```

Measured before the change: 30220.

## Write encoder last-layer latent attention compactly and gather residual rows inside fused MLP

In the encoder's last layer, the latent-only attention now writes its output straight into a compact latent buffer using per-clip descriptors. The fused MLP gathers residual rows through a row map and writes its result to a compact buffer, which the encoder tail then reads directly. This removes the two row-gather copy kernels and the scattered tail read. The cost is a new template variant with an indirect row load in the MLP front, plus extra eligibility conditions.

```diff
diff --git a/titok_video_amd/csrc/ttv_api.hip b/titok_video_amd/csrc/ttv_api.hip
--- a/titok_video_amd/csrc/ttv_api.hip
+++ b/titok_video_amd/csrc/ttv_api.hip
@@ -156,7 +156,9 @@
   return dt == TTV_BF16 && img && row_scale && !mx && dm % 128 == 0 && !(dm == 256 && folded);
 }
 
-static int run_layers(const ttv_tower_dims* d, const ttv_tower_weights* w, const ttv_batch* b, const TowerWs& ws, hipStream_t s) {
+static int run_layers(const ttv_tower_dims* d, const ttv_tower_weights* w, const ttv_batch* b, const TowerWs& ws, hipStream_t s,
+                      bool* latent_in_xl = nullptr) {
+  if (latent_in_xl) *latent_in_xl = false;
   const int L = b->total_rows, dm = d->width, g = d->kv_heads * d->head_dim, dt = d->dtype;
   const int split3 = (dt == TTV_F32 && w->f32_split3) ? 1 : 0;
   const bool gen_ok = (dt == TTV_BF16 && dm != 256) || split3;
@@ -170,6 +172,7 @@
   static const bool lat_env = !(getenv("TTV_ENC_LATENT_LAST") && getenv("TTV_ENC_LATENT_LAST")[0] == '0');
   const bool lat_last = lat_env && !(g_ttv_debug & 524288) && d->kind == TTV_ENCODER && b->qblocks_latent && b->n_qblocks_latent > 0 &&
                         b->latent_rows && b->sum_tokens > 0 && b->sum_tokens < L;
+  static const bool latc_env = !(getenv("TTV_ENC_LATENT_COMPACT") && getenv("TTV_ENC_LATENT_COMPACT")[0] == '0');
   static const bool pat_env = !(getenv("TTV_DEC_PATCH_LAST") && getenv("TTV_DEC_PATCH_LAST")[0] == '0');
   const bool pat_last = pat_env && !(g_ttv_debug & 2097152) && d->kind == TTV_DECODER && d->layers >= 2 && b->qblocks_patch &&
                         b->n_qblocks_patch > 0 && !split3 && !b->qblocks_paired;
@@ -213,10 +216,18 @@
     rstd_valid = false;
     qkv_ready = false;
     const bool lat_now = lat_last && i == d->layers - 1;
-    if (lat_now)
+    static const bool use_fused_mlp = !(getenv("TTV_FUSED_MLP") && getenv("TTV_FUSED_MLP")[0] == '0');
+    const int lat_flags = TTV_ATTN_GATE | (b->qblocks_all_full ? TTV_ATTN_ALLFULL : 0) | (q_scaled ? TTV_ATTN_QSCALED : 0) |
+                          (split3 ? TTV_ATTN_SPLIT3 : 0) | (s3img ? (TTV_ATTN_SPLIT_OUT | TTV_ATTN_SPLIT_IN) : 0);
+    const bool lat_direct = lat_now && latc_env && !(g_ttv_debug & 4194304) && i > 0 && b->clip_desc && d->head_dim == 64 &&
+                            ttvk_attention_is_swp(lat_flags, dt) && use_fused_mlp && ttvk_mlp_fused_supported(dt, dm, d->inner) && lw.mlp_pack;
+    if (lat_direct) {
+      TtvProfScope prof(TTV_KC_ATTENTION, s);
+      TTV_TRY(ttvk_attention_swp(ws.qkv, nq, ws.aol, dm, b->cu_seqlens, b->qblocks_latent, b->n_qblocks_latent, d->q_heads, d->kv_heads, 1, s,
+                                 b->clip_desc));
+    } else if (lat_now)
       TTV_TRY(ttvk_attention(ws.qkv, nq, ws.ao, dm, b->cu_seqlens, b->qblocks_latent, b->n_qblocks_latent, d->q_heads, d->kv_heads, d->head_dim,
-                             TTV_ATTN_GATE | (b->qblocks_all_full ? TTV_ATTN_ALLFULL : 0) | (q_scaled ? TTV_ATTN_QSCALED : 0) | (split3 ? TTV_ATTN_SPLIT3 : 0) |
-                                 (s3img ? (TTV_ATTN_SPLIT_OUT | TTV_ATTN_SPLIT_IN) : 0), dt, s));
+                             lat_flags, dt, s));
     else if (pat_last && i == d->layers - 1 && dt == TTV_BF16 && !attn_pipe)
       TTV_TRY(ttvk_attention(ws.qkv, nq, ws.ao, dm, b->cu_seqlens, b->qblocks_patch, b->n_qblocks_patch, d->q_heads, d->kv_heads, d->head_dim,
                              TTV_ATTN_GATE | (b->qblocks_all_full ? TTV_ATTN_ALLFULL : 0) | (q_scaled ? TTV_ATTN_QSCALED : 0), dt, s));
@@ -231,6 +242,12 @@
     char* cx = ws.x;
     char* cao = ws.ao;
     int Lc = L;
+    if (lat_direct) {
+      TTV_TRY(ttvk_mlp_fused(ws.aol, dm, lw.attn_post_ln, d->alpha, ws.x, dm, lw.mlp_pack, d->inner, ws.xl, dm, lw.ffd_post_ln, d->alpha, d->eps,
+                             b->sum_tokens, nullptr, s, b->latent_rows));
+      if (latent_in_xl) *latent_in_xl = true;
+      continue;
+    }
     if (lat_now) {
       const int64_t rb = (int64_t)dm * esize(dt);
       TTV_TRY(ttvk_copy_rows(ws.x, (int64_t)dm * esize(dt), b->latent_rows, ws.xl, (int64_t)dm * esize(dt), nullptr, b->sum_tokens, dm * (int)esize(dt), s));
@@ -239,7 +256,6 @@
       compacted = true;
     }
     static const bool keel_f32sum = getenv("TTV_KEEL_F32SUM") && getenv("TTV_KEEL_F32SUM")[0] == '1';
-    static const bool use_fused_mlp = !(getenv("TTV_FUSED_MLP") && getenv("TTV_FUSED_MLP")[0] == '0');
     static const bool use_fused_qkv = getenv("TTV_FUSED_QKV") && getenv("TTV_FUSED_QKV")[0] == '1';
     if (use_fused_mlp && ttvk_mlp_fused_supported(dt, dm, d->inner) && lw.mlp_pack) {
       MlpNextQkv nx = {};
@@ -585,9 +601,10 @@
   TTV_TRY(ttvk_rmsnorm(ws.pb, dt, dm, nullptr, ws.x, dt, dm, b->patch_rows, w->ln_pre_p, P, dm, d->eps, s));
   TTV_TRY(ttvk_fill_const_rows(ws.x, dt, dm, b->latent_rows, b->sum_tokens, dm, w->mask_token, w->ln_pre_t, d->eps, s));
 
-  TTV_TRY(run_layers(d, w, b, ws, s));
-
-  TTV_TRY(ttvk_enc_tail(ws.x, dt, dm, b->latent_rows, b->sum_tokens, dm, w->ln_post, d->eps, w->proj_out_w, w->proj_out_b, d->token_size, fsq, z, codes, indices, bounded, s));
+  bool lat_xl = false;
+  TTV_TRY(run_layers(d, w, b, ws, s, &lat_xl));
+
+  TTV_TRY(ttvk_enc_tail(lat_xl ? ws.xl : ws.x, dt, dm, lat_xl ? nullptr : b->latent_rows, b->sum_tokens, dm, w->ln_post, d->eps, w->proj_out_w, w->proj_out_b, d->token_size, fsq, z, codes, indices, bounded, s));
   return TTV_OK;
 }
 
diff --git a/titok_video_amd/csrc/ttv_attn.hip b/titok_video_amd/csrc/ttv_attn.hip
--- a/titok_video_amd/csrc/ttv_attn.hip
+++ b/titok_video_amd/csrc/ttv_attn.hip
@@ -1370,6 +1370,12 @@
   return TTV_OK;
 }
 
+bool ttvk_attention_is_swp(int flags, int dtype) {
+  static const bool swp_env = !(getenv("TTV_ATTN_SWP") && getenv("TTV_ATTN_SWP")[0] == '0');
+  return dtype == TTV_BF16 && swp_env && !(flags & TTV_ATTN_PIPE) && (flags & TTV_ATTN_ALLFULL) && (flags & TTV_ATTN_QSCALED) &&
+         !(flags & TTV_ATTN_PAIRED) && !(g_ttv_debug & 1048576);
+}
+
 int ttvk_attention(const void* qkvg, int ld, void* out, int ldo, const int* cu_seqlens, const int* qblocks, int n_qblocks,
                    int q_heads, int kv_heads, int head_dim, int flags, int dtype, hipStream_t s, float* lse_out, void* out_raw) {
   const int gate_mul = flags & 1, paired = (flags >> 1) & 1, prescaled = (flags >> 2) & 1;
@@ -1399,8 +1405,7 @@
   } while (0)
     const bool tape = lse_out != nullptr || out_raw != nullptr;
     TTV_CHECK_ARG(!tape || !prescaled, "attention: the training-tape outputs need unscaled q");
-    static const bool swp_env = !(getenv("TTV_ATTN_SWP") && getenv("TTV_ATTN_SWP")[0] == '0');
-    if (swp_env && !(flags & TTV_ATTN_PIPE) && (flags & TTV_ATTN_ALLFULL) && prescaled && !paired && !tape && !(g_ttv_debug & 1048576)) {
+    if (!tape && ttvk_attention_is_swp(flags, dtype)) {
       return ttvk_attention_swp(qkvg, ld, out, ldo, cu_seqlens, qblocks, n_qblocks, q_heads, kv_heads, gate_mul, s);
     }
     if ((flags & TTV_ATTN_PIPE) && (flags & TTV_ATTN_ALLFULL) && prescaled && !paired && !tape) {
diff --git a/titok_video_amd/csrc/ttv_attn_swp.hip b/titok_video_amd/csrc/ttv_attn_swp.hip
--- a/titok_video_amd/csrc/ttv_attn_swp.hip
+++ b/titok_video_amd/csrc/ttv_attn_swp.hip
@@ -37,10 +37,10 @@
 #define SWP_STAMP(seg_)
 #endif
 
-template <bool GATE>
+template <bool GATE, bool COMPACT>
 __global__ __launch_bounds__(256, SWP_OCC) void k_attn_swp(const bf16_t* __restrict__ qkvg, int ld, bf16_t* __restrict__ out, int ldo,
                                                      const int* __restrict__ cu, const int* __restrict__ qblocks, int d_model, int gqa,
-                                                     int rep, long long* __restrict__ stamps) {
+                                                     int rep, const int* __restrict__ clip_desc, long long* __restrict__ stamps) {
   __shared__ __attribute__((aligned(16))) uint4 kl[SWP_NS][SWP_KB * 8];
   __shared__ __attribute__((aligned(16))) uint4 vl[SWP_NS][SWP_KB * 8];
 
@@ -367,9 +367,15 @@
 
   const float inv_l = __builtin_amdgcn_rcpf(l_tot);
   {
-    bf16_t* orow = out + (size_t)(s0 + qrc) * ldo + head * 64;
+    int obase = s0, qlim = S;
+    if (COMPACT) {
+      const int* dsc = clip_desc + 8 * seq;
+      obase = s0 - dsc[6];
+      qlim = S - dsc[3] * dsc[4] * dsc[5];
+    }
+    bf16_t* orow = out + (size_t)(obase + qrc) * ldo + head * 64;
     const bf16_t* grow = gbase + (size_t)qrc * ld;
-    const bool store = qrow < S;
+    const bool store = qrow < qlim;
 #pragma unroll
     for (int dt = 0; dt < 2; ++dt)
 #pragma unroll
@@ -408,15 +414,19 @@
 }
 
 int ttvk_attention_swp(const void* qkvg, int ld, void* out, int ldo, const int* cu_seqlens, const int* qblocks, int n_qblocks,
-                       int q_heads, int kv_heads, int gate_mul, hipStream_t s) {
+                       int q_heads, int kv_heads, int gate_mul, hipStream_t s, const int* clip_desc) {
   const int d_model = q_heads * 64, gqa = kv_heads * 64, rep = q_heads / kv_heads;
   dim3 grid(n_qblocks);
-  if (gate_mul)
-    hipLaunchKernelGGL((k_attn_swp<true>), grid, dim3(256), 0, s, (const bf16_t*)qkvg, ld, (bf16_t*)out, ldo, cu_seqlens, qblocks, d_model,
-                       gqa, rep, g_ttv_stamps);
+  TTV_CHECK_ARG(!clip_desc || gate_mul, "attention_swp: compact output rows are a gated-attention option");
+  if (clip_desc)
+    hipLaunchKernelGGL((k_attn_swp<true, true>), grid, dim3(256), 0, s, (const bf16_t*)qkvg, ld, (bf16_t*)out, ldo, cu_seqlens, qblocks,
+                       d_model, gqa, rep, clip_desc, g_ttv_stamps);
+  else if (gate_mul)
+    hipLaunchKernelGGL((k_attn_swp<true, false>), grid, dim3(256), 0, s, (const bf16_t*)qkvg, ld, (bf16_t*)out, ldo, cu_seqlens, qblocks,
+                       d_model, gqa, rep, (const int*)nullptr, g_ttv_stamps);
   else
-    hipLaunchKernelGGL((k_attn_swp<false>), grid, dim3(256), 0, s, (const bf16_t*)qkvg, ld, (bf16_t*)out, ldo, cu_seqlens, qblocks, d_model,
-                       gqa, rep, g_ttv_stamps);
+    hipLaunchKernelGGL((k_attn_swp<false, false>), grid, dim3(256), 0, s, (const bf16_t*)qkvg, ld, (bf16_t*)out, ldo, cu_seqlens, qblocks,
+                       d_model, gqa, rep, (const int*)nullptr, g_ttv_stamps);
   TTV_CHECK_LAUNCH("attention_swp");
   return TTV_OK;
 }
diff --git a/titok_video_amd/csrc/ttv_elem.hip b/titok_video_amd/csrc/ttv_elem.hip
--- a/titok_video_amd/csrc/ttv_elem.hip
+++ b/titok_video_amd/csrc/ttv_elem.hip
@@ -564,7 +564,7 @@
   const int wave = threadIdx.x >> 6, lane = threadIdx.x & 63;
   const int r = blockIdx.x * ROWS_PER_BLOCK + wave;
   if (r >= rows) return;
-  const T* px = x + (size_t)rows_map[r] * ld;
+  const T* px = x + (size_t)(rows_map ? rows_map[r] : r) * ld;
   f32x4 v[MAX_ITERS];
   float ss = 0.f;
 #pragma unroll
diff --git a/titok_video_amd/csrc/ttv_kernels.h b/titok_video_amd/csrc/ttv_kernels.h
--- a/titok_video_amd/csrc/ttv_kernels.h
+++ b/titok_video_amd/csrc/ttv_kernels.h
@@ -86,7 +86,8 @@
                    void* out_raw = nullptr);
 
 int ttvk_attention_swp(const void* qkvg, int ld, void* out, int ldo, const int* cu_seqlens, const int* qblocks, int n_qblocks,
-                       int q_heads, int kv_heads, int gate_mul, hipStream_t s);
+                       int q_heads, int kv_heads, int gate_mul, hipStream_t s, const int* clip_desc = nullptr);
+bool ttvk_attention_is_swp(int flags, int dtype);
 int ttvk_attention_mxout(const void* qkvg, int ld, void* out_q, void* out_mx, int ld_mx, const int* cu_seqlens, const int* qblocks,
                          int n_qblocks, int q_heads, int kv_heads, hipStream_t s);
 
@@ -111,7 +112,8 @@
 int ttvk_mlp_pack(const void* w12_folded, const void* w3, const void* wo, const void* next_qkv_folded, int next_qkv_rows, int inner,
                   void* packed, hipStream_t s);
 int ttvk_mlp_fused(const void* ao, int ldao, const float* front_gain, float front_alpha, const void* x, int ldx, const void* packed,
-                   int inner, void* y, int ldy, const float* post_gain, float alpha, float eps, int M, const MlpNextQkv* nq, hipStream_t s);
+                   int inner, void* y, int ldy, const float* post_gain, float alpha, float eps, int M, const MlpNextQkv* nq, hipStream_t s,
+                   const int* x_rows = nullptr);
 
 int ttvk_l1_loss(void* const* recon, void* const* target, void* const* grad, const int* sizes, int n_clips, int total_clips, int dtype,
                  float* loss, hipStream_t s);
diff --git a/titok_video_amd/csrc/ttv_mlp.hip b/titok_video_amd/csrc/ttv_mlp.hip
--- a/titok_video_amd/csrc/ttv_mlp.hip
+++ b/titok_video_amd/csrc/ttv_mlp.hip
@@ -10,6 +10,7 @@
   const bf16_t* x; int ldx;
   const uint4* pack;
   const bf16_t* ao; int ldao;
+  const int* x_rows;
   const float* front_gain;
   float front_alpha;
   bf16_t* qkv; int ldq;
@@ -103,7 +104,7 @@
 #define MLP_STAMP() do { (void)n_stamp; } while (0)
 #endif
 
-template <int TPB, int T1, int T2, bool GELU_FIRST, bool KEEL, bool FRONT, bool BACK>
+template <int TPB, int T1, int T2, bool GELU_FIRST, bool KEEL, bool FRONT, bool BACK, bool XMAP>
 __device__ __forceinline__ void mlp_wave(const MlpDev& p, uint4* l12, uint4* l3, uint4* hb, const float* gl, int tile, int wave, int lane,
                                          int P1F, int P2F, int& n_stamp) {
   constexpr int T1A = T1 > 0 ? T1 : 1, T2A = T2 > 0 ? T2 : 1;
@@ -191,7 +192,8 @@
     for (int j = 0; j < T1; ++j) {
       const int t = tok0 + 16 * (P1F + j);
       const int tc = t < p.M ? t : p.M - 1;
-      const uint32_t roff = ((uint32_t)tc * (uint32_t)p.ldx + kq * 4) * 2u;
+      const int xr = XMAP ? p.x_rows[tc] : tc;
+      const uint32_t roff = ((uint32_t)xr * (uint32_t)p.ldx + kq * 4) * 2u;
       float ss = 0.f;
 #pragma unroll
       for (int m = 0; m < 16; ++m) {
@@ -535,8 +537,9 @@
 #undef GLDS_W3
 }
 
-template <int TILES, bool KEEL, bool FRONT, bool BACK>
+template <int TILES, bool KEEL, bool FRONT, bool BACK, bool XMAP = false>
 __global__ __launch_bounds__(512, 1) void k_mlp256(MlpDev p) {
+  static_assert(!XMAP || FRONT, "the residual row map exists for the fused front only");
   extern __shared__ __attribute__((aligned(16))) uint4 smem[];
   uint4* const l12 = smem;
   uint4* const l3 = smem + 2 * MLP_W12_CHUNKS;
@@ -551,16 +554,16 @@
   int n_stamp = 0;
   const int tile = blockIdx.x;
   if constexpr (TILES == 9) {
-    if (wave < 4) mlp_wave<9, 2, 0, false, KEEL, FRONT, BACK>(p, l12, l3, hb, gl, tile, wave, lane, 2 * wave, 0, n_stamp);
-    else if (wave < 6) mlp_wave<9, 0, 3, false, KEEL, FRONT, BACK>(p, l12, l3, hb, gl, tile, wave, lane, 0, 3 * (wave - 4), n_stamp);
-    else if (wave == 6) mlp_wave<9, 1, 1, false, KEEL, FRONT, BACK>(p, l12, l3, hb, gl, tile, wave, lane, 8, 6, n_stamp);
-    else mlp_wave<9, 0, 2, false, KEEL, FRONT, BACK>(p, l12, l3, hb, gl, tile, wave, lane, 0, 7, n_stamp);
+    if (wave < 4) mlp_wave<9, 2, 0, false, KEEL, FRONT, BACK, XMAP>(p, l12, l3, hb, gl, tile, wave, lane, 2 * wave, 0, n_stamp);
+    else if (wave < 6) mlp_wave<9, 0, 3, false, KEEL, FRONT, BACK, XMAP>(p, l12, l3, hb, gl, tile, wave, lane, 0, 3 * (wave - 4), n_stamp);
+    else if (wave == 6) mlp_wave<9, 1, 1, false, KEEL, FRONT, BACK, XMAP>(p, l12, l3, hb, gl, tile, wave, lane, 8, 6, n_stamp);
+    else mlp_wave<9, 0, 2, false, KEEL, FRONT, BACK, XMAP>(p, l12, l3, hb, gl, tile, wave, lane, 0, 7, n_stamp);
   } else {
     constexpr int NT = TILES / 4;
     constexpr int TA = NT - NT / 2;
     const int g0 = (wave & 3) * NT;
-    if (wave < 4) mlp_wave<TILES, TA, NT - TA, false, KEEL, FRONT, BACK>(p, l12, l3, hb, gl, tile, wave, lane, g0, g0 + TA, n_stamp);
-    else mlp_wave<TILES, NT - TA, TA, false, KEEL, FRONT, BACK>(p, l12, l3, hb, gl, tile, wave, lane, g0 + TA, g0, n_stamp);
+    if (wave < 4) mlp_wave<TILES, TA, NT - TA, false, KEEL, FRONT, BACK, XMAP>(p, l12, l3, hb, gl, tile, wave, lane, g0, g0 + TA, n_stamp);
+    else mlp_wave<TILES, NT - TA, TA, false, KEEL, FRONT, BACK, XMAP>(p, l12, l3, hb, gl, tile, wave, lane, g0 + TA, g0, n_stamp);
   }
 }
 #undef MLP_LD12
@@ -590,7 +593,8 @@
 }
 
 int ttvk_mlp_fused(const void* ao, int ldao, const float* front_gain, float front_alpha, const void* x, int ldx, const void* packed,
-                   int inner, void* y, int ldy, const float* post_gain, float alpha, float eps, int M, const MlpNextQkv* nq, hipStream_t s) {
+                   int inner, void* y, int ldy, const float* post_gain, float alpha, float eps, int M, const MlpNextQkv* nq, hipStream_t s,
+                   const int* x_rows) {
   if (M == 0) return TTV_OK;
   TTV_CHECK_ARG(x && packed && y, "mlp_fused: null buffer");
   TTV_CHECK_ARG(inner % 32 == 0 && ldx % 8 == 0 && ldy % 8 == 0 && (!ao || ldao % 8 == 0), "mlp_fused: inner %% 32, leading dims %% 8");
@@ -598,7 +602,7 @@
                 "mlp_fused: 16-byte alignment");
   MlpDev d;
   d.x = (const bf16_t*)x; d.ldx = ldx; d.pack = (const uint4*)packed; d.I = inner;
-  d.ao = (const bf16_t*)ao; d.ldao = ldao; d.front_gain = front_gain; d.front_alpha = front_alpha;
+  d.ao = (const bf16_t*)ao; d.ldao = ldao; d.x_rows = x_rows; d.front_gain = front_gain; d.front_alpha = front_alpha;
   d.y = (bf16_t*)y; d.ldy = ldy; d.post_gain = post_gain; d.alpha = alpha; d.eps = eps; d.M = M; d.debug = g_ttv_debug; d.stamps = g_ttv_stamps;
   d.qkv = nullptr; d.ldq = 0; d.rope_cs = nullptr; d.nqp = 0; d.rope_q_end = d.rope_k_begin = d.rope_k_end = 0;
   if (nq) {
@@ -626,11 +630,12 @@
   const int grid = d.n_tiles;
   const size_t smem = (size_t)(2 * MLP_W12_CHUNKS + 2 * MLP_W3_CHUNKS + 2 * tiles * 64) * sizeof(uint4) + 2048;
   TtvProfScope prof(TTV_KC_GEMM_GEGLU, s);
-#define LAUNCH_MLP(TILES_, KEEL_, FRONT_, BACK_)                                                                    \
+#define LAUNCH_MLP_X(TILES_, KEEL_, FRONT_, BACK_, XMAP_)                                                           \
   do {                                                                                                              \
-    (void)hipFuncSetAttribute((const void*)k_mlp256<TILES_, KEEL_, FRONT_, BACK_>, hipFuncAttributeMaxDynamicSharedMemorySize, (int)smem); \
-    hipLaunchKernelGGL((k_mlp256<TILES_, KEEL_, FRONT_, BACK_>), dim3(grid), dim3(512), smem, s, d);                \
-  } while (0)
+    (void)hipFuncSetAttribute((const void*)k_mlp256<TILES_, KEEL_, FRONT_, BACK_, XMAP_>, hipFuncAttributeMaxDynamicSharedMemorySize, (int)smem); \
+    hipLaunchKernelGGL((k_mlp256<TILES_, KEEL_, FRONT_, BACK_, XMAP_>), dim3(grid), dim3(512), smem, s, d);         \
+  } while (0)
+#define LAUNCH_MLP(TILES_, KEEL_, FRONT_, BACK_) LAUNCH_MLP_X(TILES_, KEEL_, FRONT_, BACK_, false)
 #define LAUNCH_MLP_F(TILES_, KEEL_)                                                                                 \
   do {                                                                                                              \
     if (ao && nq) LAUNCH_MLP(TILES_, KEEL_, true, true);                                                            \
@@ -643,7 +648,11 @@
     else LAUNCH_MLP(9, KEEL_, false, false);                                                                        \
   } while (0)
   TTV_CHECK_ARG(!nq || ao, "mlp_fused: the next-qkv part needs the out_proj front (ttv_layer_tail_fused)");
-  if (post_gain) {
+  TTV_CHECK_ARG(!x_rows || (ao && post_gain && !nq && x != y), "mlp_fused: a residual row map needs the front, a post norm, no next-qkv part and y apart from x");
+  if (x_rows) {
+    if (tiles == 9) LAUNCH_MLP_X(9, true, true, false, true); else if (tiles == 12) LAUNCH_MLP_X(12, true, true, false, true);
+    else if (tiles == 8) LAUNCH_MLP_X(8, true, true, false, true); else LAUNCH_MLP_X(4, true, true, false, true);
+  } else if (post_gain) {
     if (tiles == 9) LAUNCH_MLP_9(true); else if (tiles == 12) LAUNCH_MLP_F(12, true); else if (tiles == 8) LAUNCH_MLP_F(8, true); else LAUNCH_MLP_F(4, true);
   } else {
     if (tiles == 9) LAUNCH_MLP_9(false); else if (tiles == 12) LAUNCH_MLP_F(12, false); else if (tiles == 8) LAUNCH_MLP_F(8, false); else LAUNCH_MLP_F(4, false);
@@ -651,6 +660,7 @@
 #undef LAUNCH_MLP_9
 #undef LAUNCH_MLP_F
 #undef LAUNCH_MLP
+#undef LAUNCH_MLP_X
   TTV_CHECK_LAUNCH("mlp_fused");
   return TTV_OK;
 }
```

Measured after the change: 30290, median of 6. Within noise of the previous version (+0.2%).
